# goroda/c3sc

Hardware: AMD Instinct MI355X
Metric: Bellman-sweep nodes/sec (7D car rank-10) (higher is better)
Workload: dtype f64

## Files before the change

c3sc_amd/csrc/c3sc_hip.hip:

```cpp
#include <hip/hip_runtime.h>

#include <algorithm>
#include <cmath>
#include <cstdio>
#include <cstdlib>
#include <cstring>
#include <string>
#include <vector>

#include "../../include/c3sc_hip.h"
#include "fiber_partition.hpp"
#include "kernel_common.hpp"
#include "kernel_rollout.hpp"
#include "kernel_rollout_ode.hpp"
#include "model_tables.hpp"
#include "registry.hpp"

namespace c3sc {

std::vector<KernelEntry> &kernel_registry()
{
    static std::vector<KernelEntry> reg;
    return reg;
}

__global__ void k_pad_core(const double *__restrict__ src, double *__restrict__ dst, int N, int r0, int r1, int RP,
                           int kind )
{
    const int per = (kind == 1) ? RP * RP : RP;
    const long total = (long)N * per;
    for (long e = (long)blockIdx.x * blockDim.x + threadIdx.x; e < total; e += (long)gridDim.x * blockDim.x) {
        const int j = (int)(e / per), w = (int)(e - (long)j * per);
        int a, b;
        if (kind == 0) { a = 0; b = w; }
        else if (kind == 2) { a = w; b = 0; }
        else { a = w % RP; b = w / RP; }
        double v = 0.0;
        if (a < r0 && b < r1) v = src[(size_t)j * r0 * r1 + a + (size_t)b * r0];
        dst[e] = v;
    }
}

struct ImgJobs {
    int n;
    long src[3 * MAXD + 2], dst[3 * MAXD + 2];
    int nodes[3 * MAXD + 2], per[3 * MAXD + 2], stride[3 * MAXD + 2];
    int tab[3 * MAXD + 2], nodes2[3 * MAXD + 2];
    long src2[3 * MAXD + 2];
};
__global__ void k_core_images(double *__restrict__ arena, const ImgJobs J)
{
    const int jb = blockIdx.y;
    const double *core = arena + J.src[jb];
    double *img = arena + J.dst[jb];
    const int per = J.per[jb], stride = J.stride[jb];
    if (J.tab[jb] != 0) {
        const double *core2 = arena + J.src2[jb];
        const int RP = per, n2 = J.nodes2[jb];
        const bool left = J.tab[jb] == 1;
        const long total = (long)J.nodes[jb] * n2 * RP;
        for (long e = (long)blockIdx.x * blockDim.x + threadIdx.x; e < total; e += (long)gridDim.x * blockDim.x) {
            const long row = e / RP;
            const int c = (int)(e - row * RP), a = (int)(row / n2), b = (int)(row - (long)a * n2);
            const double *vec = left ? core + (size_t)a * RP : core2 + (size_t)b * RP;
            const double *mat = left ? core2 + (size_t)b * RP * RP + (size_t)c * RP : core + (size_t)a * RP * RP + c;
            const int ms = left ? 1 : RP;
            double t = 0.0;
            for (int s = 0; s < RP; s++) t = fma(vec[s], mat[(size_t)s * ms], t);
            img[e] = t;
        }
        return;
    }
    const long total = (long)J.nodes[jb] * stride;
    for (long e = (long)blockIdx.x * blockDim.x + threadIdx.x; e < total; e += (long)gridDim.x * blockDim.x) {
        const int j = (int)(e / stride), w = (int)(e - (long)j * stride);
        img[e] = (w < per) ? core[(size_t)j * per + w] : 0.0;
    }
}

__global__ void k_quad_aux(const double *__restrict__ core, double *__restrict__ coreT, double *__restrict__ aop, int N, int RP)
{
    const int C = RP / 4, MB = (C + 3) / 4;
    const int per_t = RP * RP, per_a = 2 * MB * C * 64;
    const long total = (long)N * (per_t + per_a);
    for (long e = (long)blockIdx.x * blockDim.x + threadIdx.x; e < total; e += (long)gridDim.x * blockDim.x) {
        const int j = (int)(e / (per_t + per_a)), w = (int)(e - (long)j * (per_t + per_a));
        const double *G = core + (size_t)j * per_t;
        if (w < per_t) {
            const int a = w / RP, b = w % RP;
            coreT[(size_t)j * per_t + w] = G[a + b * RP];
        } else {
            const int u = w - per_t;
            const int l = u % 64, s = (u / 64) % C, mb = (u / (64 * C)) % MB, prod = u / (64 * C * MB);
            const int i = l % 16, g = 4 * mb + i / 4;
            const int xc = (i % 4) * C + g, yc = (l / 16) * C + s;
            double v = 0.0;
            if (g < C) v = (prod == 0) ? G[xc + yc * RP] : G[yc + xc * RP];
            aop[(size_t)j * per_a + u] = v;
        }
    }
}

__global__ void k_peak_fma(double *out, int iters)
{
    double a0 = threadIdx.x * 1e-9, a1 = a0 + 1, a2 = a0 + 2, a3 = a0 + 3, a4 = a0 + 4, a5 = a0 + 5, a6 = a0 + 6, a7 = a0 + 7;
    const double m = 1.0000001, c = 1e-9;
    for (int i = 0; i < iters; i++) {
        a0 = fma(a0, m, c); a1 = fma(a1, m, c); a2 = fma(a2, m, c); a3 = fma(a3, m, c);
        a4 = fma(a4, m, c); a5 = fma(a5, m, c); a6 = fma(a6, m, c); a7 = fma(a7, m, c);
    }
    out[(size_t)blockIdx.x * blockDim.x + threadIdx.x] = a0 + a1 + a2 + a3 + a4 + a5 + a6 + a7;
}

typedef double v4d __attribute__((ext_vector_type(4)));
__global__ void k_peak_mfma(double *out, int iters)
{
    v4d c0 = {0, 0, 0, 0}, c1 = c0, c2 = c0, c3 = c0;
    const double a = 1.0 + threadIdx.x * 1e-9, b = 1e-9;
    for (int i = 0; i < iters; i++) {
        c0 = __builtin_amdgcn_mfma_f64_16x16x4f64(a, b, c0, 0, 0, 0);
        c1 = __builtin_amdgcn_mfma_f64_16x16x4f64(a, b, c1, 0, 0, 0);
        c2 = __builtin_amdgcn_mfma_f64_16x16x4f64(a, b, c2, 0, 0, 0);
        c3 = __builtin_amdgcn_mfma_f64_16x16x4f64(a, b, c3, 0, 0, 0);
    }
    out[(size_t)blockIdx.x * blockDim.x + threadIdx.x] = c0[0] + c1[1] + c2[2] + c3[3];
}

}

using namespace c3sc;

#include "ctx.hpp"

static int model_ncf(int model) { return model == C3SC_MODEL_SCAR4D ? 1 : (model == C3SC_MODEL_COTHRUST6D ? 3 : 0); }
static double model_cand_feature(int model, int q, const double *u)
{
    if (model == C3SC_MODEL_COTHRUST6D) {
        const double m = 1.227, g = 9.81, mg = m * g;
        const double cphi = cos(u[1]), sphi = sin(u[1]), cth = cos(u[2]), sth = sin(u[2]);
        return q == 0 ? cphi * sth * (u[0] - mg) / m : (q == 1 ? -sphi * (u[0] - mg) / m : g + cth * cphi * (u[0] - mg) / m);
    }
    (void)q;
    return tan(u[0]);
}

static size_t static_layout(c3sc_hip_ctx *c)
{
    size_t off = c->xgrid_flat.size();
    c->obs_off = (int)off;
    off += c->obs.size();
    c->cands_off = (int)off;
    off += c->cands.size();
    for (int t = 0; t < 4; t++) c->tab_off[t] = 0;
    const int nt = model_ntab(c->model);
    for (int t = 0; t < nt; t++) {
        const int dim = model_tab_dim(c->model, t);
        c->tab_off[t] = (int)off;
        off += (dim < c->d) ? (size_t)c->ngrid[dim] : 0;
    }
    c->cfeat_off = (int)off;
    off += (size_t)model_ncf(c->model) * c->ncand;
    c->hz_off = (int)off;
    off += 4;
    return (off + 15) & ~(size_t)15;
}

static int upload_static(c3sc_hip_ctx *c)
{
    std::vector<double> st(c->static_doubles, 0.0);
    std::copy(c->xgrid_flat.begin(), c->xgrid_flat.end(), st.begin());
    std::copy(c->obs.begin(), c->obs.end(), st.begin() + c->obs_off);
    std::copy(c->cands.begin(), c->cands.end(), st.begin() + c->cands_off);
    const int nt = model_ntab(c->model);
    for (int t = 0; t < nt; t++) {
        const int dim = model_tab_dim(c->model, t);
        if (dim >= c->d) continue;
        const double *g = c->xgrid_flat.data() + c->xg_off_rel[dim];
        for (int i = 0; i < c->ngrid[dim]; i++) st[c->tab_off[t] + i] = model_table_value(c->model, t, g[i]);
    }
    const int ncf = model_ncf(c->model);
    for (int q = 0; q < c->ncand * ncf; q++)
        st[c->cfeat_off + q] = model_cand_feature(c->model, q % ncf, c->cands.data() + (size_t)(q / ncf) * c->du);
    if (c->hz_dt > 0.0) {
        st[c->hz_off] = c->hz_dt;
        st[c->hz_off + 1] = std::exp(-c->discount * c->hz_dt);
        st[c->hz_off + 2] = c->hz_dt / c->h2;
    }
    HIPCHK(c, hipMemcpy(c->arena, st.data(), st.size() * sizeof(double), hipMemcpyHostToDevice));
    c->static_dirty = false;
    return C3SC_OK;
}

static const size_t SMALL_BATCH_FIBERS = 16384;

template <class Fn>
static void each_entry(int model, Fn &&f)
{
    for (const auto &e : kernel_registry()) f(e);
    if (model == 0 || model >= C3SC_MODEL_USER) {
        const RtcEntries r = rtc_entries();
        for (int i = 0; i < r.n; i++) f(*r.e[i]);
    }
}

static const KernelEntry *find_kernel(int model, int d, int rank_needed, int N, int variant, int k, size_t F = (size_t)-1,
                                      const std::vector<const KernelEntry *> *skip = nullptr)
{
    const KernelEntry *best = nullptr;
    const bool small = (variant == C3SC_VARIANT_AUTO) && F < SMALL_BATCH_FIBERS;
    each_entry(model, [&](const KernelEntry &e) {
        if (!is_fiber_variant(e.variant)) return;
        if (e.model != model || e.d != d || e.rp < rank_needed || e.max_n < N) return;
        if (skip && std::find(skip->begin(), skip->end(), &e) != skip->end()) return;
        if (e.k >= 0 && e.k != k) return;
        if (variant != C3SC_VARIANT_AUTO && e.variant != variant) return;
        auto pref = [small](int v) {
            if (small) return v == C3SC_VARIANT_FIBER_PER_WAVE ? 0 : (v == C3SC_VARIANT_FIBER_PAIR ? 1 : (v == C3SC_VARIANT_FIBER_QUAD ? 2 : 3));
            return v == C3SC_VARIANT_FIBER_PAIR ? 0 : (v == C3SC_VARIANT_FIBER_QUAD ? 1 : (v == C3SC_VARIANT_FIBER_PER_WAVE ? 2 : 3));
        };
        if (!best || e.rp < best->rp || (e.rp == best->rp && pref(e.variant) < pref(best->variant)) ||
            (e.rp == best->rp && e.variant == best->variant && e.npl < best->npl))
            best = &e;
    });
    return best;
}

static int pick_rp(int d, int maxrank, int model, int variant)
{
    int rp = 0;
    if (variant != C3SC_VARIANT_AUTO)
        each_entry(model, [&](const KernelEntry &e) {
            if (is_fiber_variant(e.variant) && e.d == d && e.variant == variant && (model == 0 || e.model == model) && e.rp >= maxrank && (rp == 0 || e.rp < rp)) rp = e.rp;
        });
    if (rp) return rp;
    if (model != 0)
        each_entry(model, [&](const KernelEntry &e) {
            if (is_fiber_variant(e.variant) && e.d == d && e.model == model && e.rp >= maxrank && (rp == 0 || e.rp < rp)) rp = e.rp;
        });
    if (rp) return rp;
    each_entry(model, [&](const KernelEntry &e) {
        if (is_fiber_variant(e.variant) && e.d == d && e.rp >= maxrank && (rp == 0 || e.rp < rp)) rp = e.rp;
    });
    return rp;
}

static unsigned long long g_launches = 0;
static int fill_args(c3sc_hip_ctx *c, int k, size_t F, KArgs &A, bool need_model);

static int check_horizon_model(c3sc_hip_ctx *c, const char *what)
{
    if (c->hz_dt > 0.0 && !(c->model >= C3SC_MODEL_USER && rtc_model_horizon(c->model) && c->game_gsz == 0))
        return fail(c, C3SC_ERR_UNSUPPORTED, what);
    return C3SC_OK;
}

static int check_game_model(c3sc_hip_ctx *c, const char *what)
{
    int du = 0;
    bool game = false;
    if (c->game_gsz > 0 && !(c->model >= C3SC_MODEL_USER && rtc_model_info(c->model, du, game) && game && du == c->du))
        return fail(c, C3SC_ERR_UNSUPPORTED, what);
    return C3SC_OK;
}

static int ensure_scratch(c3sc_hip_ctx *c, size_t bytes)
{
    if (bytes <= c->scratch_bytes) return C3SC_OK;
    if (c->scratch) HIPCHK(c, hipFree(c->scratch));
    c->scratch = nullptr;
    c->scratch_bytes = 0;
    HIPCHK(c, hipMalloc(&c->scratch, bytes));
    c->scratch_bytes = bytes;
    return C3SC_OK;
}

static size_t align256(size_t x) { return (x + 255) & ~(size_t)255; }

static constexpr size_t ZERO_COPY_MAX_BYTES = (size_t)1 << 20;
static bool zero_copy_batch(size_t bytes)
{
    static const bool off = getenv("C3SC_NO_ZEROCOPY") != nullptr;
    return !off && bytes <= ZERO_COPY_MAX_BYTES;
}
static int ensure_pinned(c3sc_hip_ctx *c, size_t bytes)
{
    if (bytes <= c->pinned_bytes) return C3SC_OK;
    if (c->pinned) HIPCHK(c, hipHostFree(c->pinned));
    c->pinned = c->pinned_dev = nullptr;
    c->pinned_bytes = 0;
    const size_t cap = bytes < ((size_t)256 << 10) ? ((size_t)256 << 10) : bytes;
    HIPCHK(c, hipHostMalloc(&c->pinned, cap, hipHostMallocMapped | hipHostMallocPortable));
    HIPCHK(c, hipHostGetDevicePointer(&c->pinned_dev, c->pinned, 0));
    c->pinned_bytes = cap;
    return C3SC_OK;
}

enum SegDir { SEG_IN, SEG_OUT };
struct HostSeg { const void *host; size_t bytes; SegDir dir; };
enum Staging {
    STAGE_MAPPED_OR_SCRATCH,
    STAGE_SCRATCH,
    STAGE_PER_CALL,
};
struct DevPtr {
    void *p;
    template <class T> operator T *() const { return static_cast<T *>(p); }
};

template <size_t NS, class Call>
static int stage_host(c3sc_hip_ctx *c, Staging kind, const char *what, const HostSeg (&segs)[NS], Call &&call)
{
    size_t off[NS + 1] = {0};
    for (size_t i = 0; i < NS; i++) off[i + 1] = off[i] + align256(segs[i].bytes);
    auto copy = [&](SegDir dir, char *hb, const DevPtr *dev) -> int {
        for (size_t i = 0; i < NS; i++) {
            if (!dev[i].p || segs[i].dir != dir || segs[i].bytes == 0) continue;
            void *h = const_cast<void *>(segs[i].host), *b = hb ? hb + off[i] : dev[i].p;
            void *dst = dir == SEG_IN ? b : h, *src = dir == SEG_IN ? h : b;
            if (hb) memcpy(dst, src, segs[i].bytes);
            else if (hipError_t e = hipMemcpy(dst, src, segs[i].bytes, dir == SEG_IN ? hipMemcpyHostToDevice : hipMemcpyDeviceToHost); e != hipSuccess) {
                c->err = std::string(what) + ": hipMemcpy of buffer " + std::to_string(i) + (dir == SEG_IN ? " in: " : " out: ") + hipGetErrorString(e);
                return C3SC_ERR_HIP;
            }
        }
        return C3SC_OK;
    };
    auto run = [&](char *hb, char *db) -> int {
        DevPtr dev[NS];
        for (size_t i = 0; i < NS; i++) dev[i].p = segs[i].host ? db + off[i] : nullptr;
        int rc = copy(SEG_IN, hb, dev);
        if (rc == C3SC_OK) rc = call(dev);
        if (rc != C3SC_OK) return rc;
        if (hb) HIPCHK(c, hipStreamSynchronize(nullptr));
        return copy(SEG_OUT, hb, dev);
    };
    HIPCHK(c, hipSetDevice(c->device));
    const size_t total = off[NS];
    int rc;
    if (kind == STAGE_MAPPED_OR_SCRATCH && zero_copy_batch(total))
        return (rc = ensure_pinned(c, total)) != C3SC_OK ? rc : run((char *)c->pinned, (char *)c->pinned_dev);
    if (kind != STAGE_PER_CALL) return (rc = ensure_scratch(c, total)) != C3SC_OK ? rc : run(nullptr, (char *)c->scratch);
    void *buf = nullptr;
    HIPCHK(c, hipMalloc(&buf, total));
    rc = run(nullptr, (char *)buf);
    (void)hipFree(buf);
    return rc;
}

extern "C" {

int c3sc_hip_max_rank(int model, int d)
{
    int rp = 0;
    each_entry(model, [&](const KernelEntry &e) {
        if (e.model == model && e.d == d && e.rp > rp) rp = e.rp;
    });
    return rp;
}

int c3sc_hip_device_count(void)
{
    int n = 0;
    if (hipGetDeviceCount(&n) != hipSuccess) return 0;
    return n;
}

int c3sc_hip_ctx_create(int device, c3sc_hip_ctx **out)
{
    if (!out) return C3SC_ERR_ARG;
    *out = nullptr;
    int n = 0;
    if (hipGetDeviceCount(&n) != hipSuccess || n <= 0 || device < 0 || device >= n) return C3SC_ERR_NODEVICE;
    c3sc_hip_ctx *c = new c3sc_hip_ctx();
    c->device = device;
    if (hipSetDevice(device) != hipSuccess || hipMalloc((void **)&c->d_status, sizeof(unsigned)) != hipSuccess ||
        hipMemset(c->d_status, 0, sizeof(unsigned)) != hipSuccess || hipEventCreate(&c->ev0) != hipSuccess ||
        hipEventCreate(&c->ev1) != hipSuccess) {
        delete c;
        return C3SC_ERR_HIP;
    }
    *out = c;
    return C3SC_OK;
}

void c3sc_hip_ctx_destroy(c3sc_hip_ctx *c)
{
    if (!c) return;
    (void)hipSetDevice(c->device);
    if (c->arena) (void)hipFree(c->arena);
    if (c->hz_stack) (void)hipFree(c->hz_stack);
    if (c->d_status) (void)hipFree(c->d_status);
    if (c->d_dbg) (void)hipFree(c->d_dbg);
    if (c->scratch) (void)hipFree(c->scratch);
    if (c->sim_state) (void)hipFree(c->sim_state);
    for (void *p : c->part)
        if (p) (void)hipFree(p);
    if (c->pinned) (void)hipHostFree(c->pinned);
    c3sc_hip_cross_free(c);
    for (int i = 0; i < c3sc_hip_ctx::NSIDE; i++) {
        if (c->side[i]) { (void)hipStreamSynchronize(c->side[i]); (void)hipStreamDestroy(c->side[i]); }
        if (c->join_ev[i]) (void)hipEventDestroy(c->join_ev[i]);
    }
    if (c->fork_ev) (void)hipEventDestroy(c->fork_ev);
    if (c->ev0) (void)hipEventDestroy(c->ev0);
    if (c->ev1) (void)hipEventDestroy(c->ev1);
    delete c;
}

const char *c3sc_hip_last_error(const c3sc_hip_ctx *c) { return c ? c->err.c_str() : "null context"; }
const char *c3sc_hip_last_kernel(const c3sc_hip_ctx *c) { return c ? c->last_kernel : ""; }

int c3sc_hip_set_grid(c3sc_hip_ctx *c, int d, const size_t *ngrid, const double *const *xgrid)
{
    if (!c || !ngrid || !xgrid || d < 2 || d > MAXD) return fail(c, C3SC_ERR_ARG, "set_grid: need 2 <= d <= 12");
    c->d = d;
    c->xgrid_flat.clear();
    for (int m = 0; m < d; m++) {
        if (ngrid[m] < 2 || ngrid[m] > 4096) return fail(c, C3SC_ERR_ARG, "set_grid: need 2 <= N_m <= 4096");
        c->ngrid[m] = (int)ngrid[m];
        c->xg_off_rel[m] = (int)c->xgrid_flat.size();
        c->xgrid_flat.insert(c->xgrid_flat.end(), xgrid[m], xgrid[m] + ngrid[m]);
    }
    c->static_dirty = true;
    c->have_value = false;
    return C3SC_OK;
}

int c3sc_hip_set_boundary(c3sc_hip_ctx *c, const int *bctype, int nobs, const double *obs_lb, const double *obs_ub)
{
    if (!c || c->d == 0 || !bctype) return fail(c, C3SC_ERR_ARG, "set_boundary: set_grid first");
    if (nobs < 0 || nobs > C3SC_MAX_OBSTACLES) return fail(c, C3SC_ERR_ARG, "set_boundary: at most 10 obstacles (boundary.c:393)");
    for (int m = 0; m < c->d; m++) {
        if (bctype[m] != C3SC_ABSORB && bctype[m] != C3SC_PERIODIC && bctype[m] != C3SC_REFLECT)
            return fail(c, C3SC_ERR_ARG, "set_boundary: boundary type must be absorb/periodic/reflect (nodeutil.c:532-535)");
        c->bctype[m] = bctype[m];
    }
    c->nobs = nobs;
    c->obs.assign((size_t)nobs * 2 * c->d, 0.0);
    for (int o = 0; o < nobs; o++)
        for (int m = 0; m < c->d; m++) {
            c->obs[((size_t)o * 2 + 0) * c->d + m] = obs_lb[(size_t)o * c->d + m];
            c->obs[((size_t)o * 2 + 1) * c->d + m] = obs_ub[(size_t)o * c->d + m];
        }
    c->have_boundary = true;
    c->static_dirty = true;
    return C3SC_OK;
}

int c3sc_hip_set_consistent_ends(c3sc_hip_ctx *c, int on)
{
    if (!c) return C3SC_ERR_ARG;
    c->cends = on ? 1 : 0;
    return C3SC_OK;
}

int c3sc_hip_get_consistent_ends(const c3sc_hip_ctx *c) { return c ? c->cends : -1; }

int c3sc_hip_set_mca(c3sc_hip_ctx *c, double h2, const double *t, double discount)
{
    if (!c || c->d == 0 || !t) return fail(c, C3SC_ERR_ARG, "set_mca: set_grid first");
    c->h2 = h2;
    c->discount = discount;
    for (int i = 0; i < 2 * c->d; i++) c->t[i] = t[i];
    c->have_mca = true;
    if (c->hz_dt > 0.0) c->static_dirty = true;
    return C3SC_OK;
}

int c3sc_hip_set_horizon_step(c3sc_hip_ctx *c, double dt)
{
    if (!c) return C3SC_ERR_ARG;
    if (dt == 0.0) {
        if (c->hz_dt > 0.0) c->static_dirty = true;
        c->hz_dt = 0.0;
        return C3SC_OK;
    }
    if (!(dt > 0.0) || !std::isfinite(dt)) return fail(c, C3SC_ERR_ARG, "set_horizon_step: dt must be positive and finite (0 clears)");
    if (!c->have_mca) return fail(c, C3SC_ERR_ARG, "set_horizon_step: set_mca first");
    if (c->model == 0) return fail(c, C3SC_ERR_ARG, "set_horizon_step: set_model first");
    if (c->model < C3SC_MODEL_USER || !rtc_model_known(c->model))
        return fail(c, C3SC_ERR_UNSUPPORTED, "set_horizon_step: horizon mode needs a run-time compiled model (c3sc_hip_model_compile_fh with horizon = 1)");
    if (!rtc_model_horizon(c->model))
        return fail(c, C3SC_ERR_UNSUPPORTED, "set_horizon_step: this model was compiled without horizon kernels (c3sc_hip_model_compile_fh, horizon = 1)");
    if (c->game_gsz > 0) return fail(c, C3SC_ERR_UNSUPPORTED, "set_horizon_step: games have no horizon form");
    c->hz_dt = dt;
    c->static_dirty = true;
    return C3SC_OK;
}

int c3sc_hip_set_model(c3sc_hip_ctx *c, int model, const double *params, int nparams)
{
    if (!c || model <= 0 || nparams < 0 || nparams > C3SC_MAX_PARAMS) return fail(c, C3SC_ERR_ARG, "set_model: bad arguments");
    if (model >= C3SC_MODEL_USER && !rtc_model_known(model)) return fail(c, C3SC_ERR_ARG, "set_model: no run-time model has this id");
    c->model = model;
    std::memset(c->prm, 0, sizeof(c->prm));
    for (int i = 0; i < nparams; i++) c->prm[i] = params[i];
    c->static_dirty = true;
    return C3SC_OK;
}

int c3sc_hip_set_controls(c3sc_hip_ctx *c, int ncand, int du, const double *cands)
{
    if (!c || ncand < 1 || du < 1 || !cands) return fail(c, C3SC_ERR_ARG, "set_controls: bad arguments");
    c->ncand = ncand;
    c->du = du;
    c->cands.assign(cands, cands + (size_t)ncand * du);
    c->static_dirty = true;
    c->game_gsz = c->game_ngrp = c->game_order = 0;
    return C3SC_OK;
}

int c3sc_hip_set_game(c3sc_hip_ctx *c, int du_min, int nu, const double *U, int nw, const double *W, int order)
{
    if (!c) return C3SC_ERR_ARG;
    if (nu == 0) {
        c->game_gsz = c->game_ngrp = c->game_order = 0;
        return C3SC_OK;
    }
    if (order != C3SC_GAME_MINMAX && order != C3SC_GAME_MAXMIN) return fail(c, C3SC_ERR_ARG, "set_game: order must be C3SC_GAME_MINMAX or C3SC_GAME_MAXMIN");
    if (c->model == 0) return fail(c, C3SC_ERR_ARG, "set_game: set_model first");
    if (c->model == C3SC_MODEL_TABLE) return fail(c, C3SC_ERR_UNSUPPORTED, "set_game: the TABLE model has no game kernels");
    if (c->hz_dt > 0.0) return fail(c, C3SC_ERR_UNSUPPORTED, "set_game: games have no horizon form (c3sc_hip_set_horizon_step(ctx, 0) first)");
    int mdu = 0;
    bool has_game = false;
    if (c->model < C3SC_MODEL_USER || !rtc_model_info(c->model, mdu, has_game))
        return fail(c, C3SC_ERR_UNSUPPORTED, "set_game: games need a run-time compiled model (c3sc_hip_model_compile_ex with game = 1)");
    if (!has_game) return fail(c, C3SC_ERR_UNSUPPORTED, "set_game: this model was compiled without game kernels (c3sc_hip_model_compile_ex, game = 1)");
    if (nu < 0 || nw < 1 || du_min < 1 || du_min >= mdu || !U || !W)
        return fail(c, C3SC_ERR_ARG, "set_game: du_min + du_max must equal the model's du, each at least 1, with nu, nw >= 1 and both lists given");
    if ((long long)nu * nw > (1ll << 24)) return fail(c, C3SC_ERR_ARG, "set_game: nu * nw too large");
    const int dmax = mdu - du_min, ncand = nu * nw;
    std::vector<double> cands((size_t)ncand * mdu);
    for (int iu = 0; iu < nu; iu++)
        for (int iw = 0; iw < nw; iw++) {
            const size_t p = order == C3SC_GAME_MINMAX ? (size_t)iu * nw + iw : (size_t)iw * nu + iu;
            double *row = cands.data() + p * mdu;
            for (int i = 0; i < du_min; i++) row[i] = U[(size_t)iu * du_min + i];
            for (int i = 0; i < dmax; i++) row[du_min + i] = W[(size_t)iw * dmax + i];
        }
    c->ncand = ncand;
    c->du = mdu;
    c->cands.swap(cands);
    c->static_dirty = true;
    c->game_order = order;
    c->game_gsz = order == C3SC_GAME_MINMAX ? nw : nu;
    c->game_ngrp = order == C3SC_GAME_MINMAX ? nu : nw;
    return C3SC_OK;
}

int c3sc_hip_set_control_box(c3sc_hip_ctx *c, int du, const double *lb, const double *ub, int grid, int polish)
{
    if (!c || du < 1 || du > C3SC_MAX_DU || !lb || !ub || grid < 2 || polish < 0) return fail(c, C3SC_ERR_ARG, "set_control_box: bad arguments");
    double tot = 1.0;
    for (int i = 0; i < du; i++) {
        if (!(lb[i] <= ub[i])) return fail(c, C3SC_ERR_ARG, "set_control_box: lb > ub");
        c->box_lb[i] = lb[i];
        c->box_ub[i] = ub[i];
        tot *= grid;
    }
    if (tot > 1e6) return fail(c, C3SC_ERR_ARG, "set_control_box: grid^du too large");
    c->box_du = du; c->box_grid = grid; c->box_polish = polish;
    if (c->ncand == 0) {
        c->ncand = 1; c->du = du;
        c->cands.assign(du, 0.0);
        c->static_dirty = true;
    }
    return C3SC_OK;
}

int c3sc_hip_set_variant(c3sc_hip_ctx *c, int variant)
{
    if (!c) return C3SC_ERR_ARG;
    c->variant = variant;
    return C3SC_OK;
}

static int prepare_value(c3sc_hip_ctx *c, const size_t *ranks, size_t *cores_doubles)
{
    if (!c || c->d == 0 || !ranks) return fail(c, C3SC_ERR_ARG, "upload_value: set_grid first");
    const int d = c->d;
    if (ranks[0] != 1 || ranks[d] != 1) return fail(c, C3SC_ERR_ARG, "upload_value: ranks[0] and ranks[d] must be 1");
    size_t maxrank = 1;
    for (int m = 0; m <= d; m++) {
        if (ranks[m] < 1) return fail(c, C3SC_ERR_ARG, "upload_value: rank < 1");
        maxrank = std::max(maxrank, ranks[m]);
    }
    const int rp = pick_rp(d, (int)maxrank, c->model, c->variant);
    if (rp == 0) return fail(c, C3SC_ERR_UNSUPPORTED, "upload_value: no kernel instantiation for this (dim, rank)");
    HIPCHK(c, hipSetDevice(c->device));
    const size_t stat = static_layout(c);
    size_t off = stat;
    long core_off[MAXD];
    for (int m = 0; m < d; m++) {
        core_off[m] = (long)off;
        const size_t per = (m == 0 || m == d - 1) ? rp : (size_t)rp * rp;
        off += ((size_t)c->ngrid[m] * per + 15) & ~(size_t)15;
    }
    const size_t primary_end = off;
    long coreT_off[MAXD] = {0}, aop_off[MAXD] = {0};
    bool have_quad = false;
    for (const auto &e : kernel_registry())
        if (e.variant == C3SC_VARIANT_FIBER_QUAD && e.d == d && e.rp == rp && (c->model == 0 || e.model == c->model)) have_quad = true;
    if (rp % 4 == 0 && have_quad) {
        const int C = rp / 4, MB = (C + 3) / 4;
        for (int m = 1; m < d - 1; m++) {
            coreT_off[m] = (long)off;
            off += ((size_t)c->ngrid[m] * rp * rp + 15) & ~(size_t)15;
            aop_off[m] = (long)off;
            off += ((size_t)c->ngrid[m] * 2 * MB * C * 64 + 15) & ~(size_t)15;
        }
    }
    long img_off[MAXD] = {0};
    for (int m = 0; m < d; m++) {
        const size_t per = (m == 0 || m == d - 1) ? rp : (size_t)rp * rp;
        img_off[m] = (long)off;
        off += (size_t)pair_img_doubles(c->ngrid[m], (int)per);
    }
    long tabL_off = 0, tabR_off = 0;
    bool have_pair = false;
    for (const auto &e : kernel_registry())
        if (e.variant == C3SC_VARIANT_FIBER_PAIR && e.d == d && e.rp == rp) have_pair = true;
    if (d >= 4 && have_pair) {
        tabL_off = (long)off;
        off += (size_t)pair_tab_doubles(c->ngrid[0], c->ngrid[1], rp);
        tabR_off = (long)off;
        off += (size_t)pair_tab_doubles(c->ngrid[d - 2], c->ngrid[d - 1], rp);
    }
    long qimgL_off[MAXD] = {0}, qimgR_off[MAXD] = {0};
    if (rp % 4 == 0 && have_quad) {
        for (int m = 0; m < d; m++) {
            const size_t per = (m == 0 || m == d - 1) ? rp : (size_t)rp * rp;
            const size_t sz = ((size_t)c->ngrid[m] * (per + 2) + 15) & ~(size_t)15;
            if (m < d - 1) { qimgL_off[m] = (long)off; off += sz; }
            if (m > 0) { qimgR_off[m] = (long)off; off += sz; }
        }
    }
    if (off > c->arena_cap) {
        if (c->arena) HIPCHK(c, hipFree(c->arena));
        c->arena = nullptr;
        c->arena_cap = 0;
        HIPCHK(c, hipMalloc((void **)&c->arena, off * sizeof(double)));
        c->arena_cap = off;
        c->static_dirty = true;
    }
    if (stat != c->static_doubles) c->static_dirty = true;
    c->static_doubles = stat;
    for (int m = 0; m < d; m++) { c->core_off[m] = core_off[m]; c->coreT_off[m] = coreT_off[m]; c->aop_off[m] = aop_off[m]; c->img_off[m] = img_off[m]; c->qimgL_off[m] = qimgL_off[m]; c->qimgR_off[m] = qimgR_off[m]; }
    c->tabL_off = tabL_off;
    c->tabR_off = tabR_off;
    for (int m = 0; m <= d; m++) c->ranks[m] = ranks[m];
    c->rp = rp;
    *cores_doubles = primary_end - stat;
    if (c->static_dirty) return upload_static(c);
    return C3SC_OK;
}

static int make_quad_aux(c3sc_hip_ctx *c, void *stream)
{
    for (int m = 1; m < c->d - 1; m++) {
        if (c->aop_off[m] == 0) continue;
        const long total = (long)c->ngrid[m] * (c->rp * c->rp + 2 * ((c->rp / 4 + 3) / 4) * (c->rp / 4) * 64);
        const int grid = (int)std::min<long>((total + 255) / 256, 1024);
        hipLaunchKernelGGL(k_quad_aux, dim3(grid), dim3(256), 0, (hipStream_t)stream, c->arena + c->core_off[m],
                           c->arena + c->coreT_off[m], c->arena + c->aop_off[m], c->ngrid[m], c->rp);
    }
    ImgJobs J;
    J.n = 0;
    long maxtotal = 1;
    auto add = [&](long src, long dst, int nodes, int per, int stride) {
        J.src[J.n] = src; J.dst[J.n] = dst; J.nodes[J.n] = nodes; J.per[J.n] = per; J.stride[J.n] = stride;
        J.tab[J.n] = 0; J.nodes2[J.n] = 0; J.src2[J.n] = 0;
        J.n++;
        maxtotal = std::max(maxtotal, (long)nodes * stride);
    };
    for (int m = 0; m < c->d; m++) {
        const int per = (m == 0 || m == c->d - 1) ? c->rp : c->rp * c->rp;
        add(c->core_off[m], c->img_off[m], c->ngrid[m], per, per | 1);
        if (c->qimgL_off[m]) add(c->core_off[m], c->qimgL_off[m], c->ngrid[m], per, per + 2);
        if (c->qimgR_off[m]) add((m == c->d - 1) ? c->core_off[m] : c->coreT_off[m], c->qimgR_off[m], c->ngrid[m], per, per + 2);
    }
    auto add_tab = [&](int tab, long dst, int ma, int mb) {
        add(c->core_off[ma], dst, c->ngrid[ma], c->rp, c->rp);
        J.tab[J.n - 1] = tab; J.nodes2[J.n - 1] = c->ngrid[mb]; J.src2[J.n - 1] = c->core_off[mb];
        maxtotal = std::max(maxtotal, (long)c->ngrid[ma] * c->ngrid[mb] * c->rp);
    };
    if (c->tabL_off) add_tab(1, c->tabL_off, 0, 1);
    if (c->tabR_off) add_tab(2, c->tabR_off, c->d - 2, c->d - 1);
    hipLaunchKernelGGL(k_core_images, dim3((unsigned)std::min<long>((maxtotal + 255) / 256, 64), (unsigned)J.n), dim3(256), 0, (hipStream_t)stream,
                       c->arena, J);
    HIPCHK(c, hipGetLastError());
    return C3SC_OK;
}

static void pad_cores_host(int d, const int *ngrid, int rp, const size_t *ranks, const double *const *cores, double *const *dst)
{
    for (int m = 0; m < d; m++) {
        const size_t r0 = ranks[m], r1 = ranks[m + 1];
        const double *src = cores[m];
        const size_t per = (m == 0 || m == d - 1) ? rp : (size_t)rp * rp;
        for (int j = 0; j < ngrid[m]; j++)
            for (size_t b = 0; b < r1; b++)
                for (size_t a = 0; a < r0; a++) {
                    const size_t w = (m == 0) ? b : ((m == d - 1) ? a : a + b * rp);
                    dst[m][(size_t)j * per + w] = src[(size_t)j * r0 * r1 + a + b * r0];
                }
    }
}

int c3sc_hip_upload_value(c3sc_hip_ctx *c, const size_t *ranks, const double *const *cores)
{
    size_t cd = 0;
    int rc = prepare_value(c, ranks, &cd);
    if (rc != C3SC_OK) return rc;
    const int d = c->d, rp = c->rp;
    std::vector<double> buf(cd, 0.0);
    double *dst[MAXD];
    for (int m = 0; m < d; m++) dst[m] = buf.data() + (c->core_off[m] - (long)c->static_doubles);
    pad_cores_host(d, c->ngrid, rp, ranks, cores, dst);
    HIPCHK(c, hipMemcpy(c->arena + c->static_doubles, buf.data(), cd * sizeof(double), hipMemcpyHostToDevice));
    rc = make_quad_aux(c, nullptr);
    if (rc != C3SC_OK) return rc;
    HIPCHK(c, hipStreamSynchronize(nullptr));
    c->have_value = true;
    return C3SC_OK;
}

int c3sc_hip_upload_value_stack(c3sc_hip_ctx *c, int nstack, const size_t *ranks, const double *const *cores)
{
    if (!c) return C3SC_ERR_ARG;
    if (nstack == 0) {
        if (c->hz_stack) HIPCHK(c, hipFree(c->hz_stack));
        c->hz_stack = nullptr;
        c->hz_nstack = 0;
        return C3SC_OK;
    }
    if (nstack < 0 || !ranks || !cores) return fail(c, C3SC_ERR_ARG, "upload_value_stack: bad arguments");
    if (c->d == 0 || !c->have_value) return fail(c, C3SC_ERR_ARG, "upload_value_stack: upload_value first (the stack shares its static section)");
    if (static_layout(c) != c->static_doubles)
        return fail(c, C3SC_ERR_ARG, "upload_value_stack: static data changed size after upload_value; upload the value again");
    const int d = c->d;
    std::vector<int> rps(nstack);
    std::vector<long> offs((size_t)nstack * MAXD, 0);
    size_t off = c->static_doubles;
    for (int s = 0; s < nstack; s++) {
        const size_t *r = ranks + (size_t)s * (d + 1);
        if (r[0] != 1 || r[d] != 1) return fail(c, C3SC_ERR_ARG, "upload_value_stack: ranks[s][0] and ranks[s][d] must be 1");
        size_t maxrank = 1;
        for (int m = 0; m <= d; m++) {
            if (r[m] < 1) return fail(c, C3SC_ERR_ARG, "upload_value_stack: rank < 1");
            maxrank = std::max(maxrank, r[m]);
        }
        for (int m = 0; m < d; m++)
            if (!cores[(size_t)s * d + m]) return fail(c, C3SC_ERR_ARG, "upload_value_stack: null core");
        rps[s] = pick_rp(d, (int)maxrank, c->model, C3SC_VARIANT_AUTO);
        if (rps[s] == 0) return fail(c, C3SC_ERR_UNSUPPORTED, "upload_value_stack: no kernel instantiation for a stage's (dim, rank)");
        for (int m = 0; m < d; m++) {
            offs[(size_t)s * MAXD + m] = (long)off;
            const size_t per = (m == 0 || m == d - 1) ? rps[s] : (size_t)rps[s] * rps[s];
            off += ((size_t)c->ngrid[m] * per + 15) & ~(size_t)15;
        }
    }
    std::vector<double> buf(off - c->static_doubles, 0.0);
    for (int s = 0; s < nstack; s++) {
        double *dst[MAXD];
        for (int m = 0; m < d; m++) dst[m] = buf.data() + (offs[(size_t)s * MAXD + m] - (long)c->static_doubles);
        pad_cores_host(d, c->ngrid, rps[s], ranks + (size_t)s * (d + 1), cores + (size_t)s * d, dst);
    }
    HIPCHK(c, hipSetDevice(c->device));
    if (c->hz_stack) HIPCHK(c, hipFree(c->hz_stack));
    c->hz_stack = nullptr;
    c->hz_nstack = 0;
    HIPCHK(c, hipMalloc((void **)&c->hz_stack, off * sizeof(double)));
    HIPCHK(c, hipMemcpy(c->hz_stack + c->static_doubles, buf.data(), buf.size() * sizeof(double), hipMemcpyHostToDevice));
    c->hz_stack_static = c->static_doubles;
    c->hz_rp.swap(rps);
    c->hz_core_off.swap(offs);
    c->hz_nstack = nstack;
    return C3SC_OK;
}

int c3sc_hip_upload_value_device(c3sc_hip_ctx *c, const size_t *ranks, const double *const *d_cores, void *stream)
{
    size_t cd = 0;
    int rc = prepare_value(c, ranks, &cd);
    if (rc != C3SC_OK) return rc;
    const int d = c->d, rp = c->rp;
    for (int m = 0; m < d; m++) {
        const int kind = (m == 0) ? 0 : (m == d - 1 ? 2 : 1);
        const long total = (long)c->ngrid[m] * (kind == 1 ? rp * rp : rp);
        const int grid = (int)std::min<long>((total + 255) / 256, 1024);
        hipLaunchKernelGGL(k_pad_core, dim3(grid), dim3(256), 0, (hipStream_t)stream, d_cores[m], c->arena + c->core_off[m],
                           c->ngrid[m], (int)ranks[m], (int)ranks[m + 1], rp, kind);
    }
    HIPCHK(c, hipGetLastError());
    rc = make_quad_aux(c, stream);
    if (rc != C3SC_OK) return rc;
    c->have_value = true;
    return C3SC_OK;
}

static int fill_args(c3sc_hip_ctx *c, int k, size_t F, KArgs &A, bool need_model)
{
    if (!c) return C3SC_ERR_ARG;
    if (c->d == 0 || !c->have_boundary || !c->have_value) return fail(c, C3SC_ERR_ARG, "launch: grid, boundary and value must be set");
    if (need_model && (!c->have_mca || c->model == 0 || c->ncand == 0))
        return fail(c, C3SC_ERR_ARG, "launch: mca, model and controls must be set");
    if (k < 0 || k >= c->d) return fail(c, C3SC_ERR_ARG, "launch: dim_vary out of range");
    HIPCHK(c, hipSetDevice(c->device));
    if (c->static_dirty) {
        if (static_layout(c) != c->static_doubles)
            return fail(c, C3SC_ERR_ARG, "launch: static data changed size after upload_value; upload the value again");
        int rc = upload_static(c);
        if (rc != C3SC_OK) return rc;
    }
    std::memset(&A, 0, sizeof(A));
    A.d = c->d;
    A.k = k;
    A.N = c->ngrid[k];
    A.ncand = c->ncand;
    A.F = (long)F;
    for (int m = 0; m < c->d; m++) {
        A.ngrid[m] = c->ngrid[m];
        A.bctype[m] = c->bctype[m];
        A.xg_off[m] = c->xg_off_rel[m];
        A.core_off[m] = c->core_off[m];
        A.quad_coreT_off[m] = c->coreT_off[m];
        A.quad_aop_off[m] = c->aop_off[m];
        A.pair_img_off[m] = c->img_off[m];
        A.quad_imgL_off[m] = c->qimgL_off[m];
        A.quad_imgR_off[m] = c->qimgR_off[m];
    }
    A.img_base = c->arena;
    if (c->tabL_off && (c->tabL_off != pair_tabL_off(A, c->rp) || c->tabR_off != pair_tabR_off(A, c->rp)))
        return fail(c, C3SC_ERR_ARG, "launch: the pair kernel's product tables are not where the kernel looks for them");
    A.cends = c->cends;
    A.memo_keys = nullptr;
    A.skip = c->skip_flag;
    A.nobs = c->nobs;
    A.obs_off = c->obs_off;
    A.cands_off = c->cands_off;
    for (int t = 0; t < 4; t++) A.tab_off[t] = c->tab_off[t];
    A.cfeat_off = c->cfeat_off;
    A.h2 = c->h2;
    A.discount = c->discount;
    for (int i = 0; i < 2 * c->d; i++) A.t[i] = c->t[i];
    for (int i = 0; i < C3SC_MAX_PARAMS; i++) A.prm[i] = c->prm[i];
    A.status = c->d_status;
    A.game_gsz = c->game_gsz;
    A.game_ngrp = c->game_ngrp;
    A.game_order = c->game_order;
    A.hz_off = c->hz_dt > 0.0 ? c->hz_off : 0;
    {
        static const int dbg_env = [] { const char *e = getenv("C3SC_DBG"); return e ? atoi(e) : 0; }();
        A.dbg = dbg_env;
        if (dbg_env && !c->d_dbg) { HIPCHK(c, hipMalloc((void **)&c->d_dbg, 65536 * 8 * sizeof(unsigned long long))); }
        A.dbgbuf = c->d_dbg;
        if (A.dbg & 8) A.ncand = 1;
        if (A.dbg & 16) A.ncand = 3;
    }
    return C3SC_OK;
}

static void arm_memo(c3sc_hip_ctx *c, const KernelEntry *e, KArgs &A)
{
    A.memo_keys = nullptr;
    if (c->memo.keys == nullptr || e->variant != C3SC_VARIANT_FIBER_PER_WAVE) return;
    A.memo_keys = c->memo.keys; A.memo_vals = c->memo.vals; A.memo_capmask = c->memo.capmask; A.memo_epoch_bits = c->memo.epoch_bits;
    A.memo_shift = c->memo.shift; A.memo_counters = c->memo.counters; A.memo_mode = c->memo.mode;
    for (int m = 0; m < c->d; m++) A.memo_stride[m] = c->memo.stride[m];
    c->memo.applied = true;
}

static int launch_one(c3sc_hip_ctx *c, const KernelEntry *e, const KArgs &A, const LaunchIO &io, const char *unsupported = nullptr)
{
    c->last_kernel = e->name;
    g_launches++;
    c->status_cache_valid = false;
    const hipError_t he = launch_entry(*e, A, io);
    if (he == hipErrorNotSupported && unsupported) return fail(c, C3SC_ERR_UNSUPPORTED, unsupported);
    HIPCHK(c, he);
    return C3SC_OK;
}

constexpr long FIBER_PARTITION_MIN = 524288;
static long fiber_partition_min()
{
    const char *e = getenv("C3SC_FIBER_PARTITION");
    if (!e || !*e) return FIBER_PARTITION_MIN;
    const long v = atol(e);
    return v > 0 ? v : -1;
}

static long fiber_group_floor()
{
    const char *e = getenv("C3SC_FIBER_GROUP");
    if (!e || !*e) return FPART_MIN_PER_BIN;
    const long v = atol(e);
    return v > 0 ? v : -1;
}

static int partition_fibers(c3sc_hip_ctx *c, const KernelEntry *e, const KArgs &A, LaunchIO &io, int slot, int &launched)
{
    io.perm = nullptr;
    io.nlive = nullptr;
    launched = 0;
    if (e->variant != C3SC_VARIANT_FIBER_PAIR || e->rtc || A.ncand > 64) return C3SC_OK;
    bool faces = false;
    for (int m = 0; m < A.d; m++) faces = faces || (m != A.k && A.bctype[m] == C3SC_ABSORB);
    const long fmin = fiber_partition_min();
    if (!faces || fmin < 0 || A.F < fmin || A.F > 0x40000000L) return C3SC_OK;
    PartArgs P;
    P.d = A.d;
    P.k = A.k;
    P.F = A.F;
    for (int m = 0; m < MAXD; m++) { P.ngrid[m] = A.ngrid[m]; P.bctype[m] = A.bctype[m]; }
    fpart_plan(P, fpp_group_levels(A.d, e->rp, A.k), fiber_group_floor());
    const size_t need = fpart_bytes(A.F, P.nbins);
    if (need > c->part_bytes[slot]) {
        if (c->part[slot]) HIPCHK(c, hipFree(c->part[slot]));
        c->part[slot] = nullptr;
        c->part_bytes[slot] = 0;
        c->part_last[slot] = {};
        HIPCHK(c, hipMalloc(&c->part[slot], need));
        c->part_bytes[slot] = need;
    }
    const PartScratch ps = fpart_carve(c->part[slot], A.F, P.nbins);
    c->part_last[slot] = {ps.perm, ps.nlive, A.F, io.stream};
    HIPCHK(c, fpart_launch(P, io.idx, ps, io.stream));
    launched = 3;
    io.perm = ps.perm;
    io.nlive = ps.nlive;
    return C3SC_OK;
}

static int launch_bellman(c3sc_hip_ctx *c, int k, size_t F, const int32_t *d_idx, const int32_t *d_policy, double *d_out,
                          int32_t *d_uidx, int32_t *d_absorbed, void *stream, int part_slot = 0)
{
    KArgs A;
    int rc = fill_args(c, k, F, A, true);
    if (rc != C3SC_OK) return rc;
    int variant = c->variant;
    if (c->game_gsz > 0) {
        rc = check_game_model(c, "bellman_fibers: game mode needs a model compiled with game kernels of the game's du");
        if (rc != C3SC_OK) return rc;
        if (variant != C3SC_VARIANT_AUTO && variant != C3SC_VARIANT_FIBER_PER_WAVE)
            return fail(c, C3SC_ERR_UNSUPPORTED, "bellman_fibers: game mode runs on the fiber-per-wave kernel only (the pair and quad variants have no game form)");
        variant = C3SC_VARIANT_FIBER_PER_WAVE;
    }
    if (c->hz_dt > 0.0) {
        rc = check_horizon_model(c, "bellman_fibers: horizon mode needs a model compiled with horizon kernels (and no game)");
        if (rc != C3SC_OK) return rc;
        if (variant != C3SC_VARIANT_AUTO && variant != C3SC_VARIANT_FIBER_PER_WAVE)
            return fail(c, C3SC_ERR_UNSUPPORTED, "bellman_fibers: horizon mode runs on the fiber-per-wave kernel only (the pair and quad variants have no horizon form)");
        variant = C3SC_VARIANT_FIBER_PER_WAVE;
    }
    if (F == 0) return C3SC_OK;
    if (!d_idx || !d_out) return fail(c, C3SC_ERR_ARG, "bellman_fibers: null buffer");
    A.forced = d_policy;
    LaunchIO io{c->arena, d_idx, d_out, d_uidx, d_absorbed, nullptr, nullptr, nullptr, nullptr, (hipStream_t)stream};
    std::vector<const KernelEntry *> declined;
    hipError_t he = hipSuccess;
    int part_launches = 0;
    for (;;) {
        const KernelEntry *e = find_kernel(c->model, c->d, c->rp, A.N, variant, k, F, &declined);
        if (!e || e->rp != c->rp) {
            if (declined.empty()) return fail(c, C3SC_ERR_UNSUPPORTED, "bellman_fibers: no kernel instantiation for (model, dim, rank, N)");
            return fail(c, C3SC_ERR_UNSUPPORTED, he == hipErrorOutOfMemory
                            ? "bellman_fibers: N x rank^2 of the varying core exceeds the 160 KB of LDS the per-wave kernel stages it in"
                            : "bellman_fibers: no kernel instantiation serves this call (model, dim, rank, N, control mode)");
        }
        c->last_kernel = e->name;
        arm_memo(c, e, A);
        rc = partition_fibers(c, e, A, io, part_slot, part_launches);
        if (rc != C3SC_OK) return rc;
        he = launch_entry(*e, A, io);
        if (he != hipErrorOutOfMemory && he != hipErrorNotSupported) break;
        c->memo.applied = false;
        if (getenv("C3SC_VERBOSE")) fprintf(stderr, "c3sc: %s declined (%s), trying the next instantiation\n", e->name, hipGetErrorName(he));
        declined.push_back(e);
    }
    g_launches += 1 + part_launches;
    c->status_cache_valid = false;
    HIPCHK(c, he);
    return C3SC_OK;
}

int c3sc_hip_bellman_fibers(c3sc_hip_ctx *c, int k, size_t F, const int32_t *d_idx, double *d_out, int32_t *d_uidx,
                            int32_t *d_absorbed, void *stream)
{
    return launch_bellman(c, k, F, d_idx, nullptr, d_out, d_uidx, d_absorbed, stream);
}

static int launch_bellman_all(c3sc_hip_ctx *c, int nk, const int *ks, const size_t *F, const int32_t *const *d_idx,
                              const int32_t *const *d_policy, double *const *d_out, int32_t *const *d_uidx, int32_t *const *d_absorbed,
                              void *stream)
{
    if (!c) return C3SC_ERR_ARG;
    if (nk < 1 || nk > MAXD || !ks || !F || !d_idx || !d_out) return fail(c, C3SC_ERR_ARG, "bellman_fibers_all: bad arguments");
    static const bool no_overlap = getenv("C3SC_NO_OVERLAP") != nullptr;
    bool overlap = nk > 1 && !no_overlap && c->memo.keys == nullptr && c->skip_flag == nullptr;
    for (int s = 0; s < nk; s++) {
        if (ks[s] < 0 || ks[s] >= c->d) return fail(c, C3SC_ERR_ARG, "bellman_fibers_all: dim_vary out of range");
        if (F[s] > 0 && (!d_idx[s] || !d_out[s])) return fail(c, C3SC_ERR_ARG, "bellman_fibers_all: null buffer");
        if (d_policy && !d_policy[s]) return fail(c, C3SC_ERR_ARG, "bellman_fibers_all: null policy");
        for (int q = 0; q < s; q++)
            if (d_out[q] == d_out[s] && F[s] > 0) return fail(c, C3SC_ERR_ARG, "bellman_fibers_all: two segments share an output array");
    }
    hipStream_t st = (hipStream_t)stream;
    if (overlap) {
        HIPCHK(c, hipSetDevice(c->device));
        if (!c->fork_ev) {
            HIPCHK(c, hipEventCreateWithFlags(&c->fork_ev, hipEventDisableTiming));
            for (int i = 0; i < c3sc_hip_ctx::NSIDE; i++) {
                HIPCHK(c, hipStreamCreateWithFlags(&c->side[i], hipStreamNonBlocking));
                HIPCHK(c, hipEventCreateWithFlags(&c->join_ev[i], hipEventDisableTiming));
            }
        }
        HIPCHK(c, hipEventRecord(c->fork_ev, st));
        for (int i = 0; i < c3sc_hip_ctx::NSIDE; i++) HIPCHK(c, hipStreamWaitEvent(c->side[i], c->fork_ev, 0));
    }
    int rc = C3SC_OK;
    for (int s = 0; s < nk && rc == C3SC_OK; s++) {
        const int lane = overlap ? s % (c3sc_hip_ctx::NSIDE + 1) : 0;
        rc = launch_bellman(c, ks[s], F[s], d_idx[s], d_policy ? d_policy[s] : nullptr, d_out[s], d_uidx ? d_uidx[s] : nullptr,
                            d_absorbed ? d_absorbed[s] : nullptr, lane == 0 ? stream : (void *)c->side[lane - 1], lane);
    }
    if (overlap)
        for (int i = 0; i < c3sc_hip_ctx::NSIDE; i++) {
            HIPCHK(c, hipEventRecord(c->join_ev[i], c->side[i]));
            HIPCHK(c, hipStreamWaitEvent(st, c->join_ev[i], 0));
        }
    return rc;
}

int c3sc_hip_bellman_fibers_all(c3sc_hip_ctx *c, int nk, const int *ks, const size_t *F, const int32_t *const *d_idx, double *const *d_out,
                                int32_t *const *d_uidx, int32_t *const *d_absorbed, void *stream)
{
    return launch_bellman_all(c, nk, ks, F, d_idx, nullptr, d_out, d_uidx, d_absorbed, stream);
}

int c3sc_hip_policy_fibers_all(c3sc_hip_ctx *c, int nk, const int *ks, const size_t *F, const int32_t *const *d_idx,
                               const int32_t *const *d_policy, double *const *d_out, int32_t *const *d_absorbed, void *stream)
{
    if (!d_policy) return fail(c, C3SC_ERR_ARG, "policy_fibers_all: null policy");
    return launch_bellman_all(c, nk, ks, F, d_idx, d_policy, d_out, nullptr, d_absorbed, stream);
}

static int launch_box(c3sc_hip_ctx *c, int k, size_t F, const int32_t *d_idx, const double *d_policy_u, double *d_out,
                      double *d_uopt, int32_t *d_absorbed, void *stream)
{
    if (!c) return C3SC_ERR_ARG;
    if (c->box_du == 0) return fail(c, C3SC_ERR_ARG, "bellman_fibers_box: c3sc_hip_set_control_box first");
    if (c->game_gsz > 0) return fail(c, C3SC_ERR_UNSUPPORTED, "bellman_fibers_box: games have no control-box form");
    if (c->hz_dt > 0.0) return fail(c, C3SC_ERR_UNSUPPORTED, "bellman_fibers_box: horizon mode has no control-box form");
    if (model_ncf(c->model) != 0 && c->model != C3SC_MODEL_COTHRUST6D)
        return fail(c, C3SC_ERR_UNSUPPORTED, "bellman_fibers_box: this model needs transcendental functions of the control");
    KArgs A;
    int rc = fill_args(c, k, F, A, true);
    if (rc != C3SC_OK) return rc;
    if (F == 0) return C3SC_OK;
    if (!d_idx || !d_out) return fail(c, C3SC_ERR_ARG, "bellman_fibers_box: null buffer");
    A.cmode = 1;
    A.ugrid = c->box_grid;
    A.upolish = c->box_polish;
    for (int i = 0; i < c->box_du; i++) { A.ulb[i] = c->box_lb[i]; A.uub[i] = c->box_ub[i]; }
    A.uopt = d_uopt;
    A.forced_u = d_policy_u;
    const KernelEntry *e = find_kernel(c->model, c->d, c->rp, A.N, C3SC_VARIANT_FIBER_PER_WAVE, k);
    if (!e || e->rp != c->rp) return fail(c, C3SC_ERR_UNSUPPORTED, "bellman_fibers_box: no fiber-per-wave instantiation for (model, dim, rank, N)");
    arm_memo(c, e, A);
    LaunchIO io{c->arena, d_idx, d_out, nullptr, d_absorbed, nullptr, nullptr, nullptr, nullptr, (hipStream_t)stream};
    return launch_one(c, e, A, io, "bellman_fibers_box: no box-minimiser instantiation for this model");
}

int c3sc_hip_bellman_fibers_box(c3sc_hip_ctx *c, int k, size_t F, const int32_t *d_idx, double *d_out, double *d_uopt,
                                int32_t *d_absorbed, void *stream)
{
    return launch_box(c, k, F, d_idx, nullptr, d_out, d_uopt, d_absorbed, stream);
}

int c3sc_hip_policy_fibers_box(c3sc_hip_ctx *c, int k, size_t F, const int32_t *d_idx, const double *d_policy_u, double *d_out,
                               int32_t *d_absorbed, void *stream)
{
    if (F != 0 && !d_policy_u) return fail(c, C3SC_ERR_ARG, "policy_fibers_box: null policy");
    return launch_box(c, k, F, d_idx, d_policy_u, d_out, nullptr, d_absorbed, stream);
}

int c3sc_hip_bellman_fibers_box_host(c3sc_hip_ctx *c, int k, size_t F, const int32_t *h_idx, double *h_out, double *h_uopt,
                                     int32_t *h_absorbed)
{
    if (!c || c->d == 0 || k < 0 || k >= c->d || c->box_du == 0) return fail(c, C3SC_ERR_ARG, "bellman_fibers_box_host: bad arguments");
    if (F == 0) return C3SC_OK;
    const size_t FN = F * c->ngrid[k];
    return stage_host(c, STAGE_MAPPED_OR_SCRATCH, "bellman_fibers_box_host",
                      {{h_idx, F * c->d * sizeof(int32_t), SEG_IN}, {h_out, FN * sizeof(double), SEG_OUT},
                       {h_uopt, FN * c->box_du * sizeof(double), SEG_OUT}, {h_absorbed, FN * sizeof(int32_t), SEG_OUT}},
                      [&](const DevPtr *d) { return c3sc_hip_bellman_fibers_box(c, k, F, d[0], d[1], d[2], d[3], nullptr); });
}

int c3sc_hip_policy_fibers_box_host(c3sc_hip_ctx *c, int k, size_t F, const int32_t *h_idx, const double *h_policy_u, double *h_out,
                                    int32_t *h_absorbed)
{
    if (F != 0 && !h_policy_u) return fail(c, C3SC_ERR_ARG, "policy_fibers_box_host: null policy");
    if (!c || c->d == 0 || k < 0 || k >= c->d || c->box_du == 0) return fail(c, C3SC_ERR_ARG, "policy_fibers_box_host: bad arguments");
    if (F == 0) return C3SC_OK;
    const size_t FN = F * c->ngrid[k];
    return stage_host(c, STAGE_MAPPED_OR_SCRATCH, "policy_fibers_box_host",
                      {{h_idx, F * c->d * sizeof(int32_t), SEG_IN}, {h_out, FN * sizeof(double), SEG_OUT},
                       {h_policy_u, FN * c->box_du * sizeof(double), SEG_IN}, {h_absorbed, FN * sizeof(int32_t), SEG_OUT}},
                      [&](const DevPtr *d) { return c3sc_hip_policy_fibers_box(c, k, F, d[0], d[2], d[1], d[3], nullptr); });
}

int c3sc_hip_policy_fibers(c3sc_hip_ctx *c, int k, size_t F, const int32_t *d_idx, const int32_t *d_policy, double *d_out,
                           int32_t *d_absorbed, void *stream)
{
    if (F != 0 && !d_policy) return fail(c, C3SC_ERR_ARG, "policy_fibers: null policy");
    return launch_bellman(c, k, F, d_idx, d_policy, d_out, nullptr, d_absorbed, stream);
}

static int launch_tables(c3sc_hip_ctx *c, int k, size_t F, const int32_t *d_idx, const double *d_tables, const double *d_costs2,
                         const int32_t *d_policy, double *d_out, int32_t *d_uidx, int32_t *d_absorbed, void *stream)
{
    if (!c) return C3SC_ERR_ARG;
    const int saved_model = c->model;
    if (c->game_gsz > 0) return fail(c, C3SC_ERR_UNSUPPORTED, "bellman_fibers_tables: the TABLE model has no game kernels");
    if (c->hz_dt > 0.0) return fail(c, C3SC_ERR_UNSUPPORTED, "bellman_fibers_tables: the TABLE model has no horizon kernels");
    c->model = C3SC_MODEL_TABLE;
    KArgs A;
    int rc = fill_args(c, k, F, A, true);
    c->model = saved_model;
    if (rc != C3SC_OK) return rc;
    if (F == 0) return C3SC_OK;
    if (!d_idx || !d_out || !d_tables || !d_costs2) return fail(c, C3SC_ERR_ARG, "bellman_fibers_tables: null buffer");
    A.forced = d_policy;
    const KernelEntry *e = find_kernel(C3SC_MODEL_TABLE, c->d, c->rp, A.N, C3SC_VARIANT_AUTO, k);
    if (!e || e->rp != c->rp) return fail(c, C3SC_ERR_UNSUPPORTED, "bellman_fibers_tables: no kernel instantiation for (dim, rank, N)");
    LaunchIO io{c->arena, d_idx, d_out, d_uidx, d_absorbed, nullptr, nullptr, d_tables, d_costs2, (hipStream_t)stream};
    return launch_one(c, e, A, io);
}

int c3sc_hip_bellman_fibers_tables(c3sc_hip_ctx *c, int k, size_t F, const int32_t *d_idx, const double *d_tables,
                                   const double *d_costs2, double *d_out, int32_t *d_uidx, int32_t *d_absorbed, void *stream)
{
    return launch_tables(c, k, F, d_idx, d_tables, d_costs2, nullptr, d_out, d_uidx, d_absorbed, stream);
}

int c3sc_hip_policy_fibers_tables(c3sc_hip_ctx *c, int k, size_t F, const int32_t *d_idx, const double *d_tables,
                                  const double *d_costs2, const int32_t *d_policy, double *d_out, int32_t *d_absorbed, void *stream)
{
    if (F != 0 && !d_policy) return fail(c, C3SC_ERR_ARG, "policy_fibers_tables: null policy");
    return launch_tables(c, k, F, d_idx, d_tables, d_costs2, d_policy, d_out, nullptr, d_absorbed, stream);
}

int c3sc_hip_bellman_fibers_tables_host(c3sc_hip_ctx *c, int k, size_t F, const int32_t *h_idx, const double *h_tables,
                                        const double *h_costs2, double *h_out, int32_t *h_uidx, int32_t *h_absorbed)
{
    if (!c || c->d == 0 || k < 0 || k >= c->d || c->ncand == 0) return fail(c, C3SC_ERR_ARG, "bellman_fibers_tables_host: bad arguments");
    if (F == 0) return C3SC_OK;
    const size_t FN = F * c->ngrid[k], S = 2 * c->d + 1;
    return stage_host(c, STAGE_SCRATCH, "bellman_fibers_tables_host",
                      {{h_idx, F * c->d * sizeof(int32_t), SEG_IN}, {h_out, FN * sizeof(double), SEG_OUT}, {h_uidx, FN * sizeof(int32_t), SEG_OUT},
// ... 310 lines not shown
}

int c3sc_hip_simulate_host(c3sc_hip_ctx *c, const c3sc_hip_sim_args *h)
{
    if (!c) return C3SC_ERR_ARG;
    if (!h) return fail(c, C3SC_ERR_ARG, "simulate_host: null argument struct");
    if (h->n == 0) return c3sc_hip_simulate(c, h, nullptr);
    HostShape sh;
    const int rc = closed_loop_host_shape(c, "simulate", h, h->nsteps, sh);
    if (rc != C3SC_OK) return rc;
    const size_t n = sh.n, d = sh.d, D = sizeof(double);
    return stage_host(c, STAGE_PER_CALL, "simulate_host",
                      {{h->d_x0, n * d * D, SEG_IN}, {h->d_noise, h->d_noise ? n * h->nsteps * d * D : 0, SEG_IN},
                       {h->d_traj, h->d_traj ? n * sh.nrow * d * D : 0, SEG_OUT}, {h->d_u, h->d_u ? n * sh.nurow * sh.du * D : 0, SEG_OUT},
                       {h->d_cost, n * D, SEG_OUT}, {h->d_exit, n * sizeof(int64_t), SEG_OUT}, {h->d_vend, n * D, SEG_OUT},
                       {h->d_xfinal, n * d * D, SEG_OUT}},
                      [&](const DevPtr *b) {
                          c3sc_hip_sim_args a = *h;
                          a.d_x0 = b[0]; a.d_noise = b[1]; a.d_traj = b[2]; a.d_u = b[3];
                          a.d_cost = b[4]; a.d_exit = b[5]; a.d_vend = b[6]; a.d_xfinal = b[7];
                          return c3sc_hip_simulate(c, &a, nullptr);
                      });
}

static const size_t ODE_MAX_EVALS = (size_t)1 << 40;

static long long ode_nsub(double dt_out, double dt_int)
{
    if (dt_int == 0.0) return 1;
    const double r = dt_out / dt_int, q = std::nearbyint(r);
    if (!(q >= 1.0) || !(std::fabs(r - q) <= 1e-9 * q) || q > (double)(1 << 30)) return 0;
    return (long long)q;
}

static bool ode_box_ok(const double *b, int d)
{
    if (!b) return true;
    for (int m = 0; m < d; m++)
        if (!(b[m] <= b[d + m])) return false;
    return true;
}

int c3sc_hip_integrate(c3sc_hip_ctx *c, const c3sc_hip_ode_args *a, void *stream)
{
    const char *who = "integrate";
    int rc = closed_loop_setup(c, who, a);
    if (rc != C3SC_OK) return rc;
    if (c->hz_dt > 0.0) return fail(c, C3SC_ERR_UNSUPPORTED, "integrate: deterministic closed loops are not offered in horizon mode");
    KArgs A;
    rc = fill_args(c, 0, 0, A, false);
    if (rc != C3SC_OK) return rc;
    rc = check_bounds_set(c, "integrate: every dimension needs a boundary type");
    if (rc != C3SC_OK) return rc;
    if (!(a->dt_out > 0.0) || !std::isfinite(a->dt_out)) return fail(c, C3SC_ERR_ARG, "integrate: dt_out must be positive and finite");
    if (!(a->dt_int >= 0.0) || !std::isfinite(a->dt_int)) return fail(c, C3SC_ERR_ARG, "integrate: dt_int must be >= 0 and finite");
    const long long nsub = ode_nsub(a->dt_out, a->dt_int);
    if (nsub == 0) return fail(c, C3SC_ERR_ARG, "integrate: dt_out / dt_int is not an integer (to 1e-9 relative)");
    if (a->method != C3SC_ODE_FORWARD_EULER && a->method != C3SC_ODE_RK4)
        return fail(c, C3SC_ERR_ARG, "integrate: method must be C3SC_ODE_FORWARD_EULER or C3SC_ODE_RK4");
    const int nstage = a->method == C3SC_ODE_RK4 ? 4 : 1;
    if (a->nout > (size_t)1 << 30) return fail(c, C3SC_ERR_ARG, "integrate: nout too large");
    if ((size_t)nsub * a->nout * nstage > ODE_MAX_EVALS) return fail(c, C3SC_ERR_ARG, "integrate: more than 2^40 controller evaluations per trajectory");
    rc = closed_loop_sizes(c, who, a, a->nout, "integrate: more than 2^31 trajectories in one call (split the batch)",
                           "integrate: save_every larger than nout");
    if (rc != C3SC_OK) return rc;
    if (a->evals_per_launch < 0) return fail(c, C3SC_ERR_ARG, "integrate: evals_per_launch < 0");
    if (!ode_box_ok(a->goal, c->d) || !ode_box_ok(a->keep, c->d))
        return fail(c, C3SC_ERR_ARG, "integrate: a stop box has lo > hi (or a NaN)");
    const KernelEntry *e = find_sim_kernel(VARIANT_ROLLOUT_ODE, c->model, c->d, c->rp);
    if (!e) return fail(c, C3SC_ERR_UNSUPPORTED, "integrate: no integrate instantiation for this model at this padded rank");
    if (a->n == 0) return C3SC_OK;
    if (!a->d_x0) return fail(c, C3SC_ERR_ARG, "integrate: null d_x0");
    const int d = c->d;
    const size_t n = a->n;
    rc = closed_loop_state(c, n * (size_t)(d + 3) * sizeof(double));
    if (rc != C3SC_OK) return rc;
    closed_loop_box(c, a->box, A);
    OdeK S;
    std::memset(&S, 0, sizeof(S));
    S.n = (long)n;
    S.nsub = (int)nsub;
    S.nout = (int)a->nout;
    S.nstage = nstage;
    S.save_every = (int)a->save_every;
    S.wrap = a->wrap_periodic ? 1 : 0;
    S.constelm = c->constelm;
    S.h = a->dt_int == 0.0 ? a->dt_out : a->dt_int;
    S.dt_out = a->dt_out;
    S.has_goal = a->goal ? 1 : 0;
    S.has_keep = a->keep ? 1 : 0;
    for (int m = 0; m < d; m++) {
        S.goal_lo[m] = a->goal ? a->goal[m] : 0.0;
        S.goal_hi[m] = a->goal ? a->goal[d + m] : 0.0;
        S.keep_lo[m] = a->keep ? a->keep[m] : -INFINITY;
        S.keep_hi[m] = a->keep ? a->keep[d + m] : INFINITY;
    }
    S.x0 = a->d_x0;
    S.x = (double *)c->sim_state;
    S.cost = S.x + n * d;
    S.stop_step = (long long *)(S.cost + n);
    S.stop_reason = (int32_t *)(S.stop_step + n);
    S.traj = a->d_traj;
    S.u = a->d_u;
    S.vend = a->d_vend;
    const long long ktot = nsub * (long long)a->nout;
    const long long chunk = std::max<long long>(1, (a->evals_per_launch > 0 ? a->evals_per_launch : 256) / nstage);
    long long k0 = 0;
    do {
        S.k0 = k0;
        S.k1 = std::min(k0 + chunk, ktot);
        LaunchIO io{c->arena, nullptr, nullptr, nullptr, nullptr, nullptr, nullptr, nullptr, nullptr, (hipStream_t)stream, &S};
        rc = launch_one(c, e, A, io, "integrate: this integrate kernel has no box minimiser");
        if (rc != C3SC_OK) return rc;
        k0 = S.k1;
    } while (k0 < ktot);
    rc = closed_loop_results(c, a, a->d_stop_step, stream);
    if (rc != C3SC_OK) return rc;
    return copy_back(c, a->d_stop_reason, S.stop_reason, n * sizeof(int32_t), stream);
}

int c3sc_hip_integrate_host(c3sc_hip_ctx *c, const c3sc_hip_ode_args *h)
{
    if (!c) return C3SC_ERR_ARG;
    if (!h) return fail(c, C3SC_ERR_ARG, "integrate_host: null argument struct");
    if (h->n == 0) return c3sc_hip_integrate(c, h, nullptr);
    HostShape sh;
    const int rc = closed_loop_host_shape(c, "integrate", h, h->nout, sh);
    if (rc != C3SC_OK) return rc;
    const size_t n = sh.n, d = sh.d, D = sizeof(double);
    return stage_host(c, STAGE_PER_CALL, "integrate_host",
                      {{h->d_x0, n * d * D, SEG_IN}, {h->d_traj, h->d_traj ? n * sh.nrow * d * D : 0, SEG_OUT},
                       {h->d_u, h->d_u ? n * sh.nurow * sh.du * D : 0, SEG_OUT}, {h->d_cost, n * D, SEG_OUT},
                       {h->d_stop_step, n * sizeof(int64_t), SEG_OUT}, {h->d_stop_reason, n * sizeof(int32_t), SEG_OUT},
                       {h->d_vend, n * D, SEG_OUT}, {h->d_xfinal, n * d * D, SEG_OUT}},
                      [&](const DevPtr *b) {
                          c3sc_hip_ode_args a = *h;
                          a.d_x0 = b[0]; a.d_traj = b[1]; a.d_u = b[2]; a.d_cost = b[3];
                          a.d_stop_step = b[4]; a.d_stop_reason = b[5]; a.d_vend = b[6]; a.d_xfinal = b[7];
                          return c3sc_hip_integrate(c, &a, nullptr);
                      });
}

int c3sc_hip_normals(uint64_t seed, uint64_t traj0, size_t ntraj, uint64_t step0, size_t nsteps, int dw, double *out)
{
    if (!out || dw < 1 || dw > MAXD) return C3SC_ERR_ARG;
    for (size_t t = 0; t < ntraj; t++)
        for (size_t k = 0; k < nsteps; k++)
            for (int j = 0; j < dw; j++)
                out[(t * nsteps + k) * dw + j] = philox_normal(seed, traj0 + t, (uint32_t)(step0 + k), (uint32_t)j);
    return C3SC_OK;
}

unsigned long long c3sc_hip_launch_count(void) { return g_launches; }

int c3sc_hip_last_partition(c3sc_hip_ctx *c, int slot, int32_t *perm, size_t cap, size_t *F, int *nlive)
{
    if (!c) return C3SC_ERR_ARG;
    if (slot < 0 || slot > c3sc_hip_ctx::NSIDE || !F || !nlive) return fail(c, C3SC_ERR_ARG, "last_partition: bad arguments");
    const auto &lp = c->part_last[slot];
    if (!lp.perm) return fail(c, C3SC_ERR_ARG, "last_partition: no partition has run on this slot");
    *F = (size_t)lp.F;
    HIPCHK(c, hipStreamSynchronize(lp.stream));
    int32_t nl = 0;
    HIPCHK(c, hipMemcpy(&nl, lp.nlive, sizeof(nl), hipMemcpyDeviceToHost));
    *nlive = nl;
    if (perm) {
        if (cap < (size_t)lp.F) return fail(c, C3SC_ERR_ARG, "last_partition: perm holds fewer than F entries");
        HIPCHK(c, hipMemcpy(perm, lp.perm, (size_t)lp.F * sizeof(int32_t), hipMemcpyDeviceToHost));
    }
    return C3SC_OK;
}

int c3sc_hip_debug_read(c3sc_hip_ctx *c, unsigned long long *out, size_t n)
{
    if (!c || !c->d_dbg || !out) return C3SC_ERR_ARG;
    HIPCHK(c, hipMemcpy(out, c->d_dbg, n * sizeof(unsigned long long), hipMemcpyDeviceToHost));
    return C3SC_OK;
}

int c3sc_hip_timer_start(c3sc_hip_ctx *c, void *stream)
{
    if (!c) return C3SC_ERR_ARG;
    HIPCHK(c, hipEventRecord(c->ev0, (hipStream_t)stream));
    return C3SC_OK;
}

int c3sc_hip_timer_stop(c3sc_hip_ctx *c, void *stream, float *ms)
{
    if (!c || !ms) return C3SC_ERR_ARG;
    HIPCHK(c, hipEventRecord(c->ev1, (hipStream_t)stream));
    HIPCHK(c, hipEventSynchronize(c->ev1));
    HIPCHK(c, hipEventElapsedTime(ms, c->ev0, c->ev1));
    return C3SC_OK;
}

static int run_peak(c3sc_hip_ctx *c, bool mfma, double *tflops)
{
    if (!c || !tflops) return C3SC_ERR_ARG;
    HIPCHK(c, hipSetDevice(c->device));
    const char *ev = getenv("C3SC_PEAK_BLOCKS_PER_CU");
    const int blocks = 256 * (ev ? atoi(ev) : 8), threads = 256, iters = 20000;
    int rc = ensure_scratch(c, (size_t)blocks * threads * sizeof(double));
    if (rc != C3SC_OK) return rc;
    float best = 1e30f;
    for (int rep = 0; rep < 4; rep++) {
        HIPCHK(c, hipEventRecord(c->ev0, nullptr));
        if (mfma) hipLaunchKernelGGL(k_peak_mfma, dim3(blocks), dim3(threads), 0, nullptr, (double *)c->scratch, iters);
        else hipLaunchKernelGGL(k_peak_fma, dim3(blocks), dim3(threads), 0, nullptr, (double *)c->scratch, iters);
        HIPCHK(c, hipEventRecord(c->ev1, nullptr));
        HIPCHK(c, hipEventSynchronize(c->ev1));
        float ms = 0;
        HIPCHK(c, hipEventElapsedTime(&ms, c->ev0, c->ev1));
        if (rep > 0 && ms < best) best = ms;
    }
    const double waves = (double)blocks * threads / 64.0;
    const double flop = mfma ? waves * iters * 4.0 * (2.0 * 16 * 16 * 4) : (double)blocks * threads * iters * 8.0 * 2.0;
    *tflops = flop / (best * 1e-3) / 1e12;
    return C3SC_OK;
}

int c3sc_hip_peak_fma_f64(c3sc_hip_ctx *c, double *tflops) { return run_peak(c, false, tflops); }
int c3sc_hip_peak_mfma_f64(c3sc_hip_ctx *c, double *tflops) { return run_peak(c, true, tflops); }

}
```

c3sc_amd/csrc/ctx.hpp:

```cpp
#pragma once
#include <hip/hip_runtime.h>

#include <string>
#include <vector>

#include "../../include/c3sc_hip.h"
#include "kernel_common.hpp"

struct c3sc_cross_dev;
struct c3sc_hip_comm;

struct c3sc_hip_ctx {
    int device = 0;
    std::string err;
    int d = 0;
    int ngrid[c3sc::MAXD] = {0};
    std::vector<double> xgrid_flat;
    int xg_off_rel[c3sc::MAXD] = {0};
    int bctype[c3sc::MAXD] = {0};
    int cends = 0;
    bool have_boundary = false;
    int nobs = 0;
    std::vector<double> obs;
    bool have_mca = false;
    double h2 = 0, discount = 0, t[2 * c3sc::MAXD] = {0};
    int model = 0;
    double prm[C3SC_MAX_PARAMS] = {0};
    int ncand = 0, du = 0;
    std::vector<double> cands;
    int game_gsz = 0, game_ngrp = 0, game_order = 0;
    double hz_dt = 0.0;
    int hz_off = 0;
    double *hz_stack = nullptr;
    size_t hz_stack_static = 0;
    int hz_nstack = 0;
    std::vector<int> hz_rp;
    std::vector<long> hz_core_off;
    int box_du = 0, box_grid = 0, box_polish = 0;
    double box_lb[C3SC_MAX_DU] = {0}, box_ub[C3SC_MAX_DU] = {0};
    bool have_value = false;
    size_t ranks[c3sc::MAXD + 1] = {0};
    int rp = 0;
    double *arena = nullptr;
    size_t arena_cap = 0;
    size_t static_doubles = 0;
    bool static_dirty = true;
    long core_off[c3sc::MAXD] = {0};
    long coreT_off[c3sc::MAXD] = {0}, aop_off[c3sc::MAXD] = {0};
    long img_off[c3sc::MAXD] = {0};
    long qimgL_off[c3sc::MAXD] = {0}, qimgR_off[c3sc::MAXD] = {0};
    long tabL_off = 0, tabR_off = 0;
    int obs_off = 0, cands_off = 0, tab_off[4] = {0, 0, 0, 0}, cfeat_off = 0;
    unsigned *d_status = nullptr;
    unsigned status_cache = 0;
    bool status_cache_valid = false;
    unsigned long long *d_dbg = nullptr;
    int variant = C3SC_VARIANT_AUTO;
    const char *last_kernel = "";
    hipEvent_t ev0 = nullptr, ev1 = nullptr;
    static constexpr int NSIDE = 2;
    hipStream_t side[NSIDE] = {nullptr, nullptr};
    hipEvent_t fork_ev = nullptr, join_ev[NSIDE] = {nullptr, nullptr};
    void *part[NSIDE + 1] = {nullptr, nullptr, nullptr};
    size_t part_bytes[NSIDE + 1] = {0, 0, 0};
    struct {
        int32_t *perm = nullptr, *nlive = nullptr;
        long F = 0;
        hipStream_t stream = nullptr;
    } part_last[NSIDE + 1];
    void *scratch = nullptr;
    size_t scratch_bytes = 0;
    void *sim_state = nullptr;
    size_t sim_state_bytes = 0;
    int constelm = 0;
    void *pinned = nullptr, *pinned_dev = nullptr;
    size_t pinned_bytes = 0;
    struct {
        unsigned long long *keys = nullptr;
        double *vals = nullptr;
        unsigned long long capmask = 0, epoch_bits = 0;
        int shift = 0;
        long long stride[c3sc::MAXD] = {0};
        unsigned long long *counters = nullptr;
        int mode = 0;
        bool applied = false;
    } memo;
    const int *skip_flag = nullptr;
    c3sc_hip_comm *shard_comm = nullptr;
    c3sc_cross_dev *cross = nullptr;
};

#define HIPCHK(ctx, call)                                                                    \
    do {                                                                                     \
        hipError_t e__ = (call);                                                             \
        if (e__ != hipSuccess) {                                                             \
            (ctx)->err = std::string(#call) + ": " + hipGetErrorString(e__);                 \
            return C3SC_ERR_HIP;                                                             \
        }                                                                                    \
    } while (0)

static inline int fail(c3sc_hip_ctx *ctx, int code, const char *msg)
{
    if (ctx) ctx->err = msg;
    return code;
}
```

c3sc_amd/csrc/inst_car7d_fpp.hip:

```cpp
#include "launch_fpw.hpp"
#include "launch_fpp.hpp"
#include "models.hpp"
namespace c3sc {
#define REG7P(RP)                                  \
    C3SC_REG_FPP1(C3SC_MODEL_CAR7D, RP, 0, Car7D)  \
    C3SC_REG_FPP1(C3SC_MODEL_CAR7D, RP, 1, Car7D)  \
    C3SC_REG_FPP1(C3SC_MODEL_CAR7D, RP, 2, Car7D)  \
    C3SC_REG_FPP1(C3SC_MODEL_CAR7D, RP, 3, Car7D)  \
    C3SC_REG_FPP1(C3SC_MODEL_CAR7D, RP, 4, Car7D)  \
    C3SC_REG_FPP1(C3SC_MODEL_CAR7D, RP, 5, Car7D)  \
    C3SC_REG_FPP1(C3SC_MODEL_CAR7D, RP, 6, Car7D)
#define CAR7_MAP(K, MERGED, NVEC)                                                                   \
    static_assert(PairPark<Car7D, K>::merged() == (MERGED), "car7d: merged dimensions of K = " #K); \
    static_assert(PairMap<Car7D, K>::nv() == (NVEC), "car7d: folded vectors of K = " #K);
CAR7_MAP(0, 0x1Eu, 5)
CAR7_MAP(1, 0x1Du, 6)
CAR7_MAP(2, 0x18u, 9)
CAR7_MAP(3, 0x04u, 11)
CAR7_MAP(4, 0x0Bu, 7)
CAR7_MAP(5, 0x0Fu, 5)
CAR7_MAP(6, 0x17u, 5)
REG7P(4)
REG7P(10)
}
```

c3sc_amd/csrc/kernel_common.hpp:

```cpp
#pragma once
#ifdef __HIPCC_RTC__
#include "rtc_prelude.hpp"
#else
#include <type_traits>
#include <hip/hip_runtime.h>
#include <stdint.h>
#endif

#include "../../include/c3sc_hip.h"

#ifdef C3SC_STAMPS
#define C3SC_STAMPS_ON 1
#else
#define C3SC_STAMPS_ON 0
#endif

namespace c3sc {

constexpr int MAXD = C3SC_MAX_DIM;

struct KArgs {
    int d, k, N, ncand;
    long F;
    int ngrid[MAXD];
    int bctype[MAXD];
    int xg_off[MAXD];
    long core_off[MAXD];
    int nobs;
    int obs_off;
    int cands_off;
    int tab_off[4];
    int cfeat_off;
    double h2, discount;
    double t[2 * MAXD];
    double prm[C3SC_MAX_PARAMS];
    unsigned *status;
    unsigned long long *dbgbuf;
    const int32_t *forced;
    int dbg;
    int cmode, ugrid, upolish;
    double ulb[C3SC_MAX_DU], uub[C3SC_MAX_DU];
    double *uopt;
    const double *forced_u;
    int tbl_off;
    int hz_off;
    long quad_coreT_off[MAXD];
    long quad_aop_off[MAXD];
    int quad_sv_off;
    int quad_x_off;
    int quad_m1_off;
    int quad_ix_off;
    long quad_imgL_off[MAXD];
    long quad_imgR_off[MAXD];
    long pair_img_off[MAXD];
    int cends;
    int game_gsz;
    unsigned long long *memo_keys;
    double *memo_vals;
    unsigned long long memo_capmask, memo_epoch_bits;
    int memo_shift;
    int game_ngrp;
    long long memo_stride[MAXD];
    unsigned long long *memo_counters;
    const int *skip;
    int memo_mode;
    int game_order;
    const double *img_base;
};

__host__ __device__ constexpr long arena_block(long doubles) { return (doubles + 15) & ~15L; }
__host__ __device__ constexpr long pair_img_doubles(int nodes, int per) { return arena_block((long)nodes * (per | 1) + 2); }
__host__ __device__ constexpr long pair_tab_doubles(int na, int nb, int rp) { return arena_block((long)na * nb * rp); }
__host__ __device__ inline long pair_tabL_off(const KArgs &A, int rp) { return A.pair_img_off[A.d - 1] + pair_img_doubles(A.ngrid[A.d - 1], rp); }
__host__ __device__ inline long pair_tabR_off(const KArgs &A, int rp) { return pair_tabL_off(A, rp) + pair_tab_doubles(A.ngrid[0], A.ngrid[1], rp); }

struct KeyLevels {
    int n, major, minor;
};
__host__ __device__ constexpr KeyLevels fpp_key_levels(int d, int k, bool tab)
{
    const int lfirst = (tab && k >= 2) ? 2 : 1, rfirst = (tab && k <= d - 3) ? d - 3 : d - 2;
    const int nl = k - lfirst > 0 ? k - lfirst : 0, nr = rfirst - k > 0 ? rfirst - k : 0;
    if (nl > 0 && nr > 0) return {2, k - 1, k + 1};
    if (nl > 0) return {nl > 1 ? 2 : 1, k - 1, nl > 1 ? k - 2 : -1};
    if (nr > 0) return {nr > 1 ? 2 : 1, k + 1, nr > 1 ? k + 2 : -1};
    return {0, -1, -1};
}
#ifndef FPP_DIRECT_MAXD
#define FPP_DIRECT_MAXD 3
#endif
#ifndef FPP_EDGE_TABLES
#define FPP_EDGE_TABLES 1
#endif
#ifndef FPP_GROUP_FOLD
#define FPP_GROUP_FOLD 1
#endif
__host__ __device__ constexpr bool fpp_group_fold_optout(int d, int rp, int k) { return d == 7 && rp == 10 && k == 1; }
__host__ __device__ constexpr KeyLevels fpp_group_levels(int d, int rp, int k)
{
    const bool direct = d <= FPP_DIRECT_MAXD && rp <= 8;
    if (!FPP_GROUP_FOLD || direct || fpp_group_fold_optout(d, rp, k)) return {0, -1, -1};
    return fpp_key_levels(d, k, FPP_EDGE_TABLES && d >= 4);
}

__device__ inline int game_list_to_pair(const KArgs &A, int p)
{
    return A.game_order == C3SC_GAME_MAXMIN ? (p % A.game_gsz) * A.game_ngrp + p / A.game_gsz : p;
}
__device__ inline int game_pair_to_list(const KArgs &A, int i)
{
    return A.game_order == C3SC_GAME_MAXMIN ? (i % A.game_ngrp) * A.game_gsz + i / A.game_ngrp : i;
}

template <class M>
struct GameOf : M {
    static constexpr bool GAME = true;
};
template <class Model>
constexpr bool model_game()
{
    if constexpr (requires { Model::GAME; }) return Model::GAME;
    else return false;
}

template <class M>
struct HorizonOf : M {
    static constexpr bool HORIZON = true;
};
template <class Model>
constexpr bool model_horizon()
{
    if constexpr (requires { Model::HORIZON; }) return Model::HORIZON;
    else return false;
}

struct KOut {
    double *out;
    double *costs;
    int32_t *uidx;
    int32_t *absorbed;
};

__device__ inline void wave_sync()
{
    __builtin_amdgcn_fence(__ATOMIC_RELEASE, "wavefront");
    __builtin_amdgcn_wave_barrier();
    __builtin_amdgcn_fence(__ATOMIC_ACQUIRE, "wavefront");
}

__device__ inline bool fixed_neighbors(int i, int n, int bc, int &lo, int &hi)
{
    const bool first = (i == 0), last = (i == n - 1) & !first;
    const bool absorb = (bc == C3SC_ABSORB), reflect = (bc == C3SC_REFLECT);
    const int lo_first = absorb ? i : (reflect ? i : n - 2);
    const int hi_first = absorb ? i : i + 1;
    const int lo_last = absorb ? i : i - 1;
    const int hi_last = absorb ? i : (reflect ? i : 1);
    lo = first ? lo_first : (last ? lo_last : i - 1);
    hi = first ? hi_first : (last ? hi_last : i + 1);
    return (first | last) & absorb;
}

__device__ inline int vary_neighbors(int j, int n, int bc, int ab_in, int &lo, int &hi, int keep_ends = 0)
{
    int ab = ab_in;
    const int ab_end = keep_ends ? ab_in : 0;
    if (j == 0) {
        if (bc == C3SC_ABSORB) { lo = 0; hi = 0; ab = 1; }
        else if (bc == C3SC_REFLECT) { lo = 0; hi = 1; ab = ab_end; }
        else { lo = n - 2; hi = 1; ab = ab_end; }
    } else if (j == n - 1) {
        if (bc == C3SC_ABSORB) { lo = n - 1; hi = n - 1; ab = 1; }
        else if (bc == C3SC_REFLECT) { lo = n - 2; hi = n - 1; ab = ab_end; }
        else { lo = n - 2; hi = 1; ab = ab_end; }
    } else if (ab == 0) {
        lo = j - 1;
        hi = j + 1;
    } else {
        lo = j;
        hi = j;
    }
    return ab;
}

constexpr unsigned long long MEMO_PENDING = 1ull << 48, MEMO_EPOCH_MASK = ~((1ull << 49) - 1), MEMO_ID_MASK = (1ull << 48) - 1;
__device__ inline double memo_merge(unsigned long long *keys, double *vals, unsigned long long capmask, int shift, unsigned long long epoch_bits,
                                    unsigned long long id, double v, int &inserted, int &overflow)
{
    const unsigned long long K = epoch_bits | id, KP = K | MEMO_PENDING;
    unsigned long long slot = (id * 0x9E3779B97F4A7C15ull) >> shift;
    for (unsigned long long probe = 0; probe <= capmask; probe++, slot = (slot + 1) & capmask) {
        unsigned long long cur = __hip_atomic_load(&keys[slot], __ATOMIC_ACQUIRE, __HIP_MEMORY_SCOPE_AGENT);
        while ((cur & MEMO_EPOCH_MASK) != epoch_bits) {
            const unsigned long long prev = atomicCAS(&keys[slot], cur, KP);
            if (prev == cur) {
                vals[slot] = v;
                __hip_atomic_store(&keys[slot], K, __ATOMIC_RELEASE, __HIP_MEMORY_SCOPE_AGENT);
                inserted = 1;
                return v;
            }
            cur = prev;
        }
        if ((cur & ~MEMO_PENDING) == K)
            return (cur & MEMO_PENDING) ? v : __hip_atomic_load(&vals[slot], __ATOMIC_RELAXED, __HIP_MEMORY_SCOPE_AGENT);
    }
    overflow = 1;
    return v;
}

template <int D>
__device__ inline bool in_obstacle(const KArgs &A, const double *__restrict__ ro, const double (&x)[D])
{
    int any = 0;
    for (int o = 0; o < A.nobs; o++) {
        const double *lb = ro + A.obs_off + (size_t)o * 2 * D;
        const double *ub = lb + D;
        int outside = 0;
#pragma unroll
        for (int m = 0; m < D; m++) outside |= (int)(x[m] < lb[m]) | (int)(x[m] > ub[m]);
        any |= (outside == 0);
    }
    return any != 0;
}

template <int D>
__device__ inline unsigned obstacle_mask_fixed(const KArgs &A, const double *__restrict__ ro, const double (&x)[D], int skip)
{
    unsigned mask = 0;
    for (int o = 0; o < A.nobs; o++) {
        const double *lb = ro + A.obs_off + (size_t)o * 2 * D;
        const double *ub = lb + D;
        int outside = 0;
#pragma unroll
        for (int m = 0; m < D; m++)
            if (m != skip) outside |= (int)(x[m] < lb[m]) | (int)(x[m] > ub[m]);
        mask |= (outside == 0 ? 1u : 0u) << o;
    }
    return mask;
}
template <int D>
__device__ inline unsigned obstacle_mask_dim(const KArgs &A, const double *__restrict__ ro, int k, double xk)
{
    unsigned mask = 0;
    for (int o = 0; o < A.nobs; o++) {
        const double lb = ro[A.obs_off + (size_t)o * 2 * D + k], ub = ro[A.obs_off + (size_t)o * 2 * D + D + k];
        mask |= ((xk < lb || xk > ub) ? 0u : 1u) << o;
    }
    return mask;
}

// ... 765 lines not shown
```

c3sc_amd/csrc/kernel_fiber_pair.hpp:

```cpp
#pragma once
#include <utility>

#include "fold_lds.hpp"

#ifndef FPP_CGD
#define FPP_CGD 3
#endif
#ifndef FPP_PIPE2
#define FPP_PIPE2 1
#endif
#ifndef FPP_CG
#define FPP_CG 1
#endif
#ifndef FPP_NV
#define FPP_NV 4
#endif

#ifndef FPP_DIRECT_MAXD
#define FPP_DIRECT_MAXD 3
#endif
#ifndef FPP_EDGE_TABLES
#define FPP_EDGE_TABLES 1
#endif

// ... 30 lines not shown
__device__ inline void apply_core_and(const double *G, double (&W)[NW][RP], double (&E)[RP])
{
    constexpr int N1 = COUNT >= FPP_NV - 1 ? FPP_NV - 1 : COUNT;
    double tmp[N1 + 1][RP];
#pragma unroll
    for (int a = 0; a < RP; a++) tmp[0][a] = E[a];
#pragma unroll
    for (int s = 0; s < N1; s++)
#pragma unroll
        for (int a = 0; a < RP; a++) tmp[s + 1][a] = W[FIRST + s][a];
    if constexpr (ROWVEC) vecmat_lds<RP, N1 + 1>(G, tmp);
    else matvec_lds<RP, N1 + 1>(G, tmp);
#pragma unroll
    for (int a = 0; a < RP; a++) E[a] = tmp[0][a];
#pragma unroll
    for (int s = 0; s < N1; s++)
#pragma unroll
        for (int a = 0; a < RP; a++) W[FIRST + s][a] = tmp[s + 1][a];
    apply_core<RP, NW, FIRST + N1, COUNT - N1, ROWVEC, FPP_NV>(G, W);
}

template <int RP, int NW, int FIRST, int COUNT, bool ROWVEC>
__device__ __forceinline__ void apply_uni_and(const double *__restrict__ G, double (&W)[NW][RP], double (&E)[RP])
{
    constexpr int N1 = COUNT >= FPP_NV - 1 ? FPP_NV - 1 : COUNT;
    double tmp[N1 + 1][RP];
#pragma unroll
    for (int a = 0; a < RP; a++) tmp[0][a] = E[a];
#pragma unroll
    for (int s = 0; s < N1; s++)
#pragma unroll
        for (int a = 0; a < RP; a++) tmp[s + 1][a] = W[FIRST + s][a];
    apply_uni<RP, N1 + 1, ROWVEC>(G, tmp);
#pragma unroll
    for (int a = 0; a < RP; a++) E[a] = tmp[0][a];
#pragma unroll
    for (int s = 0; s < N1; s++)
#pragma unroll
        for (int a = 0; a < RP; a++) W[FIRST + s][a] = tmp[s + 1][a];
    apply_range_uni<RP, NW, FIRST + N1, COUNT - N1, ROWVEC, FPP_NV>(G, W);
}

template <int N, class F>
__device__ __forceinline__ void static_for(F &&f)
{
    [&]<int... Is>(std::integer_sequence<int, Is...>) { (f(std::integral_constant<int, Is>{}), ...); }(std::make_integer_sequence<int, N>{});
}

template <bool KEY, class Body>
__device__ __forceinline__ void fold_level(int v, Body &&body)
{
    if constexpr (KEY) {
        const int u = __builtin_amdgcn_readfirstlane(v);
        if (__ballot(v != u) == 0ull) body(std::true_type{}, u);
        else body(std::false_type{}, 0);
    } else
        body(std::false_type{}, 0);
}

__device__ inline void pair_barrier()
{
    asm volatile("s_waitcnt lgkmcnt(0)\n\ts_barrier" ::: "memory");
}

template <int H>
__device__ inline void stage_core_image(double *sK, const double *img, int n_doubles)
{
    typedef __attribute__((address_space(3))) char lds_char;
    typedef __attribute__((address_space(3))) void lds_void;
    typedef const __attribute__((address_space(1))) void glb_void;
    const int pieces = (n_doubles + 1) >> 1;
    const int lane = threadIdx.x & 63;
    for (int base = H * 64; base < pieces; base += FPP_THREADS) {
        const int b = max(min(base, pieces - 64), 0);
        const int p = min(b + lane, pieces - 1);
        __builtin_amdgcn_global_load_lds((glb_void *)(img + 2 * p), (lds_void *)((lds_char *)sK + 16 * b), 16, 0, 0);
    }
    asm volatile("s_waitcnt vmcnt(0)" ::: "memory");
}

template <int K>
__host__ __device__ constexpr int pair_owner(int m) { return m < K ? ((K - 1 - m) & 1) : ((m - K) & 1); }

template <class Model, int K>
struct PairPark {
    static constexpr int D = Model::D, NTAB = Model::NTAB;
    static constexpr unsigned UM = Model::UDEP_MASK, UC = Model::UCONST_MASK, ALL = (1u << D) - 1u;
    __host__ __device__ static constexpr bool has_deps()
    {
        if constexpr (requires { Model::HAS_DEPS; }) return Model::HAS_DEPS;
        else return false;
    }
    __host__ __device__ static constexpr unsigned dep(int m)
    {
        if constexpr (has_deps()) return Model::dep_mask(m);
        else return ALL;
    }
    __host__ __device__ static constexpr unsigned cost_dep()
    {
        if constexpr (has_deps()) return Model::COST_DEP;
        else return ALL;
    }
    __host__ __device__ static constexpr unsigned constd()
    {
        unsigned c = 0;
        if (has_deps())
            for (int m = 0; m < D; m++)
                if (!((UM >> m) & 1u) && !((dep(m) >> K) & 1u)) c |= 1u << m;
        return c;
    }
    __host__ __device__ static constexpr unsigned need()
    {
        unsigned n = cost_dep();
        for (int m = 0; m < D; m++) {
            const bool ctl = (UM >> m) & 1u, cst = (constd() >> m) & 1u;
            if ((!ctl && !cst) || (ctl && !((UC >> m) & 1u))) n |= dep(m);
        }
        return n & ALL;
    }
    __host__ __device__ static constexpr bool need_x(int m) { return m != K && ((need() >> m) & 1u); }
    __host__ __device__ static constexpr bool need_t(int t) { return Model::tab_dim(t) != K && ((need() >> Model::tab_dim(t)) & 1u); }
    __host__ __device__ static constexpr int row_x(int m)
    {
        int r = 0;
        for (int q = 0; q < m; q++) r += need_x(q);
        return r;
    }
    __host__ __device__ static constexpr int nx() { return row_x(D); }
    __host__ __device__ static constexpr int row_t(int t)
    {
        int r = nx();
        for (int q = 0; q < t; q++) r += need_t(q);
        return r;
    }
    __host__ __device__ static constexpr int nt() { return row_t(NTAB) - nx(); }
    __host__ __device__ static constexpr unsigned merged() { return constd() & ~(1u << K); }
    __host__ __device__ static constexpr unsigned rates() { return constd() & (1u << K); }
    __host__ __device__ static constexpr int row_pm(int m)
    {
        int r = nx() + nt();
        for (int q = 0; q < m; q++) r += 2 * ((rates() >> q) & 1u);
        return r;
    }
    __host__ __device__ static constexpr int row_q() { return row_pm(D); }
    __host__ __device__ static constexpr int rows() { return row_q() + (merged() != 0u); }
};

struct FoldPlan {
    int lfirst, rfirst;
    bool ledge, redge;
    int staged;
    int products;
};
template <class Model, int K, bool TAB = false>
struct PairMap {
    typedef PairPark<Model, K> PK;
    static constexpr int D = Model::D, NIT = D + 2, UL = D, UR = D + 1;
    __host__ __device__ static constexpr bool mg(int m) { return (PK::merged() >> m) & 1u; }
    template <bool LEFT>
    struct Side {
        static constexpr bool ROWVEC = LEFT;
        static constexpr int NC = LEFT ? K : D - 1 - K;
        static constexpr int EDGE = LEFT ? 0 : D - 1;
        static constexpr int U = LEFT ? UL : UR;
        __host__ __device__ static constexpr int depth(int m) { return LEFT ? m : D - 1 - m; }
        __host__ __device__ static constexpr int core(int q) { return LEFT ? q : D - 1 - q; }
        __host__ __device__ static constexpr bool tab() { return TAB && NC >= 2; }
        __host__ __device__ static constexpr int first() { return core(tab() ? 2 : 1); }
        __host__ __device__ static constexpr int nsteps() { return NC - depth(first()) > 0 ? NC - depth(first()) : 0; }
        __host__ __device__ static constexpr int step(int i) { return core(depth(first()) + i); }
        __host__ __device__ static constexpr int first_merged()
        {
            for (int q = 0; q < NC; q++)
                if (mg(core(q))) return core(q);
            return -1;
        }
        __host__ __device__ static constexpr int nv()
        {
            int c = count(U);
            for (int q = 0; q < NC; q++) c += count(core(q));
            return c;
        }
        __host__ __device__ static constexpr int cost_u()
        {
            int c = NC - 1 - depth(first_merged()) - (tab() && first_merged() == EDGE);
            for (int q = depth(first()); q < NC; q++) c += 2 * mg(core(q));
            return c;
        }
        __host__ __device__ static constexpr int cost_pair(int m)
        {
            return (tab() && depth(m) <= 1) ? 2 * (NC - 2) : (m != EDGE ? 2 : 0) + 2 * (NC - 1 - depth(m));
        }
        __host__ __device__ static constexpr int created(int m) { return !mg(m) ? m : (m == first_merged() ? U : -1); }
        template <int H>
        __host__ __device__ static constexpr int before(int m)
        {
            int c = 0;
            for (int q = 0; q < depth(m) && q < NC; q++)
                if (created(core(q)) >= 0 && owner(created(core(q))) == H) c += count(created(core(q)));
            return c;
        }
        template <int H>
        __host__ __device__ static constexpr int base() { return LEFT ? 0 : Side<true>::template before<H>(K); }
        template <int H>
        __host__ __device__ static constexpr int slot(int it) { return base<H>() + before<H>(it == U ? first_merged() : it); }
    };
    typedef Side<true> SL;
    typedef Side<false> SR;
    __host__ __device__ static constexpr bool valid(int it)
    {
        return it == UL ? SL::first_merged() >= 0 : (it == UR ? SR::first_merged() >= 0 : (it != K && !mg(it)));
    }
    __host__ __device__ static constexpr int count(int it) { return !valid(it) ? 0 : (it < D ? 2 : 1); }
    __host__ __device__ static constexpr int nv() { return SL::nv() + SR::nv(); }
    __host__ __device__ static constexpr int gslot(int it)
    {
        if (it == UL) return 0;
        if (it == UR) return SL::nv();
        int c = it < K ? count(UL) : SL::nv() + count(UR);
        for (int m = it < K ? 0 : K + 1; m < it; m++) c += count(m);
        return c;
    }
    __host__ __device__ static constexpr int cost(int it)
    {
        if (!valid(it)) return 0;
        if (it == UL) return SL::cost_u();
        if (it == UR) return SR::cost_u();
        return it < K ? SL::cost_pair(it) : SR::cost_pair(it);
    }
    __host__ __device__ static constexpr FoldPlan plan()
    {
        FoldPlan p{SL::first(), SR::first(), K > 0 && !TAB, K < D - 1 && !TAB, 0, 0};
        p.staged = SL::nsteps() + SR::nsteps() + p.ledge + p.redge;
        p.products = SL::nsteps() + SR::nsteps();
        for (int it = 0; it < NIT; it++) p.products += cost(it);
        return p;
    }
    __host__ __device__ static constexpr int level_products(int m)
    {
        return 3 + (m < K ? SL::template before<0>(m) + SL::template before<1>(m) : SR::template before<0>(m) + SR::template before<1>(m));
    }
    __host__ __device__ static constexpr int uniform_rounds() { return fpp_key_levels(D, K, TAB).n; }
    __host__ __device__ static constexpr int uniform_products()
    {
        constexpr KeyLevels kl = fpp_key_levels(D, K, TAB);
        return (kl.n > 0 ? level_products(kl.major) : 0) + (kl.n > 1 ? level_products(kl.minor) : 0);
    }
    __host__ __device__ static constexpr int owner(int it)
    {
        if (PK::merged() == 0u) return pair_owner<K>(it);
        int load[2] = {0, 0}, own[NIT] = {};
        bool done[NIT] = {};
        for (int n = 0; n < NIT; n++) {
            int best = -1;
            for (int q = 0; q < NIT; q++)
                if (valid(q) && !done[q] && (best < 0 || cost(q) > cost(best))) best = q;
            if (best < 0) break;
            const int h = load[1] < load[0] ? 1 : 0;
            own[best] = h;
            load[h] += cost(best);
            done[best] = true;
        }
        return own[it];
    }
    template <int H>
    __host__ __device__ static constexpr int lslot(int it)
    {
        return (it == UL || it < K) ? SL::template slot<H>(it) : SR::template slot<H>(it);
    }
};

__host__ __device__ constexpr bool fpp_node_split_optout(int d, int rp, int k) { return rp < 10 || (d == 7 && rp == 10 && k == 4); }
template <class Model, int RP, int K>
__host__ __device__ constexpr bool fpp_node_split()
{
    if constexpr (!FPP_NODE_SPLIT || fpp_direct<Model, RP>()) return false;
    else
        return PairPark<Model, K>::merged() != 0u && PairMap<Model, K>::nv() * RP * 2 <= FPP_NODE_SPLIT_VGPRS &&
               !fpp_node_split_optout(Model::D, RP, K);
}

template <class Model, int K>
struct PairPre {
    static constexpr unsigned MASK = PairPark<Model, K>::merged(), RATES = PairPark<Model, K>::rates();
    const double *PX;
    int lane;
    double pvc;
    __device__ inline double q() const { return PX[PairPark<Model, K>::row_q() * 64 + lane]; }
    __device__ inline double pv() const { return pvc; }
    __device__ inline double pm(int m) const { return PX[PairPark<Model, K>::row_pm(m) * 64 + lane]; }
    __device__ inline double pp(int m) const { return PX[(PairPark<Model, K>::row_pm(m) + 1) * 64 + lane]; }
};

#define FPP_STAMP(slot)                                                   \
    if (C3SC_STAMPS_ON && (A.dbg & 128)) {                                \
        const unsigned long long now__ = clock64();                       \
        seg[slot] += now__ - tlast;                                       \
        tlast = now__;                                                    \
    }

template <class Model, int RP, int K, int H, bool PART, bool LEFT, int m, int NOWN, class Combine>
__device__ __attribute__((always_inline)) inline void fold_step(const KArgs &A, const double *__restrict__ ro, double *sK,
                                                               const int (&fi)[Model::D], const int (&nbm)[Model::D], const int (&nbp)[Model::D],
                                                               const double (&rpm)[Model::D], const double (&rpp)[Model::D], double (&V)[RP],
                                                               double (&W)[NOWN][RP], unsigned long long (&seg)[12], unsigned long long &tlast,
                                                               Combine &&combine)
{
    constexpr int D = Model::D;
    constexpr bool DIRECT = fpp_direct<Model, RP>();
    typedef PairMap<Model, K, fpp_edge_tables<Model, RP>()> PM;
    typedef typename PM::template Side<LEFT> SD;
    constexpr bool RV = SD::ROWVEC;
    constexpr int BASE = SD::template base<H>();
    constexpr KeyLevels KL = fpp_group_levels(D, RP, K);
    constexpr bool GROUP = PART && KL.n > 0;
    auto body = [&](auto uc, int iu) __attribute__((always_inline)) {
        constexpr bool UNI = decltype(uc)::value;
        constexpr int str = (DIRECT || UNI) ? RP * RP : fpl_lds_stride(RP * RP);
        constexpr int before = SD::template before<H>(m);
        constexpr bool PAIR = !PM::mg(m) && PM::owner(m) == H, ACC = PM::mg(m) && PM::owner(SD::U) == H;
        double nw[RP];
        const double *src = sK;
        FPP_STAMP(1)
        if constexpr (DIRECT || UNI) src = ro + A.core_off[m];
        else {
            pair_barrier();
            stage_core_image<H>(sK, A.img_base + A.pair_img_off[m], A.ngrid[m] * str);
            pair_barrier();
        }
        if constexpr (SD::tab() && m == SD::first()) combine();
        FPP_STAMP(7)
        const double *G = src + (UNI ? iu : fi[m]) * str;
        if constexpr (PAIR || ACC) {
            double t0[1][RP], t1[1][RP];
#pragma unroll
            for (int a = 0; a < RP; a++) { t0[0][a] = V[a]; t1[0][a] = V[a]; }
            if constexpr (DIRECT) {
                apply_glb<RP, 1, RV>(src + nbm[m] * str, t0);
                apply_glb<RP, 1, RV>(src + nbp[m] * str, t1);
            } else if constexpr (UNI) {
                apply_uni<RP, 1, RV>(src + __builtin_amdgcn_readfirstlane(nbm[m]) * str, t0);
                apply_uni<RP, 1, RV>(src + __builtin_amdgcn_readfirstlane(nbp[m]) * str, t1);
            } else if constexpr (RV) {
                vecmat_lds<RP, 1>(src + nbm[m] * str, t0);
                vecmat_lds<RP, 1>(src + nbp[m] * str, t1);
            } else {
                matvec_lds<RP, 1>(src + nbm[m] * str, t0);
                matvec_lds<RP, 1>(src + nbp[m] * str, t1);
            }
#pragma unroll
            for (int a = 0; a < RP; a++) {
                if constexpr (PAIR) { W[BASE + before][a] = t0[0][a]; W[BASE + before + 1][a] = t1[0][a]; }
                else nw[a] = fma(rpp[m], t1[0][a], rpm[m] * t0[0][a]);
            }
        }
        if constexpr (DIRECT) {
            double tl[1][RP];
#pragma unroll
            for (int a = 0; a < RP; a++) tl[0][a] = V[a];
            apply_glb<RP, 1, RV>(G, tl);
#pragma unroll
            for (int a = 0; a < RP; a++) V[a] = tl[0][a];
            apply_range_glb<RP, NOWN, BASE, before, RV>(G, W);
        } else if constexpr (UNI)
            apply_uni_and<RP, NOWN, BASE, before, RV>(G, W, V);
        else
            apply_core_and<RP, NOWN, BASE, before, RV>(G, W, V);
        if constexpr (ACC) {
            constexpr int su = SD::template slot<H>(SD::U);
#pragma unroll
            for (int a = 0; a < RP; a++) W[su][a] = (m == SD::first_merged()) ? nw[a] : W[su][a] + nw[a];
        }
    };
    fold_level<GROUP && (m == KL.major || (KL.n > 1 && m == KL.minor))>(fi[m], body);
}

template <class Model, int RP, int K, int H, bool FORCED, bool PART>
__device__ __attribute__((always_inline)) inline void fiber_pair_body(const KArgs &A, const double *__restrict__ ro,
                                                                     const int32_t *__restrict__ idx, double *__restrict__ outv,
                                                                     int32_t *__restrict__ uidx, int32_t *__restrict__ absorbed,
                                                                     const int32_t *__restrict__ perm, const int32_t *__restrict__ nlive_p,
                                                                     double *sK, unsigned &st)
{
    constexpr int D = Model::D;
    constexpr int S = 2 * D + 1;
    constexpr int RH = RP / 2;
    typedef PairPark<Model, K> PK;
    constexpr bool ET = fpp_edge_tables<Model, RP>();
    typedef PairMap<Model, K, ET> PM;
    constexpr FoldPlan PL = PM::plan();
    constexpr int NV = PM::nv();
    constexpr int NVL = PM::SL::nv();
    constexpr int NOL = PM::SL::template before<H>(K);
    constexpr int NOR = PM::SR::template before<H>(K);
    constexpr int NOWN = (NOL + NOR) > 0 ? (NOL + NOR) : 1;
    constexpr int NP = NV + 1;
    constexpr bool DIRECT = fpp_direct<Model, RP>();
    constexpr KeyLevels KL = fpp_group_levels(D, RP, K);
    constexpr bool GROUP = PART && KL.n > 0;
    static_assert(!GROUP || fpp_key_levels(D, K, ET).major == KL.major, "the key levels follow the kernel's own fold plan");
    static_assert(RP % 2 == 0, "rank-split kernel needs an even padded rank");
    const int lane = threadIdx.x & 63;
    const int N = A.N;
    const long ntiles = (A.F + 63) / 64;
    int first_dead = 0x7fffffff;
    if constexpr (PART) first_dead = __builtin_amdgcn_readfirstlane((int)(((long)*nlive_p + 63) >> 6));
    unsigned long long seg[12] = {0, 0, 0, 0, 0, 0, 0, 0, 0, 0, 0, 0}, tlast = clock64();
    CandLds<Model> cr;
    NodeLds<Model, K> nr;
    {
        CandRegs<Model> cr0;
        cr0.load(A, ro);
        NodeRegs<Model, K> nr0;
        nr0.load(A, ro);
        double *tb = sK + A.tbl_off;
        cr.fill(tb, cr0, A.ncand);
        nr.fill(tb + CandLds<Model>::doubles(A.ncand), nr0, N);
        pair_barrier();
    }

    for (long tile = blockIdx.x; tile < ntiles; tile += gridDim.x) {
        FPP_STAMP(7)
        const long f_raw = tile * 64 + lane;
        const bool live = f_raw < A.F;
        const long f_pos = live ? f_raw : A.F - 1;
        long f = f_pos;
        if constexpr (PART) f = (long)perm[f_pos];
        const bool dead_tile = PART && tile >= (long)first_dead;

        if constexpr (PART) if (dead_tile) {
            const bool whole = A.bctype[K] == C3SC_ABSORB || A.cends != 0;
            const int jb = whole ? 0 : 1, je = whole ? N : N - 1;
            double xb[D];
#pragma unroll
            for (int m = 0; m < D; m++) xb[m] = (m != K && PK::need_x(m)) ? ro[A.xg_off[m] + idx[f * D + m]] : 0.0;
            for (int j = jb + ((jb ^ H) & 1); j < je; j += 2) {
                xb[K] = nr.x_at(j);
                outv[(size_t)f * N + j] = Model::boundcost(A.prm, xb);
                if (uidx) uidx[(size_t)f * N + j] = -1;
                if (absorbed) absorbed[(size_t)f * N + j] = 1;
            }
            if (whole) continue;
        }

        int fi[D], nbm[D], nbp[D];
        bool fiber_abs = false;
        double x[D];
#pragma unroll
        for (int m = 0; m < D; m++) {
            fi[m] = (m == K) ? 0 : idx[f * D + m];
            const bool face = fixed_neighbors(fi[m], A.ngrid[m], A.bctype[m], nbm[m], nbp[m]);
            if (m != K) fiber_abs = fiber_abs || face;
            x[m] = ro[A.xg_off[m] + fi[m]];
        }

        const unsigned obs_fixed = obstacle_mask_fixed<D>(A, ro, x, K);
        double tv[Model::NTAB > 0 ? Model::NTAB : 1];
        table_values<Model>(A, ro, fi, tv);

        double rpm[D], rpp[D];
#pragma unroll
        for (int m = 0; m < D; m++) { rpm[m] = 0.0; rpp[m] = 0.0; }
        if constexpr (PK::constd() != 0) {
            typename Model::Node nd0;
            Model::prep(A.prm, x, tv, nd0);
            double u0[Model::DU], cf0[Model::NCF > 0 ? Model::NCF : 1], b0[D], s0[D];
#pragma unroll
            for (int i = 0; i < Model::DU; i++) u0[i] = cr.get_u(i, 0);
            cf0[0] = 0.0;
#pragma unroll
            for (int i = 0; i < Model::NCF; i++) cf0[i] = cr.get_cf(i, 0);
            Model::drift(A.prm, nd0, x, u0, cf0, b0);
            Model::sigma(A.prm, x, u0, s0);
#pragma unroll
            for (int m = 0; m < D; m++)
                if ((PK::constd() >> m) & 1u) upwind_rates(A.t[2 * m], A.t[2 * m + 1], b0[m], s0[m], rpm[m], rpp[m]);
        }

        double L[RP], R[RP], W[NOWN][RP];
#pragma unroll
        for (int a = 0; a < RP; a++) { L[a] = (a == 0) ? 1.0 : 0.0; R[a] = (a == 0) ? 1.0 : 0.0; }

        FPP_STAMP(0)
        if (!(C3SC_STAMPS_ON && (A.dbg & 1))) {
        if constexpr (K > 0) {
            constexpr bool OWN0 = PM::SL::tab() && (PM::mg(0) ? PM::owner(PM::UL) == H : PM::owner(0) == H);
            constexpr bool OWN1 = PM::SL::tab() && (PM::mg(1) ? PM::owner(PM::UL) == H : PM::owner(1) == H);
            double t0m[OWN0 ? RP : 1], t0p[OWN0 ? RP : 1], t1m[OWN1 ? RP : 1], t1p[OWN1 ? RP : 1];
            if constexpr (PM::SL::tab()) {
                const double *T = ro + pair_tabL_off(A, RP);
                const int n1 = A.ngrid[1];
                load_row16<RP>(T + ((long)fi[0] * n1 + fi[1]) * RP, L);
                if constexpr (OWN0) {
                    load_row16<RP>(T + ((long)nbm[0] * n1 + fi[1]) * RP, t0m);
                    load_row16<RP>(T + ((long)nbp[0] * n1 + fi[1]) * RP, t0p);
                }
                if constexpr (OWN1) {
                    load_row16<RP>(T + ((long)fi[0] * n1 + nbm[1]) * RP, t1m);
                    load_row16<RP>(T + ((long)fi[0] * n1 + nbp[1]) * RP, t1p);
                }
                __builtin_amdgcn_sched_barrier(0);
            }
            auto left_combine = [&]() __attribute__((always_inline)) {
                if constexpr (OWN0) {
#pragma unroll
                    for (int b = 0; b < RP; b++) {
                        if constexpr (PM::mg(0)) W[0][b] = fma(rpp[0], t0p[b], rpm[0] * t0m[b]);
                        else { W[0][b] = t0m[b]; W[1][b] = t0p[b]; }
                    }
                }
                if constexpr (OWN1) {
                    constexpr int before = PM::SL::template before<H>(1);
#pragma unroll
                    for (int b = 0; b < RP; b++) {
                        if constexpr (PM::mg(1)) {
                            constexpr int su = PM::template lslot<H>(PM::UL);
                            const double nw = fma(rpp[1], t1p[b], rpm[1] * t1m[b]);
                            W[su][b] = (1 == PM::SL::first_merged()) ? nw : W[su][b] + nw;
                        } else { W[before][b] = t1m[b]; W[before + 1][b] = t1p[b]; }
                    }
                }
            };
            if constexpr (PM::SL::tab() && K == PL.lfirst) left_combine();
            if constexpr (!PM::SL::tab()) {
                constexpr bool GLB = DIRECT || !PL.ledge;
                constexpr int str = GLB ? RP : fpl_lds_stride(RP);
                const double *src = sK;
                FPP_STAMP(1)
                if constexpr (GLB) src = ro + A.core_off[0];
                else {
                    pair_barrier();
                    stage_core_image<H>(sK, A.img_base + A.pair_img_off[0], A.ngrid[0] * str);
                    pair_barrier();
                }
                FPP_STAMP(7)
#pragma unroll
                for (int b = 0; b < RP; b++) {
                    L[b] = src[fi[0] * str + b];
                    if constexpr (PM::mg(0)) {
                        if constexpr (PM::owner(PM::UL) == H) W[0][b] = fma(rpp[0], src[nbp[0] * str + b], rpm[0] * src[nbm[0] * str + b]);
                    } else if constexpr (PM::owner(0) == H) {
                        W[0][b] = src[nbm[0] * str + b];
                        W[1][b] = src[nbp[0] * str + b];
                    }
                }
            }
            auto left_step = [&](auto mc) __attribute__((always_inline)) {
                fold_step<Model, RP, K, H, PART, true, decltype(mc)::value>(A, ro, sK, fi, nbm, nbp, rpm, rpp, L, W, seg, tlast, left_combine);
            };
            static_for<PM::SL::nsteps()>([&](auto ic) __attribute__((always_inline)) { left_step(std::integral_constant<int, PM::SL::step(decltype(ic)::value)>{}); });
        }

        if constexpr (K < D - 1) {
            constexpr bool OWN0 = PM::SR::tab() && (PM::mg(D - 1) ? PM::owner(PM::UR) == H : PM::owner(D - 1) == H);
            constexpr bool OWN1 = PM::SR::tab() && (PM::mg(D - 2) ? PM::owner(PM::UR) == H : PM::owner(D - 2) == H);
            double t0m[OWN0 ? RP : 1], t0p[OWN0 ? RP : 1], t1m[OWN1 ? RP : 1], t1p[OWN1 ? RP : 1];
            if constexpr (PM::SR::tab()) {
                const double *T = ro + pair_tabR_off(A, RP);
                const int n1 = A.ngrid[D - 1];
                load_row16<RP>(T + ((long)fi[D - 2] * n1 + fi[D - 1]) * RP, R);
                if constexpr (OWN0) {
                    load_row16<RP>(T + ((long)fi[D - 2] * n1 + nbm[D - 1]) * RP, t0m);
                    load_row16<RP>(T + ((long)fi[D - 2] * n1 + nbp[D - 1]) * RP, t0p);
                }
                if constexpr (OWN1) {
                    load_row16<RP>(T + ((long)nbm[D - 2] * n1 + fi[D - 1]) * RP, t1m);
                    load_row16<RP>(T + ((long)nbp[D - 2] * n1 + fi[D - 1]) * RP, t1p);
                }
                __builtin_amdgcn_sched_barrier(0);
            }
            auto right_combine = [&]() __attribute__((always_inline)) {
                if constexpr (OWN0) {
#pragma unroll
                    for (int a = 0; a < RP; a++) {
                        if constexpr (PM::mg(D - 1)) W[NOL][a] = fma(rpp[D - 1], t0p[a], rpm[D - 1] * t0m[a]);
                        else { W[NOL][a] = t0m[a]; W[NOL + 1][a] = t0p[a]; }
                    }
                }
                if constexpr (OWN1) {
                    constexpr int after = PM::SR::template before<H>(D - 2);
#pragma unroll
                    for (int a = 0; a < RP; a++) {
                        if constexpr (PM::mg(D - 2)) {
                            constexpr int su = PM::template lslot<H>(PM::UR);
                            const double nw = fma(rpp[D - 2], t1p[a], rpm[D - 2] * t1m[a]);
                            W[su][a] = (D - 2 == PM::SR::first_merged()) ? nw : W[su][a] + nw;
                        } else { W[NOL + after][a] = t1m[a]; W[NOL + after + 1][a] = t1p[a]; }
                    }
                }
            };
            if constexpr (PM::SR::tab() && K == PL.rfirst) right_combine();
            if constexpr (!PM::SR::tab()) {
                constexpr bool GLB = DIRECT || !PL.redge;
                constexpr int str = GLB ? RP : fpl_lds_stride(RP);
                const double *src = sK;
                FPP_STAMP(1)
                if constexpr (GLB) src = ro + A.core_off[D - 1];
                else {
                    pair_barrier();
                    stage_core_image<H>(sK, A.img_base + A.pair_img_off[D - 1], A.ngrid[D - 1] * str);
                    pair_barrier();
                }
                FPP_STAMP(7)
#pragma unroll
                for (int a = 0; a < RP; a++) {
                    R[a] = src[fi[D - 1] * str + a];
                    if constexpr (PM::mg(D - 1)) {
                        if constexpr (PM::owner(PM::UR) == H)
                            W[NOL][a] = fma(rpp[D - 1], src[nbp[D - 1] * str + a], rpm[D - 1] * src[nbm[D - 1] * str + a]);
                    } else if constexpr (PM::owner(D - 1) == H) {
                        W[NOL][a] = src[nbm[D - 1] * str + a];
                        W[NOL + 1][a] = src[nbp[D - 1] * str + a];
                    }
                }
            }
            auto right_step = [&](auto mc) __attribute__((always_inline)) {
                fold_step<Model, RP, K, H, PART, false, decltype(mc)::value>(A, ro, sK, fi, nbm, nbp, rpm, rpp, R, W, seg, tlast, right_combine);
            };
            static_for<PM::SR::nsteps()>([&](auto ic) __attribute__((always_inline)) { right_step(std::integral_constant<int, PM::SR::step(decltype(ic)::value)>{}); });
        }

        }
        FPP_STAMP(1)
        constexpr bool NS = fpp_node_split<Model, RP, K>();
        double Wh[NS ? 1 : NV][RH];
        double Wf[NS ? NV : 1][RP];
        if constexpr (NS) {
            double *X = sK;
            auto put_get_own = [&](auto ic, auto pc) __attribute__((always_inline)) {
                constexpr int it = decltype(ic)::value, P = decltype(pc)::value;
                if constexpr (PM::valid(it) && PM::owner(it) == H) {
                    constexpr int slot = PM::template lslot<H>(it);
#pragma unroll
                    for (int s = 0; s < PM::count(it); s++) {
                        const int g = PM::gslot(it) + s;
#pragma unroll
                        for (int i = 0; i < RH; i++) {
                            X[(g * RH + i) * 64 + lane] = W[slot + s][P * RH + i];
                            Wf[g][P * RH + i] = W[slot + s][P * RH + i];
                        }
                    }
                }
            };
            auto get_other = [&](auto ic, auto pc) __attribute__((always_inline)) {
                constexpr int it = decltype(ic)::value, P = decltype(pc)::value;
                if constexpr (PM::valid(it) && PM::owner(it) != H) {
#pragma unroll
                    for (int s = 0; s < PM::count(it); s++) {
                        const int g = PM::gslot(it) + s;
#pragma unroll
                        for (int i = 0; i < RH; i++) Wf[g][P * RH + i] = X[(g * RH + i) * 64 + lane];
                    }
                }
            };
            auto half = [&](auto pc) __attribute__((always_inline)) {
                pair_barrier();
                static_for<PM::NIT>([&](auto ic) __attribute__((always_inline)) { put_get_own(ic, pc); });
                pair_barrier();
                static_for<PM::NIT>([&](auto ic) __attribute__((always_inline)) { get_other(ic, pc); });
            };
            half(std::integral_constant<int, 0>{});
            half(std::integral_constant<int, 1>{});
            pair_barrier();
        } else {
            double *X = sK;
            pair_barrier();
            auto put_get_own = [&](auto ic) __attribute__((always_inline)) {
                constexpr int it = decltype(ic)::value;
                if constexpr (PM::valid(it) && PM::owner(it) == H) {
                    constexpr int slot = PM::template lslot<H>(it);
#pragma unroll
                    for (int s = 0; s < PM::count(it); s++) {
                        const int g = PM::gslot(it) + s;
#pragma unroll
                        for (int i = 0; i < RH; i++) {
                            X[(g * RH + i) * 64 + lane] = W[slot + s][(1 - H) * RH + i];
                            Wh[g][i] = W[slot + s][H * RH + i];
                        }
                    }
                }
            };
            static_for<PM::NIT>(put_get_own);
            pair_barrier();
            auto get_other = [&](auto ic) __attribute__((always_inline)) {
                constexpr int it = decltype(ic)::value;
                if constexpr (PM::valid(it) && PM::owner(it) != H) {
#pragma unroll
                    for (int s = 0; s < PM::count(it); s++) {
                        const int g = PM::gslot(it) + s;
#pragma unroll
                        for (int i = 0; i < RH; i++) Wh[g][i] = X[(g * RH + i) * 64 + lane];
                    }
                }
            };
            static_for<PM::NIT>(get_other);
            pair_barrier();
        }
        double *sL = sK, *sR = sK + RP * 64;
        {
#pragma unroll
            for (int a = 0; a < RP; a++) {
                if constexpr (H == 0) sL[a * 64 + lane] = L[a];
                else sR[a * 64 + lane] = R[a];
            }
            if constexpr (H == 0) {
                static_assert(PK::rows() <= NP, "parking rows exceed the reserved block");
                double *PXw = sK + (2 * RP + 2 * (NP + 1) + NP) * 64;
#pragma unroll
                for (int m = 0; m < D; m++)
                    if (PK::need_x(m)) PXw[PK::row_x(m) * 64 + lane] = x[m];
#pragma unroll
                for (int t = 0; t < Model::NTAB; t++)
                    if (PK::need_t(t)) PXw[PK::row_t(t) * 64 + lane] = tv[t];
#pragma unroll
                for (int m = 0; m < D; m++)
                    if ((PK::rates() >> m) & 1u) {
                        PXw[PK::row_pm(m) * 64 + lane] = rpm[m];
                        PXw[(PK::row_pm(m) + 1) * 64 + lane] = rpp[m];
                    }
                if constexpr (PK::merged() != 0u) {
                    double qc = 0.0;
#pragma unroll
                    for (int m = 0; m < D; m++)
                        if (PM::mg(m)) { qc += rpm[m]; qc += rpp[m]; }
                    PXw[PK::row_q() * 64 + lane] = qc;
                }
            }
            pair_barrier();
        }
        FPP_STAMP(2)

        const int bck = A.bctype[K];
        const double *Gk = ro + A.core_off[K];
        auto partials = [&](int j, auto &&sink) __attribute__((always_inline)) -> double {
            double pv;
            if constexpr (K == 0) {
                double ah[RH];
#pragma unroll
                for (int i = 0; i < RH; i++) ah[i] = Gk[(size_t)j * RP + H * RH + i];
                double v = 0.0;
#pragma unroll
                for (int i = 0; i < RH; i++) v = fma(ah[i], sR[(H * RH + i) * 64 + lane], v);
                pv = v;
#pragma unroll
                for (int g = 0; g < NV; g++) sink(g, dot_reg<RH>(ah, Wh[g]));
            } else if constexpr (K == D - 1) {
                double ch[RH];
#pragma unroll
                for (int i = 0; i < RH; i++) ch[i] = Gk[(size_t)j * RP + H * RH + i];
                double v = 0.0;
#pragma unroll
                for (int i = 0; i < RH; i++) v = fma(sL[(H * RH + i) * 64 + lane], ch[i], v);
                pv = v;
#pragma unroll
                for (int g = 0; g < NV; g++) sink(g, dot_reg<RH>(Wh[g], ch));
            } else {
                const double *GC0 = Gk + (size_t)j * RP * RP;
                const double *GC = GC0 + (size_t)H * RH * RP;
                double ch[RH], ah[RH];
#pragma unroll
                for (int i = 0; i < RH; i++) { ch[i] = 0.0; ah[i] = 0.0; }
#pragma unroll
                for (int b = 0; b < RP; b++) {
                    const double rb = sR[b * 64 + lane];
#pragma unroll
                    for (int i = 0; i < RH; i++) ch[i] = fma(GC0[H * RH + i + b * RP], rb, ch[i]);
                }
#pragma unroll
                for (int a = 0; a < RP; a++) {
                    const double la = sL[a * 64 + lane];
// ... 254 lines not shown
        }
        pair_barrier();
        } else {
        double vwrap = 0.0;
        if (bck == C3SC_PERIODIC) {
            const double pv = partials(N - 2, [](int, double) __attribute__((always_inline)) {});
            if constexpr (H == 0) B0[NP * 64 + lane] = pv;
            else B1[NP * 64 + lane] = pv;
            pair_barrier();
            vwrap = pv + (H == 0 ? B1[NP * 64 + lane] : B0[NP * 64 + lane]);
            pair_barrier();
        }
        double vone = 0.0;
        double v_m2 = 0.0, v_m1 = 0.0;
        double Vd[NP];
#pragma unroll
        for (int g = 0; g < NP; g++) Vd[g] = 0.0;

        const int T = N / 2 + 1;
        for (int t = 0; t < T; t++) {
            const int j0 = 2 * t, j1 = 2 * t + 1;
            const bool has0 = j0 < N, has1 = j1 < N;
            double pv0 = 0.0, pv1 = 0.0;
            double Pown[NP];
#pragma unroll
            for (int g = 0; g < NP; g++) Pown[g] = 0.0;
            auto own_sink = [&](int g, double v) __attribute__((always_inline)) { Pown[g] = v; };
            if constexpr (K > 0 && K < D - 1 && FPP_PIPE2) {
                if (has0 && has1) {
                    double chA[RH], ahA[RH], chB[RH], ahB[RH];
                    auto nofill = [](int) __attribute__((always_inline)) {};
                    auto value_of = [&](const double (&ch)[RH]) __attribute__((always_inline)) -> double {
                        double v = 0.0;
#pragma unroll
                        for (int i = 0; i < RH; i++) v = fma(sL[(H * RH + i) * 64 + lane], ch[i], v);
                        return v;
                    };
                    if constexpr (H == 0) {
                        auto sinkA = to_lds(B0);
                        ca_part(j1, chA, ahA, nofill);
                        ca_part(j0, chB, ahB, [&](int q) __attribute__((always_inline)) { dots_quarter(q, chA, ahA, sinkA); });
                        pv1 = value_of(chA);
                        sinkA(NV, pv1);
                        pv0 = dots_part(chB, ahB, own_sink);
                        B0[NP * 64 + lane] = pv0;
                    } else {
                        auto sinkA = to_lds(B1);
                        ca_part(j0, chA, ahA, nofill);
                        ca_part(j1, chB, ahB, [&](int q) __attribute__((always_inline)) { dots_quarter(q, chA, ahA, sinkA); });
                        pv0 = value_of(chA);
                        sinkA(NV, pv0);
                        pv1 = dots_part(chB, ahB, to_lds(B2));
                        B1[NP * 64 + lane] = pv1;
                    }
                } else if (has0) {
                    if constexpr (H == 0) { pv0 = partials(j0, own_sink); B0[NP * 64 + lane] = pv0; }
                    else pv0 = partials(j0, to_lds(B1));
                }
            } else if constexpr (H == 0) {
                if (has1) pv1 = partials(j1, to_lds(B0));
                if (has0) {
                    pv0 = partials(j0, own_sink);
                    B0[NP * 64 + lane] = pv0;
                }
            } else {
                if (has0) pv0 = partials(j0, to_lds(B1));
                if (has1) {
                    pv1 = partials(j1, to_lds(B2));
                    B1[NP * 64 + lane] = pv1;
                }
            }
            FPP_STAMP(3)
            pair_barrier();
            FPP_STAMP(4)
            double v0 = 0.0, v1 = 0.0;
            if constexpr (H == 0) {
                if (has1) v1 = pv1 + B1[NP * 64 + lane];
                if (has0) {
                    double P0[NP];
#pragma unroll
                    for (int g = 0; g < NP; g++) P0[g] = Pown[g] + B1[g * 64 + lane];
                    v0 = P0[NV];
                    double vlo, vhi;
                    dimk_values(j0, N, bck, v_m1, v0, v1, vwrap, (j0 == 0 ? v1 : vone), vlo, vhi);
                    finalize(j0, P0, vlo, vhi);
                }
            } else {
                if (has0) v0 = pv0 + B0[NP * 64 + lane];
                if (t >= 1) {
                    const int jn = j0 - 1;
                    double vlo, vhi;
                    dimk_values(jn, N, bck, v_m2, Vd[NV], v0, vwrap, (jn == 1 ? Vd[NV] : vone), vlo, vhi);
                    finalize(jn, Vd, vlo, vhi);
                }
                if (has1) {
#pragma unroll
                    for (int g = 0; g < NP; g++) Vd[g] = B0[g * 64 + lane] + B2[g * 64 + lane];
                    v1 = Vd[NV];
                }
            }
            if (t == 0) vone = v1;
            v_m2 = v0;
            v_m1 = v1;
            FPP_STAMP(5)
            pair_barrier();
            FPP_STAMP(6)
            if (PART && dead_tile && t == 0 && T > 3) t = T - 3;
        }
        }
    }
    if (C3SC_STAMPS_ON && (A.dbg & 128) && lane == 0) {
        const size_t w = ((size_t)blockIdx.x * 2 + H) * 12;
        if (w < 65536 * 8)
            for (int i = 0; i < 12; i++) A.dbgbuf[w + i] = seg[i];
    }
}

#ifndef FPP_WPS_LOW
#define FPP_WPS_LOW 4
#endif
#ifndef FPP_WPS_HIGH
#define FPP_WPS_HIGH 2
#endif
template <class Model, int RP>
__host__ __device__ constexpr int fpp_waves_per_simd() { return (fpp_direct<Model, RP>() && RP <= 6) ? FPP_WPS_LOW : (FPP_WPS_HIGH); }

template <class Model, int RP, int K, bool FORCED>
__global__ void __launch_bounds__(FPP_THREADS, (fpp_waves_per_simd<Model, RP>()))
    k_fiber_pair(const KArgs A, const double *__restrict__ ro, const int32_t *__restrict__ idx, double *__restrict__ outv,
                 int32_t *__restrict__ uidx, int32_t *__restrict__ absorbed)
{
    extern __shared__ double sKp[];
    unsigned st = 0;
    const int h = __builtin_amdgcn_readfirstlane(threadIdx.x >> 6);
    if (h == 0) fiber_pair_body<Model, RP, K, 0, FORCED, false>(A, ro, idx, outv, uidx, absorbed, nullptr, nullptr, sKp, st);
    else fiber_pair_body<Model, RP, K, 1, FORCED, false>(A, ro, idx, outv, uidx, absorbed, nullptr, nullptr, sKp, st);
    if (st) atomicOr(A.status, st);
}

template <class Model, int RP, int K, bool FORCED>
__global__ void __launch_bounds__(FPP_THREADS, (fpp_waves_per_simd<Model, RP>()))
    k_fiber_pair_part(const KArgs A, const double *__restrict__ ro, const int32_t *__restrict__ idx, double *__restrict__ outv,
                      int32_t *__restrict__ uidx, int32_t *__restrict__ absorbed, const int32_t *__restrict__ perm,
                      const int32_t *__restrict__ nlive_p)
{
    extern __shared__ double sKp[];
    unsigned st = 0;
    const int h = __builtin_amdgcn_readfirstlane(threadIdx.x >> 6);
    if (h == 0) fiber_pair_body<Model, RP, K, 0, FORCED, true>(A, ro, idx, outv, uidx, absorbed, perm, nlive_p, sKp, st);
    else fiber_pair_body<Model, RP, K, 1, FORCED, true>(A, ro, idx, outv, uidx, absorbed, perm, nlive_p, sKp, st);
    if (st) atomicOr(A.status, st);
}

}
```

c3sc_amd/csrc/launch_fpp.hpp:

```cpp
#pragma once
#include "kernel_fiber_pair.hpp"
#include "registry.hpp"

namespace c3sc {

template <class Model, int RP, int K>
__host__ __device__ constexpr size_t fpp_tile_doubles(bool node_split)
{
    constexpr int NV = PairMap<Model, K>::nv(), NP = NV + 1, RH = RP / 2;
    const size_t swap = (size_t)NV * RH * 64;
    const size_t parked = (size_t)(2 * RP + (NP + 1) * 2 + NP) * 64;
    const size_t rows = node_split ? parked + (size_t)PairPark<Model, K>::rows() * 64 : parked + (size_t)NP * 64;
    return swap > rows ? swap : rows;
}

template <class Model, int RP, int K, bool FORCED, bool PART>
hipError_t launch_fpp_impl(const KArgs &A, const LaunchIO &io)
{
    constexpr int D = Model::D;
    if (A.ncand > 64) return hipErrorNotSupported;
    constexpr bool NS = fpp_node_split<Model, RP, K>();
    static_assert(fpp_tile_doubles<Model, RP, K>(NS) <= fpp_tile_doubles<Model, RP, K>(false), "the node split must not need more LDS than the rank split");
    static_assert(!NS || 4 * fpp_tile_doubles<Model, RP, K>(NS) * sizeof(double) <= 160 * 1024, "four node-split workgroups per CU must fit the LDS");
    size_t doubles = fpp_tile_doubles<Model, RP, K>(false);
    for (int m = 0; m < D; m++) {
        if (m == K || fpp_direct<Model, RP>()) continue;
        const int elems = (m == 0 || m == D - 1) ? RP : RP * RP;
        const size_t need = ((size_t)A.ngrid[m] * fpl_lds_stride(elems) + 1) & ~(size_t)1;
        if (need > doubles) doubles = need;
    }
    KArgs B = A;
    B.tbl_off = (int)doubles;
    doubles += (size_t)CandLds<Model>::doubles(A.ncand) + (size_t)NodeLds<Model, K>::doubles(A.N);
    const size_t shmem = doubles * sizeof(double);
    const void *kern = PART ? (const void *)k_fiber_pair_part<Model, RP, K, FORCED> : (const void *)k_fiber_pair<Model, RP, K, FORCED>;
    static LaunchCache cache;
    int blocks_per_cu = 1, num_cu = 256;
    hipError_t e = cache.prepare(kern, FPP_THREADS, shmem, blocks_per_cu, num_cu);
    if (e != hipSuccess) return e;
    const long ntiles = (A.F + 63) / 64;
    const long cap = (long)num_cu * blocks_per_cu;
    int grid = (int)(ntiles < cap ? ntiles : cap);
    if (ntiles >= 8 * cap && ntiles < 0x7fffffffL) grid = (int)ntiles;
    if (grid < 1) grid = 1;
    if constexpr (PART)
        hipLaunchKernelGGL((k_fiber_pair_part<Model, RP, K, FORCED>), dim3(grid), dim3(FPP_THREADS), shmem, io.stream, B, io.ro, io.idx, io.out,
                           io.uidx, io.absorbed, io.perm, io.nlive);
    else
        hipLaunchKernelGGL((k_fiber_pair<Model, RP, K, FORCED>), dim3(grid), dim3(FPP_THREADS), shmem, io.stream, B, io.ro, io.idx, io.out, io.uidx,
                           io.absorbed);
    return hipGetLastError();
}

template <class Model, int RP, int K>
hipError_t launch_fpp(const KArgs &A, const LaunchIO &io)
{
    if (io.perm) return A.forced ? launch_fpp_impl<Model, RP, K, true, true>(A, io) : launch_fpp_impl<Model, RP, K, false, true>(A, io);
    return A.forced ? launch_fpp_impl<Model, RP, K, true, false>(A, io) : launch_fpp_impl<Model, RP, K, false, false>(A, io);
}

#define C3SC_REG_FPP1(MODEL_ID, RP, K, ...)                                                                   \
    static Registrar C3SC_CAT(reg_fpp_, __COUNTER__)(KernelEntry{                                             \
        MODEL_ID, __VA_ARGS__::D, RP, 0, C3SC_VARIANT_FIBER_PAIR, 128, K, &launch_fpp<__VA_ARGS__, RP, K>, \
        "k_fiber_pair<" #__VA_ARGS__ "," #RP ",K=" #K ">"});

}
```

c3sc_amd/csrc/registry.hpp:

```cpp
#pragma once
#ifndef __HIPCC_RTC__
#include <hip/hip_runtime.h>

#include <mutex>
#include <vector>
#endif

#include "kernel_common.hpp"

namespace c3sc {

#ifndef __HIPCC_RTC__
struct LaunchIO {
    const double *ro;
    const int32_t *idx;
    double *out;
    int32_t *uidx;
    int32_t *absorbed;
    const int32_t *nbf;
    const int32_t *nbv;
    const double *tbl;
    const double *tcost;
    hipStream_t stream;
    const void *sim = nullptr;
    const int32_t *perm = nullptr;
    const int32_t *nlive = nullptr;
};
#endif

constexpr int VARIANT_ROLLOUT = 100, VARIANT_STENCIL_POINTS = 101, VARIANT_ROLLOUT_ODE = 102;
__host__ __device__ constexpr bool is_fiber_variant(int v) { return v < VARIANT_ROLLOUT; }

#ifndef __HIPCC_RTC__
struct RtcLaunch;

typedef hipError_t (*launch_fn)(const KArgs &A, const LaunchIO &io);

struct KernelEntry {
    int model;
    int d;
    int rp;
    int npl;
    int variant;
    int max_n;
    int k;
    launch_fn fn;
    const char *name;
    const RtcLaunch *rtc = nullptr;
};

std::vector<KernelEntry> &kernel_registry();

struct LaunchCache {
    static constexpr int MAXDEV = 16;
    std::mutex mu;
    size_t attr_shmem[MAXDEV] = {0}, occ_shmem[MAXDEV] = {0};
    int blocks_per_cu[MAXDEV] = {0}, num_cu[MAXDEV] = {0};
    hipError_t prepare(const void *kern, int threads, size_t shmem, int &blocks, int &cus)
    {
        int dev = 0;
        hipError_t e = hipGetDevice(&dev);
        if (e != hipSuccess) return e;
        if (dev < 0 || dev >= MAXDEV) return hipErrorInvalidDevice;
        std::lock_guard<std::mutex> lk(mu);
        if (shmem > attr_shmem[dev]) {
            e = hipFuncSetAttribute(kern, hipFuncAttributeMaxDynamicSharedMemorySize, (int)shmem);
            if (e != hipSuccess) return e;
            attr_shmem[dev] = shmem;
        }
        if (blocks_per_cu[dev] == 0 || shmem != occ_shmem[dev]) {
            int nb = 0;
            e = hipOccupancyMaxActiveBlocksPerMultiprocessor(&nb, kern, threads, shmem);
            if (e != hipSuccess) return e;
            blocks_per_cu[dev] = nb > 0 ? nb : 1;
            occ_shmem[dev] = shmem;
        }
        if (num_cu[dev] == 0) {
            hipDeviceProp_t prop;
            e = hipGetDeviceProperties(&prop, dev);
            if (e != hipSuccess) return e;
            num_cu[dev] = prop.multiProcessorCount > 0 ? prop.multiProcessorCount : 256;
        }
        blocks = blocks_per_cu[dev];
        cus = num_cu[dev];
        return hipSuccess;
    }
};

struct Registrar {
    explicit Registrar(const KernelEntry &e) { kernel_registry().push_back(e); }
};

struct RtcEntries {
    const KernelEntry *const *e;
    int n;
};
RtcEntries rtc_entries();
hipError_t rtc_launch(const KernelEntry &e, const KArgs &A, const LaunchIO &io);
bool rtc_model_known(int model);
bool rtc_model_info(int model, int &du, bool &game);
bool rtc_model_horizon(int model);
inline hipError_t launch_entry(const KernelEntry &e, const KArgs &A, const LaunchIO &io) { return e.rtc ? rtc_launch(e, A, io) : e.fn(A, io); }
#endif

}
```

c3sc_amd/engine.py:

```python
from __future__ import annotations

import ctypes as C
import os
from typing import Optional, Sequence

import numpy as np

_HERE = os.path.dirname(os.path.abspath(__file__))
LIB_PATH = os.path.join(_HERE, "csrc", "libc3sc_hip.so")
_LIB = None

c_double_p = C.POINTER(C.c_double)
c_size_p = C.POINTER(C.c_size_t)
c_int_p = C.POINTER(C.c_int)
c_i32_p = C.POINTER(C.c_int32)

EXPORTS = [
    "c3sc_hip_ctx_create", "c3sc_hip_ctx_destroy", "c3sc_hip_last_error", "c3sc_hip_device_count", "c3sc_hip_max_rank",
    "c3sc_hip_set_grid", "c3sc_hip_set_boundary", "c3sc_hip_set_consistent_ends", "c3sc_hip_get_consistent_ends", "c3sc_hip_cross_setup", "c3sc_hip_cross_iteration", "c3sc_hip_cross_iteration_streamed", "c3sc_hip_cross_wait_core", "c3sc_hip_cross_iteration_pi", "c3sc_hip_cross_confirm", "c3sc_hip_bellman_fibers_all", "c3sc_hip_policy_fibers_all", "c3sc_hip_cross_speculate", "c3sc_hip_comm_unique_id", "c3sc_hip_comm_create", "c3sc_hip_comm_destroy", "c3sc_hip_comm_world", "c3sc_hip_comm_rank", "c3sc_hip_comm_allgather", "c3sc_hip_cross_set_comm", "c3sc_hip_comm_exchange", "c3sc_hip_cross_options", "c3sc_hip_cross_grow_memo", "c3sc_hip_cross_fetch", "c3sc_hip_cross_free", "c3sc_hip_set_mca", "c3sc_hip_set_model",
    "c3sc_hip_set_controls", "c3sc_hip_upload_value", "c3sc_hip_upload_value_device", "c3sc_hip_set_variant",
    "c3sc_hip_bellman_fibers", "c3sc_hip_bellman_fibers_tables", "c3sc_hip_bellman_fibers_tables_host", "c3sc_hip_stencil_fibers", "c3sc_hip_bellman_fibers_host",
    "c3sc_hip_policy_fibers", "c3sc_hip_policy_fibers_host", "c3sc_hip_policy_fibers_tables", "c3sc_hip_policy_fibers_tables_host",
    "c3sc_hip_set_control_box", "c3sc_hip_bellman_fibers_box", "c3sc_hip_bellman_fibers_box_host", "c3sc_hip_policy_fibers_box",
    "c3sc_hip_policy_fibers_box_host",
    "c3sc_hip_stencil_fibers_host", "c3sc_hip_stencil_fibers_nb", "c3sc_hip_stencil_fibers_nb_host", "c3sc_hip_sync", "c3sc_hip_get_status", "c3sc_hip_last_kernel",
    "c3sc_hip_debug_read", "c3sc_hip_launch_count", "c3sc_hip_last_partition", "c3sc_hip_timer_start", "c3sc_hip_timer_stop", "c3sc_hip_peak_fma_f64", "c3sc_hip_peak_mfma_f64",
    "c3sc_hip_set_interp", "c3sc_hip_stencil_points", "c3sc_hip_simulate", "c3sc_hip_simulate_host", "c3sc_hip_normals",
    "c3sc_hip_integrate", "c3sc_hip_integrate_host",
    "c3sc_hip_model_compile", "c3sc_hip_model_code_object", "c3sc_hip_model_log",
    "c3sc_hip_set_game", "c3sc_hip_model_compile_ex", "c3sc_hip_model_code_object_ex",
    "c3sc_hip_model_compile_fh", "c3sc_hip_model_code_object_fh", "c3sc_hip_set_horizon_step", "c3sc_hip_upload_value_stack",
]

class SimArgs(C.Structure):
    _fields_ = [("n", C.c_size_t), ("d_x0", C.c_void_p), ("dt", C.c_double), ("nsteps", C.c_size_t),
                ("traj_offset", C.c_uint64), ("seed", C.c_uint64), ("d_noise", C.c_void_p), ("wrap_periodic", C.c_int),
                ("box", C.c_int), ("steps_per_launch", C.c_int), ("save_every", C.c_size_t), ("d_traj", C.c_void_p),
                ("d_u", C.c_void_p), ("d_cost", C.c_void_p), ("d_exit", C.c_void_p), ("d_vend", C.c_void_p),
                ("d_xfinal", C.c_void_p)]


ODE_FORWARD_EULER, ODE_RK4 = 0, 1
_ODE_METHODS = {"forward-euler": ODE_FORWARD_EULER, "euler": ODE_FORWARD_EULER, "rk4": ODE_RK4}


class OdeArgs(C.Structure):
    _fields_ = [("n", C.c_size_t), ("d_x0", C.c_void_p), ("dt_out", C.c_double), ("dt_int", C.c_double), ("nout", C.c_size_t),
                ("method", C.c_int), ("wrap_periodic", C.c_int), ("box", C.c_int), ("evals_per_launch", C.c_int),
                ("goal", C.c_void_p), ("keep", C.c_void_p), ("save_every", C.c_size_t), ("d_traj", C.c_void_p),
                ("d_u", C.c_void_p), ("d_cost", C.c_void_p), ("d_stop_step", C.c_void_p), ("d_stop_reason", C.c_void_p),
                ("d_vend", C.c_void_p), ("d_xfinal", C.c_void_p)]


class ModelSpec(C.Structure):
    _fields_ = [("source", C.c_char_p), ("name", C.c_char_p), ("d", C.c_int), ("du", C.c_int), ("udep_mask", C.c_uint),
                ("uconst_mask", C.c_uint), ("stage_udep", C.c_int), ("box", C.c_int), ("nranks", C.c_int),
                ("ranks", C.POINTER(C.c_int))]


class ModelSpecEx(C.Structure):
    _fields_ = [("base", ModelSpec), ("game", C.c_int)]


class ModelSpecFh(C.Structure):
    _fields_ = [("ex", ModelSpecEx), ("horizon", C.c_int)]


MODEL_USER = 1000
GAME_MINMAX, GAME_MAXMIN = 0, 1
_GAME_ORDERS = {"minmax": GAME_MINMAX, "upper": GAME_MINMAX, "maxmin": GAME_MAXMIN, "lower": GAME_MAXMIN}

VARIANT_AUTO, VARIANT_FIBER_PER_WAVE, VARIANT_FIBER_PER_LANE, VARIANT_FIBER_PAIR, VARIANT_FIBER_QUAD = 0, 1, 2, 3, 4


class C3scHipError(RuntimeError):
    pass


def load_library():
    global _LIB
    if _LIB is None:
        if not os.path.exists(LIB_PATH):
            raise C3scHipError(f"{LIB_PATH} is missing: build it with `python -c 'import __graft_entry__ as g; g.build()'` "
                               "or `make -C c3sc_amd/csrc`.  There is no CPU fallback.")
        import torch
        L = C.CDLL(LIB_PATH)
        L.c3sc_hip_last_error.restype = C.c_char_p
        L.c3sc_hip_last_error.argtypes = [C.c_void_p]
        L.c3sc_hip_last_kernel.restype = C.c_char_p
        L.c3sc_hip_last_kernel.argtypes = [C.c_void_p]
        L.c3sc_hip_ctx_destroy.restype = None
        L.c3sc_hip_ctx_destroy.argtypes = [C.c_void_p]
        L.c3sc_hip_bellman_fibers.argtypes = [C.c_void_p, C.c_int, C.c_size_t, C.c_void_p, C.c_void_p, C.c_void_p,
                                              C.c_void_p, C.c_void_p]
        L.c3sc_hip_stencil_fibers.argtypes = [C.c_void_p, C.c_int, C.c_size_t, C.c_void_p, C.c_void_p, C.c_void_p,
                                              C.c_void_p]
        L.c3sc_hip_bellman_fibers_host.argtypes = [C.c_void_p, C.c_int, C.c_size_t, C.c_void_p, C.c_void_p, C.c_void_p,
                                                   C.c_void_p]
        L.c3sc_hip_stencil_fibers_host.argtypes = [C.c_void_p, C.c_int, C.c_size_t, C.c_void_p, C.c_void_p, C.c_void_p]
        L.c3sc_hip_policy_fibers.argtypes = [C.c_void_p, C.c_int, C.c_size_t, C.c_void_p, C.c_void_p, C.c_void_p,
                                             C.c_void_p, C.c_void_p]
        L.c3sc_hip_policy_fibers_host.argtypes = [C.c_void_p, C.c_int, C.c_size_t, C.c_void_p, C.c_void_p, C.c_void_p,
                                                  C.c_void_p]
        L.c3sc_hip_stencil_fibers_nb_host.argtypes = [C.c_void_p, C.c_int, C.c_size_t, C.c_void_p, C.c_void_p, C.c_void_p,
                                                      C.c_void_p, C.c_void_p]
        L.c3sc_hip_bellman_fibers_tables_host.argtypes = [C.c_void_p, C.c_int, C.c_size_t] + [C.c_void_p] * 6
        L.c3sc_hip_policy_fibers_tables_host.argtypes = [C.c_void_p, C.c_int, C.c_size_t] + [C.c_void_p] * 6
        L.c3sc_hip_launch_count.restype = C.c_ulonglong
        L.c3sc_hip_last_partition.argtypes = [C.c_void_p, C.c_int, C.c_void_p, C.c_size_t, C.POINTER(C.c_size_t), C.POINTER(C.c_int)]
        L.c3sc_hip_sync.argtypes = [C.c_void_p, C.c_void_p]
        L.c3sc_hip_timer_start.argtypes = [C.c_void_p, C.c_void_p]
        L.c3sc_hip_timer_stop.argtypes = [C.c_void_p, C.c_void_p, C.POINTER(C.c_float)]
        L.c3sc_hip_upload_value_device.argtypes = [C.c_void_p, c_size_p, C.POINTER(C.c_void_p), C.c_void_p]
        L.c3sc_hip_cross_setup.argtypes = [C.c_void_p, c_size_p, C.POINTER(c_i32_p), C.POINTER(c_i32_p), C.c_int]
        L.c3sc_hip_cross_iteration.argtypes = [C.c_void_p, C.c_int, C.c_void_p]
        L.c3sc_hip_cross_confirm.argtypes = [C.c_void_p, c_int_p, C.c_void_p]
        L.c3sc_hip_cross_options.argtypes = [C.c_void_p, C.c_int, C.c_double]
        L.c3sc_hip_cross_iteration_pi.argtypes = [C.c_void_p, C.c_void_p, C.c_longlong, C.c_void_p]
        L.c3sc_hip_cross_grow_memo.argtypes = [C.c_void_p]
        L.c3sc_hip_cross_fetch.argtypes = [C.c_void_p, C.POINTER(c_double_p), C.POINTER(c_i32_p), C.POINTER(c_i32_p),
                                           C.POINTER(C.c_ulonglong), C.c_void_p]
        L.c3sc_hip_set_interp.argtypes = [C.c_void_p, C.c_int]
        L.c3sc_hip_stencil_points.argtypes = [C.c_void_p, C.c_size_t, C.c_void_p, C.c_void_p, C.c_void_p, C.c_void_p]
        L.c3sc_hip_simulate.argtypes = [C.c_void_p, C.POINTER(SimArgs), C.c_void_p]
        L.c3sc_hip_integrate.argtypes = [C.c_void_p, C.POINTER(OdeArgs), C.c_void_p]
        L.c3sc_hip_integrate_host.argtypes = [C.c_void_p, C.POINTER(OdeArgs)]
        L.c3sc_hip_normals.argtypes = [C.c_uint64, C.c_uint64, C.c_size_t, C.c_uint64, C.c_size_t, C.c_int, c_double_p]
        L.c3sc_hip_model_compile.argtypes = [C.POINTER(ModelSpec), c_int_p]
        L.c3sc_hip_model_code_object.argtypes = [C.POINTER(ModelSpec), C.c_void_p, c_size_p]
        L.c3sc_hip_model_log.restype = C.c_char_p
        L.c3sc_hip_model_log.argtypes = []
        L.c3sc_hip_model_compile_ex.argtypes = [C.POINTER(ModelSpecEx), c_int_p]
        L.c3sc_hip_model_code_object_ex.argtypes = [C.POINTER(ModelSpecEx), C.c_void_p, c_size_p]
        L.c3sc_hip_set_game.argtypes = [C.c_void_p, C.c_int, C.c_int, c_double_p, C.c_int, c_double_p, C.c_int]
        L.c3sc_hip_model_compile_fh.argtypes = [C.POINTER(ModelSpecFh), c_int_p]
        L.c3sc_hip_model_code_object_fh.argtypes = [C.POINTER(ModelSpecFh), C.c_void_p, c_size_p]
        L.c3sc_hip_set_horizon_step.argtypes = [C.c_void_p, C.c_double]
        L.c3sc_hip_upload_value_stack.argtypes = [C.c_void_p, C.c_int, c_size_p, C.POINTER(c_double_p)]
        _LIB = L
    return _LIB


def normals(seed: int, traj0: int, ntraj: int, step0: int, nsteps: int, dw: int) -> np.ndarray:
    L = load_library()
    out = np.empty((ntraj, nsteps, dw), dtype=np.float64)
    rc = L.c3sc_hip_normals(C.c_uint64(seed), C.c_uint64(traj0), C.c_size_t(ntraj), C.c_uint64(step0), C.c_size_t(nsteps),
                            C.c_int(dw), out.ctypes.data_as(c_double_p))
    if rc != 0:
        raise C3scHipError(f"c3sc_hip_normals failed (code {rc})")
    return out


def _model_spec(source, d, du, ranks, box, udep_mask, uconst_mask, stage_udep, name):
    rk = (C.c_int * max(1, len(ranks)))(*ranks)
    spec = ModelSpec(source.encode(), name.encode() if name is not None else None, int(d), int(du), int(udep_mask),
                     int(uconst_mask), 1 if stage_udep else 0, 1 if box else 0, len(ranks), rk if len(ranks) else None)
    spec._keep = rk
    return spec


def _model_fail(rc, what):
    log = load_library().c3sc_hip_model_log().decode(errors="replace")
    raise C3scHipError(f"{what} failed (code {rc}): {log}", rc)


def compile_model(source: str, d: int, du: int, ranks=(4, 8), box: bool = False, udep_mask: int = 0, uconst_mask: int = 0,
                  stage_udep: bool = True, name: Optional[str] = None, game: bool = False, horizon: bool = False) -> int:
    L = load_library()
    spec = _model_spec(source, d, du, tuple(ranks), box, udep_mask, uconst_mask, stage_udep, name)
    mid = C.c_int(0)
    if horizon:
        fh = ModelSpecFh(ModelSpecEx(spec, 1 if game else 0), 1)
        rc = L.c3sc_hip_model_compile_fh(C.byref(fh), C.byref(mid))
    elif game:
        ex = ModelSpecEx(spec, 1)
        rc = L.c3sc_hip_model_compile_ex(C.byref(ex), C.byref(mid))
    else:
        rc = L.c3sc_hip_model_compile(C.byref(spec), C.byref(mid))
    if rc != 0:
        _model_fail(rc, "c3sc_hip_model_compile")
    return mid.value


def code_object(source: str, d: int, du: int, ranks=(4, 8), box: bool = False, udep_mask: int = 0, uconst_mask: int = 0,
                stage_udep: bool = True, name: Optional[str] = None, game: bool = False, horizon: bool = False) -> bytes:
    L = load_library()
    spec = _model_spec(source, d, du, tuple(ranks), box, udep_mask, uconst_mask, stage_udep, name)
    cap = 16 << 20
    for _ in range(2):
        buf = C.create_string_buffer(cap)
        size = C.c_size_t(cap)
        if horizon:
            fh = ModelSpecFh(ModelSpecEx(spec, 1 if game else 0), 1)
            rc = L.c3sc_hip_model_code_object_fh(C.byref(fh), buf, C.byref(size))
        elif game:
            rc = L.c3sc_hip_model_code_object_ex(C.byref(ModelSpecEx(spec, 1)), buf, C.byref(size))
        else:
            rc = L.c3sc_hip_model_code_object(C.byref(spec), buf, C.byref(size))
        if rc == 0:
            return buf.raw[:size.value]
        if size.value <= cap:
            break
        cap = size.value
    _model_fail(rc, "c3sc_hip_model_code_object")


def game_split(index, nw: int):
    i = np.asarray(index)
    iu = np.where(i < 0, -1, i // nw)
    iw = np.where(i < 0, -1, i % nw)
    if np.ndim(index) == 0:
        return int(iu), int(iw)
    return iu, iw


def _f64(a):
    return np.ascontiguousarray(a, dtype=np.float64)


def _ptr_array(arrs):
    arr = (c_double_p * len(arrs))(*[a.ctypes.data_as(c_double_p) for a in arrs])
    arr._keep = arrs
    return arr


class BellmanEngine:

    def __init__(self, device: int = 0):
        self.L = load_library()
        h = C.c_void_p()
        rc = self.L.c3sc_hip_ctx_create(C.c_int(device), C.byref(h))
        if rc != 0:
            raise C3scHipError(f"c3sc_hip_ctx_create(device={device}) failed with code {rc} (no usable HIP device?)")
        self.h = h
        self.device = device
        self.w = None

    def close(self):
        if getattr(self, "h", None):
            self.L.c3sc_hip_ctx_destroy(self.h)
            self.h = None

    def __del__(self):
        try:
            self.close()
        except Exception:
            pass

    def _chk(self, rc, what):
        if rc != 0:
            msg = self.L.c3sc_hip_last_error(self.h)
            raise C3scHipError(f"{what} failed (code {rc}): {msg.decode() if msg else ''}")

    def set_grid(self, ngrid: Sequence[int], xgrid: Sequence[np.ndarray]):
        ng = np.ascontiguousarray(ngrid, dtype=np.uintp)
        xs = [_f64(g) for g in xgrid]
        self._chk(self.L.c3sc_hip_set_grid(self.h, C.c_int(len(ng)), ng.ctypes.data_as(c_size_p), _ptr_array(xs)),
                  "set_grid")
        self.ngrid = [int(n) for n in ngrid]
        self.d = len(self.ngrid)

# ... 357 lines not shown
```

include/c3sc_hip.h:

```cpp
#ifndef C3SC_HIP_H
#define C3SC_HIP_H

#ifndef __HIPCC_RTC__
#include <stddef.h>
#include <stdint.h>
#endif

#ifdef __cplusplus
extern "C" {
#endif

#define C3SC_MAX_DIM 12
#define C3SC_MAX_OBSTACLES 10
#define C3SC_MAX_PARAMS 8
#define C3SC_MAX_DU 4

enum {
    C3SC_OK = 0,
    C3SC_ERR_ARG = 1,
    C3SC_ERR_HIP = 2,
    C3SC_ERR_UNSUPPORTED = 3,
    C3SC_ERR_NODEVICE = 4
};

// ... 52 lines not shown
                               const int32_t *const *d_policy, double *const *d_out, int32_t *const *d_absorbed, void *stream);
int c3sc_hip_policy_fibers_host(c3sc_hip_ctx *ctx, int k, size_t F, const int32_t *h_idx, const int32_t *h_policy,
                                double *h_out, int32_t *h_absorbed);

int c3sc_hip_set_control_box(c3sc_hip_ctx *ctx, int du, const double *lb, const double *ub, int grid, int polish);
int c3sc_hip_bellman_fibers_box(c3sc_hip_ctx *ctx, int k, size_t F, const int32_t *d_idx, double *d_out, double *d_uopt,
                                int32_t *d_absorbed, void *stream);
int c3sc_hip_bellman_fibers_box_host(c3sc_hip_ctx *ctx, int k, size_t F, const int32_t *h_idx, double *h_out, double *h_uopt,
                                     int32_t *h_absorbed);
int c3sc_hip_policy_fibers_box(c3sc_hip_ctx *ctx, int k, size_t F, const int32_t *d_idx, const double *d_policy_u,
                               double *d_out, int32_t *d_absorbed, void *stream);
int c3sc_hip_policy_fibers_box_host(c3sc_hip_ctx *ctx, int k, size_t F, const int32_t *h_idx, const double *h_policy_u,
                                    double *h_out, int32_t *h_absorbed);

int c3sc_hip_bellman_fibers_tables(c3sc_hip_ctx *ctx, int k, size_t F, const int32_t *d_idx, const double *d_tables,
                                   const double *d_costs2, double *d_out, int32_t *d_uidx, int32_t *d_absorbed,
                                   void *stream);
int c3sc_hip_bellman_fibers_tables_host(c3sc_hip_ctx *ctx, int k, size_t F, const int32_t *h_idx,
                                        const double *h_tables, const double *h_costs2, double *h_out,
                                        int32_t *h_uidx, int32_t *h_absorbed);
int c3sc_hip_policy_fibers_tables(c3sc_hip_ctx *ctx, int k, size_t F, const int32_t *d_idx, const double *d_tables,
                                  const double *d_costs2, const int32_t *d_policy, double *d_out, int32_t *d_absorbed,
                                  void *stream);
int c3sc_hip_policy_fibers_tables_host(c3sc_hip_ctx *ctx, int k, size_t F, const int32_t *h_idx,
                                       const double *h_tables, const double *h_costs2, const int32_t *h_policy,
                                       double *h_out, int32_t *h_absorbed);

int c3sc_hip_stencil_fibers(c3sc_hip_ctx *ctx, int k, size_t F, const int32_t *d_idx, double *d_costs,
                            int32_t *d_absorbed, void *stream);

int c3sc_hip_stencil_fibers_nb(c3sc_hip_ctx *ctx, int k, size_t F, const int32_t *d_idx, const int32_t *d_nb_fixed,
                               const int32_t *d_nb_vary, double *d_costs, int32_t *d_absorbed, void *stream);
int c3sc_hip_stencil_fibers_nb_host(c3sc_hip_ctx *ctx, int k, size_t F, const int32_t *h_idx,
                                    const int32_t *h_nb_fixed, const int32_t *h_nb_vary, double *h_costs,
                                    int32_t *h_absorbed);

int c3sc_hip_bellman_fibers_host(c3sc_hip_ctx *ctx, int k, size_t F, const int32_t *h_idx, double *h_out,
                                 int32_t *h_uidx, int32_t *h_absorbed);
int c3sc_hip_stencil_fibers_host(c3sc_hip_ctx *ctx, int k, size_t F, const int32_t *h_idx, double *h_costs,
                                 int32_t *h_absorbed);

int c3sc_hip_set_interp(c3sc_hip_ctx *ctx, int constelm);
int c3sc_hip_stencil_points(c3sc_hip_ctx *ctx, size_t n, const double *d_x, double *d_out, int32_t *d_absorbed, void *stream);

typedef struct c3sc_hip_sim_args {
    size_t n;
    const double *d_x0;
    double dt;
    size_t nsteps;
    uint64_t traj_offset;
    uint64_t seed;
    const double *d_noise;
    int wrap_periodic;
    int box;
    int steps_per_launch;
    size_t save_every;
    double *d_traj;
    double *d_u;
    double *d_cost;
    int64_t *d_exit;
    double *d_vend;
    double *d_xfinal;
} c3sc_hip_sim_args;
int c3sc_hip_simulate(c3sc_hip_ctx *ctx, const c3sc_hip_sim_args *args, void *stream);
int c3sc_hip_simulate_host(c3sc_hip_ctx *ctx, const c3sc_hip_sim_args *args);

enum { C3SC_ODE_FORWARD_EULER = 0, C3SC_ODE_RK4 = 1 };
typedef struct c3sc_hip_ode_args {
    size_t n;
    const double *d_x0;
    double dt_out;
    double dt_int;
    size_t nout;
    int method;
    int wrap_periodic;
    int box;
    int evals_per_launch;
    const double *goal;
    const double *keep;
    size_t save_every;
    double *d_traj;
    double *d_u;
    double *d_cost;
    int64_t *d_stop_step;
    int32_t *d_stop_reason;
    double *d_vend;
    double *d_xfinal;
} c3sc_hip_ode_args;
int c3sc_hip_integrate(c3sc_hip_ctx *ctx, const c3sc_hip_ode_args *args, void *stream);
int c3sc_hip_integrate_host(c3sc_hip_ctx *ctx, const c3sc_hip_ode_args *args);
int c3sc_hip_normals(uint64_t seed, uint64_t traj0, size_t ntraj, uint64_t step0, size_t nsteps, int dw, double *out);

int c3sc_hip_cross_setup(c3sc_hip_ctx *ctx, const size_t *ranks, const int32_t *const *I, const int32_t *const *J, int new_sweep);
int c3sc_hip_cross_iteration(c3sc_hip_ctx *ctx, int box, void *stream);
int c3sc_hip_cross_iteration_streamed(c3sc_hip_ctx *ctx, int box, void *stream);
int c3sc_hip_cross_wait_core(c3sc_hip_ctx *ctx, int k, double *h_core);
int c3sc_hip_cross_confirm(c3sc_hip_ctx *ctx, int *confirmed, void *stream);
int c3sc_hip_cross_speculate(c3sc_hip_ctx *ctx, c3sc_hip_ctx *policy_ctx, long long policy_tag, int box, int *confirmed, void *stream);
int c3sc_hip_cross_iteration_pi(c3sc_hip_ctx *ctx, c3sc_hip_ctx *policy_ctx, long long policy_tag, void *stream);
int c3sc_hip_cross_options(c3sc_hip_ctx *ctx, int warm_pivots, double swap_tol);
int c3sc_hip_cross_grow_memo(c3sc_hip_ctx *ctx);
int c3sc_hip_cross_fetch(c3sc_hip_ctx *ctx, double *const *h_cores, int32_t *const *h_I, int32_t *const *h_J, unsigned long long *info,
                         void *stream);
void c3sc_hip_cross_free(c3sc_hip_ctx *ctx);

typedef struct c3sc_hip_comm c3sc_hip_comm;
int c3sc_hip_comm_unique_id(void *id128);
int c3sc_hip_comm_create(c3sc_hip_ctx *ctx, int world, int rank, const void *id128, c3sc_hip_comm **out);
void c3sc_hip_comm_destroy(c3sc_hip_comm *comm);
int c3sc_hip_comm_world(const c3sc_hip_comm *comm);
int c3sc_hip_comm_rank(const c3sc_hip_comm *comm);
int c3sc_hip_comm_allgather(c3sc_hip_comm *comm, const double *d_send, double *d_recv, size_t count, void *stream);
int c3sc_hip_cross_set_comm(c3sc_hip_ctx *ctx, c3sc_hip_comm *comm);
int c3sc_hip_comm_exchange(double *out, size_t F, size_t N, size_t lo, size_t hi, void *comm);

typedef struct c3sc_hip_model_spec {
    const char *source;
    const char *name;
    int d, du;
    unsigned udep_mask, uconst_mask;
    int stage_udep;
    int box;
    int nranks;
    const int *ranks;
} c3sc_hip_model_spec;
int c3sc_hip_model_compile(const c3sc_hip_model_spec *spec, int *model_id);
int c3sc_hip_model_code_object(const c3sc_hip_model_spec *spec, void *buf, size_t *size);
const char *c3sc_hip_model_log(void);

enum { C3SC_GAME_MINMAX = 0, C3SC_GAME_MAXMIN = 1 };
int c3sc_hip_set_game(c3sc_hip_ctx *ctx, int du_min, int nu, const double *U, int nw, const double *W, int order);
typedef struct c3sc_hip_model_spec_ex {
    c3sc_hip_model_spec base;
    int game;
} c3sc_hip_model_spec_ex;
int c3sc_hip_model_compile_ex(const c3sc_hip_model_spec_ex *spec, int *model_id);
int c3sc_hip_model_code_object_ex(const c3sc_hip_model_spec_ex *spec, void *buf, size_t *size);

typedef struct c3sc_hip_model_spec_fh {
    c3sc_hip_model_spec_ex ex;
    int horizon;
} c3sc_hip_model_spec_fh;
int c3sc_hip_model_compile_fh(const c3sc_hip_model_spec_fh *spec, int *model_id);
int c3sc_hip_model_code_object_fh(const c3sc_hip_model_spec_fh *spec, void *buf, size_t *size);
int c3sc_hip_set_horizon_step(c3sc_hip_ctx *ctx, double dt);
int c3sc_hip_upload_value_stack(c3sc_hip_ctx *ctx, int nstack, const size_t *ranks, const double *const *cores);

int c3sc_hip_sync(c3sc_hip_ctx *ctx, void *stream);
int c3sc_hip_get_status(c3sc_hip_ctx *ctx, unsigned *flags, int clear);
const char *c3sc_hip_last_kernel(const c3sc_hip_ctx *ctx);

int c3sc_hip_debug_read(c3sc_hip_ctx *ctx, unsigned long long *out, size_t n);
unsigned long long c3sc_hip_launch_count(void);
int c3sc_hip_last_partition(c3sc_hip_ctx *ctx, int slot, int32_t *perm, size_t cap, size_t *F, int *nlive);

int c3sc_hip_timer_start(c3sc_hip_ctx *ctx, void *stream);
int c3sc_hip_timer_stop(c3sc_hip_ctx *ctx, void *stream, float *ms);

int c3sc_hip_peak_fma_f64(c3sc_hip_ctx *ctx, double *tflops);
int c3sc_hip_peak_mfma_f64(c3sc_hip_ctx *ctx, double *tflops);

#ifdef __cplusplus
}
#endif
#endif
```

Before: 34.12 billion.

## Precompute three-core edge product tables for the car7d rank-10 pair kernel

Adds a precomputed table of products of the first three (and last three) tensor-train cores per grid triple, built lazily by a new kernel and reused across Bellman sweeps until the cores change. For car7d rank-10 with k<2, a new partitioned kernel variant reads these tables instead of folding the third core per fiber, which removes one matrix-vector contraction per side. The cost is up to 16MB of extra arena memory per side, a one-time table build with cross-stream event waits, and more template instantiations.

```diff
diff --git a/c3sc_amd/csrc/c3sc_hip.hip b/c3sc_amd/csrc/c3sc_hip.hip
--- a/c3sc_amd/csrc/c3sc_hip.hip
+++ b/c3sc_amd/csrc/c3sc_hip.hip
@@ -78,6 +78,30 @@
     }
 }
 
+struct Tab3Jobs {
+    long tab2[2], core[2], dst[2];
+    int n3[2], npairs[2];
+};
+__global__ void k_pair_tab3(double *__restrict__ arena, const Tab3Jobs J, int RP)
+{
+    const int sd = blockIdx.y;
+    const bool left = sd == 0;
+    const double *tab2 = arena + J.tab2[sd], *core = arena + J.core[sd];
+    double *dst = arena + J.dst[sd];
+    const long np = J.npairs[sd], total = (long)J.n3[sd] * np * RP;
+    for (long e = (long)blockIdx.x * blockDim.x + threadIdx.x; e < total; e += (long)gridDim.x * blockDim.x) {
+        const long row = e / RP;
+        const int c = (int)(e - row * RP);
+        const long i3 = row / np, pair = row - i3 * np;
+        const double *vec = tab2 + pair * RP;
+        const double *mat = left ? core + i3 * RP * RP + (long)c * RP : core + i3 * RP * RP + c;
+        const int ms = left ? 1 : RP;
+        double t = 0.0;
+        for (int s = 0; s < RP; s++) t = fma(vec[s], mat[(long)s * ms], t);
+        dst[e] = t;
+    }
+}
+
 __global__ void k_quad_aux(const double *__restrict__ core, double *__restrict__ coreT, double *__restrict__ aop, int N, int RP)
 {
     const int C = RP / 4, MB = (C + 3) / 4;
@@ -244,6 +268,7 @@
     return rp;
 }
 
+static unsigned long long g_tab3_launches = 0;
 static unsigned long long g_launches = 0;
 static int fill_args(c3sc_hip_ctx *c, int k, size_t F, KArgs &A, bool need_model);
 
@@ -402,6 +427,7 @@
         if (c->join_ev[i]) (void)hipEventDestroy(c->join_ev[i]);
     }
     if (c->fork_ev) (void)hipEventDestroy(c->fork_ev);
+    if (c->tab3_ev) (void)hipEventDestroy(c->tab3_ev);
     if (c->ev0) (void)hipEventDestroy(c->ev0);
     if (c->ev1) (void)hipEventDestroy(c->ev1);
     delete c;
@@ -626,6 +652,13 @@
         tabR_off = (long)off;
         off += (size_t)pair_tab_doubles(c->ngrid[d - 2], c->ngrid[d - 1], rp);
     }
+    long tab3L_off = 0, tab3R_off = 0;
+    if (tabL_off && pair_tab3_reserved(d, c->ngrid, rp)) {
+        tab3L_off = (long)off;
+        off += (size_t)pair_tab3_doubles(c->ngrid[0], c->ngrid[1], c->ngrid[2], rp);
+        tab3R_off = (long)off;
+        off += (size_t)pair_tab3_doubles(c->ngrid[d - 3], c->ngrid[d - 2], c->ngrid[d - 1], rp);
+    }
     long qimgL_off[MAXD] = {0}, qimgR_off[MAXD] = {0};
     if (rp % 4 == 0 && have_quad) {
         for (int m = 0; m < d; m++) {
@@ -648,6 +681,9 @@
     for (int m = 0; m < d; m++) { c->core_off[m] = core_off[m]; c->coreT_off[m] = coreT_off[m]; c->aop_off[m] = aop_off[m]; c->img_off[m] = img_off[m]; c->qimgL_off[m] = qimgL_off[m]; c->qimgR_off[m] = qimgR_off[m]; }
     c->tabL_off = tabL_off;
     c->tabR_off = tabR_off;
+    c->tab3L_off = tab3L_off;
+    c->tab3R_off = tab3R_off;
+    c->tab3_stale = true;
     for (int m = 0; m <= d; m++) c->ranks[m] = ranks[m];
     c->rp = rp;
     *cores_doubles = primary_end - stat;
@@ -833,6 +869,8 @@
     A.img_base = c->arena;
     if (c->tabL_off && (c->tabL_off != pair_tabL_off(A, c->rp) || c->tabR_off != pair_tabR_off(A, c->rp)))
         return fail(c, C3SC_ERR_ARG, "launch: the pair kernel's product tables are not where the kernel looks for them");
+    if (c->tab3L_off && (c->tab3L_off != pair_tab3L_off(A, c->rp) || c->tab3R_off != pair_tab3R_off(A, c->rp)))
+        return fail(c, C3SC_ERR_ARG, "launch: the pair kernel's three-core tables are not where the kernel looks for them");
     A.cends = c->cends;
     A.memo_keys = nullptr;
     A.skip = c->skip_flag;
@@ -899,16 +937,50 @@
     return v > 0 ? v : -1;
 }
 
+static bool partitions(const KernelEntry *e, const KArgs &A)
+{
+    if (e->variant != C3SC_VARIANT_FIBER_PAIR || e->rtc || A.ncand > 64) return false;
+    bool faces = false;
+    for (int m = 0; m < A.d; m++) faces = faces || (m != A.k && A.bctype[m] == C3SC_ABSORB);
+    const long fmin = fiber_partition_min();
+    return faces && fmin >= 0 && A.F >= fmin && A.F <= 0x40000000L;
+}
+
+static bool runs_tab3(const c3sc_hip_ctx *c, const KernelEntry *e, const KArgs &A)
+{
+    if (!c->tab3L_off || fpp_table3_optout(A.d, e->rp, A.k) || !partitions(e, A)) return false;
+    const char *env = getenv("C3SC_PAIR_TABLE3");
+    return !(env && *env && atol(env) == 0);
+}
+
+static int ensure_tab3(c3sc_hip_ctx *c, hipStream_t st)
+{
+    if (!c->tab3_stale) {
+        if (st != c->tab3_stream) HIPCHK(c, hipStreamWaitEvent(st, c->tab3_ev, 0));
+        return C3SC_OK;
+    }
+    const int d = c->d, rp = c->rp;
+    if (!c->tab3_ev) HIPCHK(c, hipEventCreateWithFlags(&c->tab3_ev, hipEventDisableTiming));
+    Tab3Jobs J;
+    J.tab2[0] = c->tabL_off; J.core[0] = c->core_off[2]; J.dst[0] = c->tab3L_off;
+    J.n3[0] = c->ngrid[2]; J.npairs[0] = c->ngrid[0] * c->ngrid[1];
+    J.tab2[1] = c->tabR_off; J.core[1] = c->core_off[d - 3]; J.dst[1] = c->tab3R_off;
+    J.n3[1] = c->ngrid[d - 3]; J.npairs[1] = c->ngrid[d - 2] * c->ngrid[d - 1];
+    const long total = std::max((long)J.n3[0] * J.npairs[0], (long)J.n3[1] * J.npairs[1]) * rp;
+    hipLaunchKernelGGL(k_pair_tab3, dim3((unsigned)std::min<long>((total + 255) / 256, 4096), 2), dim3(256), 0, st, c->arena, J, rp);
+    HIPCHK(c, hipGetLastError());
+    HIPCHK(c, hipEventRecord(c->tab3_ev, st));
+    c->tab3_stream = st;
+    c->tab3_stale = false;
+    return C3SC_OK;
+}
+
 static int partition_fibers(c3sc_hip_ctx *c, const KernelEntry *e, const KArgs &A, LaunchIO &io, int slot, int &launched)
 {
     io.perm = nullptr;
     io.nlive = nullptr;
     launched = 0;
-    if (e->variant != C3SC_VARIANT_FIBER_PAIR || e->rtc || A.ncand > 64) return C3SC_OK;
-    bool faces = false;
-    for (int m = 0; m < A.d; m++) faces = faces || (m != A.k && A.bctype[m] == C3SC_ABSORB);
-    const long fmin = fiber_partition_min();
-    if (!faces || fmin < 0 || A.F < fmin || A.F > 0x40000000L) return C3SC_OK;
+    if (!partitions(e, A)) return C3SC_OK;
     PartArgs P;
     P.d = A.d;
     P.k = A.k;
@@ -971,6 +1043,11 @@
         }
         c->last_kernel = e->name;
         arm_memo(c, e, A);
+        io.tab3 = runs_tab3(c, e, A);
+        if (io.tab3) {
+            rc = ensure_tab3(c, io.stream);
+            if (rc != C3SC_OK) return rc;
+        }
         rc = partition_fibers(c, e, A, io, part_slot, part_launches);
         if (rc != C3SC_OK) return rc;
         he = launch_entry(*e, A, io);
@@ -980,6 +1057,7 @@
         declined.push_back(e);
     }
     g_launches += 1 + part_launches;
+    if (io.tab3 && io.perm) g_tab3_launches++;
     c->status_cache_valid = false;
     HIPCHK(c, he);
     return C3SC_OK;
@@ -1007,6 +1085,20 @@
             if (d_out[q] == d_out[s] && F[s] > 0) return fail(c, C3SC_ERR_ARG, "bellman_fibers_all: two segments share an output array");
     }
     hipStream_t st = (hipStream_t)stream;
+    if (overlap && c->tab3L_off && c->tab3_stale && c->game_gsz == 0 && c->hz_dt <= 0.0) {
+        const long fmin = fiber_partition_min();
+        for (int s = 0; s < nk && c->tab3_stale; s++) {
+            if (F[s] == 0 || fmin < 0 || (long)F[s] < fmin) continue;
+            KArgs A;
+            int rc = fill_args(c, ks[s], F[s], A, true);
+            if (rc != C3SC_OK) return rc;
+            const KernelEntry *e = find_kernel(c->model, c->d, c->rp, A.N, c->variant, ks[s], F[s]);
+            if (e && e->rp == c->rp && runs_tab3(c, e, A)) {
+                rc = ensure_tab3(c, st);
+                if (rc != C3SC_OK) return rc;
+            }
+        }
+    }
     if (overlap) {
         HIPCHK(c, hipSetDevice(c->device));
         if (!c->fork_ev) {
@@ -1623,6 +1715,7 @@
 }
 
 unsigned long long c3sc_hip_launch_count(void) { return g_launches; }
+unsigned long long c3sc_hip_table3_launch_count(void) { return g_tab3_launches; }
 
 int c3sc_hip_last_partition(c3sc_hip_ctx *c, int slot, int32_t *perm, size_t cap, size_t *F, int *nlive)
 {
diff --git a/c3sc_amd/csrc/ctx.hpp b/c3sc_amd/csrc/ctx.hpp
--- a/c3sc_amd/csrc/ctx.hpp
+++ b/c3sc_amd/csrc/ctx.hpp
@@ -50,6 +50,10 @@
     long img_off[c3sc::MAXD] = {0};
     long qimgL_off[c3sc::MAXD] = {0}, qimgR_off[c3sc::MAXD] = {0};
     long tabL_off = 0, tabR_off = 0;
+    long tab3L_off = 0, tab3R_off = 0;
+    bool tab3_stale = true;
+    hipStream_t tab3_stream = nullptr;
+    hipEvent_t tab3_ev = nullptr;
     int obs_off = 0, cands_off = 0, tab_off[4] = {0, 0, 0, 0}, cfeat_off = 0;
     unsigned *d_status = nullptr;
     unsigned status_cache = 0;
diff --git a/c3sc_amd/csrc/inst_car7d_fpp.hip b/c3sc_amd/csrc/inst_car7d_fpp.hip
--- a/c3sc_amd/csrc/inst_car7d_fpp.hip
+++ b/c3sc_amd/csrc/inst_car7d_fpp.hip
@@ -20,6 +20,17 @@
 CAR7_MAP(4, 0x0Bu, 7)
 CAR7_MAP(5, 0x0Fu, 5)
 CAR7_MAP(6, 0x17u, 5)
+C3SC_FPP_TABLE3(Car7D, 10)
+#define CAR7_PLAN3(K, ROUNDS, PRODUCTS)                                                                                  \
+    static_assert(PairMap<Car7D, K, true, true>::plan().staged == (ROUNDS), "car7d: three-core staging rounds of K = " #K); \
+    static_assert(PairMap<Car7D, K, true, true>::plan().products == (PRODUCTS), "car7d: three-core products of K = " #K);
+CAR7_PLAN3(0, 3, 24)
+CAR7_PLAN3(1, 2, 16)
+CAR7_PLAN3(2, 1, 8)
+CAR7_PLAN3(3, 0, 0)
+CAR7_PLAN3(4, 1, 6)
+CAR7_PLAN3(5, 2, 8)
+CAR7_PLAN3(6, 3, 16)
 REG7P(4)
 REG7P(10)
 }
diff --git a/c3sc_amd/csrc/kernel_common.hpp b/c3sc_amd/csrc/kernel_common.hpp
--- a/c3sc_amd/csrc/kernel_common.hpp
+++ b/c3sc_amd/csrc/kernel_common.hpp
@@ -71,8 +71,13 @@
 __host__ __device__ constexpr long arena_block(long doubles) { return (doubles + 15) & ~15L; }
 __host__ __device__ constexpr long pair_img_doubles(int nodes, int per) { return arena_block((long)nodes * (per | 1) + 2); }
 __host__ __device__ constexpr long pair_tab_doubles(int na, int nb, int rp) { return arena_block((long)na * nb * rp); }
-__host__ __device__ inline long pair_tabL_off(const KArgs &A, int rp) { return A.pair_img_off[A.d - 1] + pair_img_doubles(A.ngrid[A.d - 1], rp); }
-__host__ __device__ inline long pair_tabR_off(const KArgs &A, int rp) { return pair_tabL_off(A, rp) + pair_tab_doubles(A.ngrid[0], A.ngrid[1], rp); }
+__host__ __device__ constexpr long pair_tabL_off(const KArgs &A, int rp) { return A.pair_img_off[A.d - 1] + pair_img_doubles(A.ngrid[A.d - 1], rp); }
+__host__ __device__ constexpr long pair_tabR_off(const KArgs &A, int rp) { return pair_tabL_off(A, rp) + pair_tab_doubles(A.ngrid[0], A.ngrid[1], rp); }
+
+constexpr long PAIR_TAB3_MAX_BYTES = 16L << 20;
+__host__ __device__ constexpr long pair_tab3_doubles(int na, int nb, int nc, int rp) { return arena_block((long)na * nb * nc * rp); }
+__host__ __device__ constexpr long pair_tab3L_off(const KArgs &A, int rp) { return pair_tabR_off(A, rp) + pair_tab_doubles(A.ngrid[A.d - 2], A.ngrid[A.d - 1], rp); }
+__host__ __device__ constexpr long pair_tab3R_off(const KArgs &A, int rp) { return pair_tab3L_off(A, rp) + pair_tab3_doubles(A.ngrid[0], A.ngrid[1], A.ngrid[2], rp); }
 
 struct KeyLevels {
     int n, major, minor;
@@ -96,6 +101,14 @@
 #define FPP_GROUP_FOLD 1
 #endif
 __host__ __device__ constexpr bool fpp_group_fold_optout(int d, int rp, int k) { return d == 7 && rp == 10 && k == 1; }
+__host__ __device__ constexpr bool fpp_table3_registered(int d, int rp) { return FPP_EDGE_TABLES && d == 7 && rp == 10; }
+__host__ __device__ constexpr bool pair_tab3_reserved(int d, const int *ngrid, int rp)
+{
+    return d >= 6 && fpp_table3_registered(d, rp) &&
+           pair_tab3_doubles(ngrid[0], ngrid[1], ngrid[2], rp) * (long)sizeof(double) <= PAIR_TAB3_MAX_BYTES &&
+           pair_tab3_doubles(ngrid[d - 3], ngrid[d - 2], ngrid[d - 1], rp) * (long)sizeof(double) <= PAIR_TAB3_MAX_BYTES;
+}
+__host__ __device__ constexpr bool fpp_table3_optout(int d, int rp, int k) { return d == 7 && rp == 10 && k >= 2; }
 __host__ __device__ constexpr KeyLevels fpp_group_levels(int d, int rp, int k)
 {
     const bool direct = d <= FPP_DIRECT_MAXD && rp <= 8;
diff --git a/c3sc_amd/csrc/kernel_fiber_pair.hpp b/c3sc_amd/csrc/kernel_fiber_pair.hpp
--- a/c3sc_amd/csrc/kernel_fiber_pair.hpp
+++ b/c3sc_amd/csrc/kernel_fiber_pair.hpp
@@ -206,7 +206,7 @@
     int staged;
     int products;
 };
-template <class Model, int K, bool TAB = false>
+template <class Model, int K, bool TAB = false, bool TAB3 = false>
 struct PairMap {
     typedef PairPark<Model, K> PK;
     static constexpr int D = Model::D, NIT = D + 2, UL = D, UR = D + 1;
@@ -220,7 +220,8 @@
         __host__ __device__ static constexpr int depth(int m) { return LEFT ? m : D - 1 - m; }
         __host__ __device__ static constexpr int core(int q) { return LEFT ? q : D - 1 - q; }
         __host__ __device__ static constexpr bool tab() { return TAB && NC >= 2; }
-        __host__ __device__ static constexpr int first() { return core(tab() ? 2 : 1); }
+        __host__ __device__ static constexpr int td() { return !tab() ? 0 : (TAB3 && NC >= 3 ? 3 : 2); }
+        __host__ __device__ static constexpr int first() { return core(tab() ? td() : 1); }
         __host__ __device__ static constexpr int nsteps() { return NC - depth(first()) > 0 ? NC - depth(first()) : 0; }
         __host__ __device__ static constexpr int step(int i) { return core(depth(first()) + i); }
         __host__ __device__ static constexpr int first_merged()
@@ -237,13 +238,14 @@
         }
         __host__ __device__ static constexpr int cost_u()
         {
-            int c = NC - 1 - depth(first_merged()) - (tab() && first_merged() == EDGE);
+            int c = NC - 1 - depth(first_merged());
+            if (td() > depth(first_merged()) + 1) c = NC - td();
             for (int q = depth(first()); q < NC; q++) c += 2 * mg(core(q));
             return c;
         }
         __host__ __device__ static constexpr int cost_pair(int m)
         {
-            return (tab() && depth(m) <= 1) ? 2 * (NC - 2) : (m != EDGE ? 2 : 0) + 2 * (NC - 1 - depth(m));
+            return depth(m) < td() ? 2 * (NC - td()) : (m != EDGE ? 2 : 0) + 2 * (NC - 1 - depth(m));
         }
         __host__ __device__ static constexpr int created(int m) { return !mg(m) ? m : (m == first_merged() ? U : -1); }
         template <int H>
@@ -258,6 +260,8 @@
         __host__ __device__ static constexpr int base() { return LEFT ? 0 : Side<true>::template before<H>(K); }
         template <int H>
         __host__ __device__ static constexpr int slot(int it) { return base<H>() + before<H>(it == U ? first_merged() : it); }
+        template <int H>
+        __host__ __device__ static constexpr bool owns(int m) { return owner(mg(m) ? U : m) == H; }
     };
     typedef Side<true> SL;
     typedef Side<false> SR;
@@ -294,11 +298,16 @@
     {
         return 3 + (m < K ? SL::template before<0>(m) + SL::template before<1>(m) : SR::template before<0>(m) + SR::template before<1>(m));
     }
-    __host__ __device__ static constexpr int uniform_rounds() { return fpp_key_levels(D, K, TAB).n; }
+    __host__ __device__ static constexpr bool staged(int m) { return m < K ? m >= SL::first() : (m > K && m <= SR::first()); }
+    __host__ __device__ static constexpr int uniform_rounds()
+    {
+        constexpr KeyLevels kl = fpp_key_levels(D, K, TAB);
+        return (kl.n > 0 && staged(kl.major)) + (kl.n > 1 && staged(kl.minor));
+    }
     __host__ __device__ static constexpr int uniform_products()
     {
         constexpr KeyLevels kl = fpp_key_levels(D, K, TAB);
-        return (kl.n > 0 ? level_products(kl.major) : 0) + (kl.n > 1 ? level_products(kl.minor) : 0);
+        return (kl.n > 0 && staged(kl.major) ? level_products(kl.major) : 0) + (kl.n > 1 && staged(kl.minor) ? level_products(kl.minor) : 0);
     }
     __host__ __device__ static constexpr int owner(int it)
     {
@@ -353,7 +362,7 @@
         tlast = now__;                                                    \
     }
 
-template <class Model, int RP, int K, int H, bool PART, bool LEFT, int m, int NOWN, class Combine>
+template <class Model, int RP, int K, int H, bool PART, bool T3, bool LEFT, int m, int NOWN, class Combine>
 __device__ __attribute__((always_inline)) inline void fold_step(const KArgs &A, const double *__restrict__ ro, double *sK,
                                                                const int (&fi)[Model::D], const int (&nbm)[Model::D], const int (&nbp)[Model::D],
                                                                const double (&rpm)[Model::D], const double (&rpp)[Model::D], double (&V)[RP],
@@ -362,7 +371,7 @@
 {
     constexpr int D = Model::D;
     constexpr bool DIRECT = fpp_direct<Model, RP>();
-    typedef PairMap<Model, K, fpp_edge_tables<Model, RP>()> PM;
+    typedef PairMap<Model, K, fpp_edge_tables<Model, RP>(), T3> PM;
     typedef typename PM::template Side<LEFT> SD;
     constexpr bool RV = SD::ROWVEC;
     constexpr int BASE = SD::template base<H>();
@@ -429,7 +438,7 @@
     fold_level<GROUP && (m == KL.major || (KL.n > 1 && m == KL.minor))>(fi[m], body);
 }
 
-template <class Model, int RP, int K, int H, bool FORCED, bool PART>
+template <class Model, int RP, int K, int H, bool FORCED, bool PART, bool T3 = false>
 __device__ __attribute__((always_inline)) inline void fiber_pair_body(const KArgs &A, const double *__restrict__ ro,
                                                                      const int32_t *__restrict__ idx, double *__restrict__ outv,
                                                                      int32_t *__restrict__ uidx, int32_t *__restrict__ absorbed,
@@ -441,7 +450,10 @@
     constexpr int RH = RP / 2;
     typedef PairPark<Model, K> PK;
     constexpr bool ET = fpp_edge_tables<Model, RP>();
-    typedef PairMap<Model, K, ET> PM;
+    typedef PairMap<Model, K, ET, T3> PM;
+    static_assert(!T3 || (PART && ET), "the three-core tables serve the partitioned kernels with edge tables");
+    static_assert(PM::nv() == PairMap<Model, K, ET>::nv() && PM::gslot(D + 1) == PairMap<Model, K, ET>::gslot(D + 1),
+                  "the table depth moves no slot of the node loop");
     constexpr FoldPlan PL = PM::plan();
     constexpr int NV = PM::nv();
     constexpr int NVL = PM::SL::nv();
@@ -535,9 +547,58 @@
 #pragma unroll
         for (int a = 0; a < RP; a++) { L[a] = (a == 0) ? 1.0 : 0.0; R[a] = (a == 0) ? 1.0 : 0.0; }
 
+        auto side3 = [&](auto lc, double (&V)[RP]) __attribute__((always_inline)) {
+            constexpr bool LEFT = decltype(lc)::value;
+            typedef typename PM::template Side<LEFT> SD;
+            constexpr int c0 = SD::core(0), c1 = SD::core(1), c2 = SD::core(2);
+            constexpr int BASE = SD::template base<H>();
+            const double *T = ro + (LEFT ? pair_tab3L_off(A, RP) : pair_tab3R_off(A, RP));
+            const int n0 = A.ngrid[c0], n1 = A.ngrid[c1];
+            auto row = [&](int j0, int j1, int j2) __attribute__((always_inline)) -> const double * {
+                return T + (LEFT ? ((long)j2 * n0 + j0) * n1 + j1 : ((long)j2 * n1 + j1) * n0 + j0) * RP;
+            };
+            constexpr bool OWN0 = SD::template owns<H>(c0), OWN1 = SD::template owns<H>(c1), OWN2 = SD::template owns<H>(c2);
+            double tm[3][RP], tp[3][RP];
+            load_row16<RP>(row(fi[c0], fi[c1], fi[c2]), V);
+            if constexpr (OWN0) {
+                load_row16<RP>(row(nbm[c0], fi[c1], fi[c2]), tm[0]);
+                load_row16<RP>(row(nbp[c0], fi[c1], fi[c2]), tp[0]);
+            }
+            if constexpr (OWN1) {
+                load_row16<RP>(row(fi[c0], nbm[c1], fi[c2]), tm[1]);
+                load_row16<RP>(row(fi[c0], nbp[c1], fi[c2]), tp[1]);
+            }
+            if constexpr (OWN2) {
+                load_row16<RP>(row(fi[c0], fi[c1], nbm[c2]), tm[2]);
+                load_row16<RP>(row(fi[c0], fi[c1], nbp[c2]), tp[2]);
+            }
+            __builtin_amdgcn_sched_barrier(0);
+            auto combine = [&]() __attribute__((always_inline)) {
+                static_for<3>([&](auto qc) __attribute__((always_inline)) {
+                    constexpr int q = decltype(qc)::value, m = SD::core(q);
+                    if constexpr (SD::template owns<H>(m)) {
+                        constexpr int before = SD::template before<H>(m);
+#pragma unroll
+                        for (int b = 0; b < RP; b++) {
+                            if constexpr (PM::mg(m)) {
+                                constexpr int su = PM::template lslot<H>(SD::U);
+                                const double nw = fma(rpp[m], tp[q][b], rpm[m] * tm[q][b]);
+                                W[su][b] = (m == SD::first_merged()) ? nw : W[su][b] + nw;
+                            } else { W[BASE + before][b] = tm[q][b]; W[BASE + before + 1][b] = tp[q][b]; }
+                        }
+                    }
+                });
+            };
+            if constexpr (SD::nsteps() == 0) combine();
+            static_for<SD::nsteps()>([&](auto ic) __attribute__((always_inline)) {
+                fold_step<Model, RP, K, H, PART, T3, LEFT, SD::step(decltype(ic)::value)>(A, ro, sK, fi, nbm, nbp, rpm, rpp, V, W, seg, tlast, combine);
+            });
+        };
+
         FPP_STAMP(0)
         if (!(C3SC_STAMPS_ON && (A.dbg & 1))) {
-        if constexpr (K > 0) {
+        if constexpr (K > 0 && PM::SL::td() == 3) side3(std::true_type{}, L);
+        else if constexpr (K > 0) {
             constexpr bool OWN0 = PM::SL::tab() && (PM::mg(0) ? PM::owner(PM::UL) == H : PM::owner(0) == H);
             constexpr bool OWN1 = PM::SL::tab() && (PM::mg(1) ? PM::owner(PM::UL) == H : PM::owner(1) == H);
             double t0m[OWN0 ? RP : 1], t0p[OWN0 ? RP : 1], t1m[OWN1 ? RP : 1], t1p[OWN1 ? RP : 1];
@@ -600,12 +661,13 @@
                 }
             }
             auto left_step = [&](auto mc) __attribute__((always_inline)) {
-                fold_step<Model, RP, K, H, PART, true, decltype(mc)::value>(A, ro, sK, fi, nbm, nbp, rpm, rpp, L, W, seg, tlast, left_combine);
+                fold_step<Model, RP, K, H, PART, T3, true, decltype(mc)::value>(A, ro, sK, fi, nbm, nbp, rpm, rpp, L, W, seg, tlast, left_combine);
             };
             static_for<PM::SL::nsteps()>([&](auto ic) __attribute__((always_inline)) { left_step(std::integral_constant<int, PM::SL::step(decltype(ic)::value)>{}); });
         }
 
-        if constexpr (K < D - 1) {
+        if constexpr (K < D - 1 && PM::SR::td() == 3) side3(std::false_type{}, R);
+        else if constexpr (K < D - 1) {
             constexpr bool OWN0 = PM::SR::tab() && (PM::mg(D - 1) ? PM::owner(PM::UR) == H : PM::owner(D - 1) == H);
             constexpr bool OWN1 = PM::SR::tab() && (PM::mg(D - 2) ? PM::owner(PM::UR) == H : PM::owner(D - 2) == H);
             double t0m[OWN0 ? RP : 1], t0p[OWN0 ? RP : 1], t1m[OWN1 ? RP : 1], t1p[OWN1 ? RP : 1];
@@ -669,7 +731,7 @@
                 }
             }
             auto right_step = [&](auto mc) __attribute__((always_inline)) {
-                fold_step<Model, RP, K, H, PART, false, decltype(mc)::value>(A, ro, sK, fi, nbm, nbp, rpm, rpp, R, W, seg, tlast, right_combine);
+                fold_step<Model, RP, K, H, PART, T3, false, decltype(mc)::value>(A, ro, sK, fi, nbm, nbp, rpm, rpp, R, W, seg, tlast, right_combine);
             };
             static_for<PM::SR::nsteps()>([&](auto ic) __attribute__((always_inline)) { right_step(std::integral_constant<int, PM::SR::step(decltype(ic)::value)>{}); });
         }
@@ -1230,4 +1292,18 @@
     if (st) atomicOr(A.status, st);
 }
 
+template <class Model, int RP, int K, bool FORCED>
+__global__ void __launch_bounds__(FPP_THREADS, (fpp_waves_per_simd<Model, RP>()))
+    k_fiber_pair_part3(const KArgs A, const double *__restrict__ ro, const int32_t *__restrict__ idx, double *__restrict__ outv,
+                       int32_t *__restrict__ uidx, int32_t *__restrict__ absorbed, const int32_t *__restrict__ perm,
+                       const int32_t *__restrict__ nlive_p)
+{
+    extern __shared__ double sKp[];
+    unsigned st = 0;
+    const int h = __builtin_amdgcn_readfirstlane(threadIdx.x >> 6);
+    if (h == 0) fiber_pair_body<Model, RP, K, 0, FORCED, true, true>(A, ro, idx, outv, uidx, absorbed, perm, nlive_p, sKp, st);
+    else fiber_pair_body<Model, RP, K, 1, FORCED, true, true>(A, ro, idx, outv, uidx, absorbed, perm, nlive_p, sKp, st);
+    if (st) atomicOr(A.status, st);
 }
+
+}
diff --git a/c3sc_amd/csrc/launch_fpp.hpp b/c3sc_amd/csrc/launch_fpp.hpp
--- a/c3sc_amd/csrc/launch_fpp.hpp
+++ b/c3sc_amd/csrc/launch_fpp.hpp
@@ -14,7 +14,20 @@
     return swap > rows ? swap : rows;
 }
 
-template <class Model, int RP, int K, bool FORCED, bool PART>
+template <class Model, int RP>
+struct FppTable3 {
+    static constexpr bool value = false;
+};
+#define C3SC_FPP_TABLE3(MODEL, RP)                                                                                              \
+    template <>                                                                                                                 \
+    struct FppTable3<MODEL, RP> {                                                                                               \
+        static constexpr bool value = true;                                                                                     \
+        static_assert(fpp_table3_registered(MODEL::D, RP) && fpp_edge_tables<MODEL, RP>(), "the host reserves no tables here"); \
+    };
+template <class Model, int RP, int K>
+constexpr bool fpp_table3() { return FppTable3<Model, RP>::value && !fpp_table3_optout(Model::D, RP, K); }
+
+template <class Model, int RP, int K, bool FORCED, bool PART, bool T3 = false>
 hipError_t launch_fpp_impl(const KArgs &A, const LaunchIO &io)
 {
     constexpr int D = Model::D;
@@ -33,7 +46,9 @@
     B.tbl_off = (int)doubles;
     doubles += (size_t)CandLds<Model>::doubles(A.ncand) + (size_t)NodeLds<Model, K>::doubles(A.N);
     const size_t shmem = doubles * sizeof(double);
+    static_assert(!T3 || PART, "the three-core kernel is a partitioned one");
     const void *kern = PART ? (const void *)k_fiber_pair_part<Model, RP, K, FORCED> : (const void *)k_fiber_pair<Model, RP, K, FORCED>;
+    if constexpr (T3) kern = (const void *)k_fiber_pair_part3<Model, RP, K, FORCED>;
     static LaunchCache cache;
     int blocks_per_cu = 1, num_cu = 256;
     hipError_t e = cache.prepare(kern, FPP_THREADS, shmem, blocks_per_cu, num_cu);
@@ -43,7 +58,10 @@
     int grid = (int)(ntiles < cap ? ntiles : cap);
     if (ntiles >= 8 * cap && ntiles < 0x7fffffffL) grid = (int)ntiles;
     if (grid < 1) grid = 1;
-    if constexpr (PART)
+    if constexpr (T3)
+        hipLaunchKernelGGL((k_fiber_pair_part3<Model, RP, K, FORCED>), dim3(grid), dim3(FPP_THREADS), shmem, io.stream, B, io.ro, io.idx, io.out,
+                           io.uidx, io.absorbed, io.perm, io.nlive);
+    else if constexpr (PART)
         hipLaunchKernelGGL((k_fiber_pair_part<Model, RP, K, FORCED>), dim3(grid), dim3(FPP_THREADS), shmem, io.stream, B, io.ro, io.idx, io.out,
                            io.uidx, io.absorbed, io.perm, io.nlive);
     else
@@ -55,6 +73,8 @@
 template <class Model, int RP, int K>
 hipError_t launch_fpp(const KArgs &A, const LaunchIO &io)
 {
+    if constexpr (fpp_table3<Model, RP, K>())
+        if (io.perm && io.tab3) return A.forced ? launch_fpp_impl<Model, RP, K, true, true, true>(A, io) : launch_fpp_impl<Model, RP, K, false, true, true>(A, io);
     if (io.perm) return A.forced ? launch_fpp_impl<Model, RP, K, true, true>(A, io) : launch_fpp_impl<Model, RP, K, false, true>(A, io);
     return A.forced ? launch_fpp_impl<Model, RP, K, true, false>(A, io) : launch_fpp_impl<Model, RP, K, false, false>(A, io);
 }
diff --git a/c3sc_amd/csrc/registry.hpp b/c3sc_amd/csrc/registry.hpp
--- a/c3sc_amd/csrc/registry.hpp
+++ b/c3sc_amd/csrc/registry.hpp
@@ -25,6 +25,7 @@
     const void *sim = nullptr;
     const int32_t *perm = nullptr;
     const int32_t *nlive = nullptr;
+    bool tab3 = false;
 };
 #endif
 
diff --git a/c3sc_amd/engine.py b/c3sc_amd/engine.py
--- a/c3sc_amd/engine.py
+++ b/c3sc_amd/engine.py
@@ -24,7 +24,7 @@
     "c3sc_hip_set_control_box", "c3sc_hip_bellman_fibers_box", "c3sc_hip_bellman_fibers_box_host", "c3sc_hip_policy_fibers_box",
     "c3sc_hip_policy_fibers_box_host",
     "c3sc_hip_stencil_fibers_host", "c3sc_hip_stencil_fibers_nb", "c3sc_hip_stencil_fibers_nb_host", "c3sc_hip_sync", "c3sc_hip_get_status", "c3sc_hip_last_kernel",
-    "c3sc_hip_debug_read", "c3sc_hip_launch_count", "c3sc_hip_last_partition", "c3sc_hip_timer_start", "c3sc_hip_timer_stop", "c3sc_hip_peak_fma_f64", "c3sc_hip_peak_mfma_f64",
+    "c3sc_hip_debug_read", "c3sc_hip_launch_count", "c3sc_hip_table3_launch_count", "c3sc_hip_last_partition", "c3sc_hip_timer_start", "c3sc_hip_timer_stop", "c3sc_hip_peak_fma_f64", "c3sc_hip_peak_mfma_f64",
     "c3sc_hip_set_interp", "c3sc_hip_stencil_points", "c3sc_hip_simulate", "c3sc_hip_simulate_host", "c3sc_hip_normals",
     "c3sc_hip_integrate", "c3sc_hip_integrate_host",
     "c3sc_hip_model_compile", "c3sc_hip_model_code_object", "c3sc_hip_model_log",
@@ -107,6 +107,7 @@
         L.c3sc_hip_bellman_fibers_tables_host.argtypes = [C.c_void_p, C.c_int, C.c_size_t] + [C.c_void_p] * 6
         L.c3sc_hip_policy_fibers_tables_host.argtypes = [C.c_void_p, C.c_int, C.c_size_t] + [C.c_void_p] * 6
         L.c3sc_hip_launch_count.restype = C.c_ulonglong
+        L.c3sc_hip_table3_launch_count.restype = C.c_ulonglong
         L.c3sc_hip_last_partition.argtypes = [C.c_void_p, C.c_int, C.c_void_p, C.c_size_t, C.POINTER(C.c_size_t), C.POINTER(C.c_int)]
         L.c3sc_hip_sync.argtypes = [C.c_void_p, C.c_void_p]
         L.c3sc_hip_timer_start.argtypes = [C.c_void_p, C.c_void_p]
diff --git a/include/c3sc_hip.h b/include/c3sc_hip.h
--- a/include/c3sc_hip.h
+++ b/include/c3sc_hip.h
@@ -228,6 +228,7 @@
 
 int c3sc_hip_debug_read(c3sc_hip_ctx *ctx, unsigned long long *out, size_t n);
 unsigned long long c3sc_hip_launch_count(void);
+unsigned long long c3sc_hip_table3_launch_count(void);
 int c3sc_hip_last_partition(c3sc_hip_ctx *ctx, int slot, int32_t *perm, size_t cap, size_t *F, int *nlive);
 
 int c3sc_hip_timer_start(c3sc_hip_ctx *ctx, void *stream);
```

After: 34.55 billion (median of 6 runs). 1.01x the previous value.
